# Cyan4973/FiniteStateEntropy

Hardware: AMD Instinct MI355X
Metric: MB/s encode+decode per GPU on 32KB probagen blocks; bit-exact vs CPU ref (higher is better)
Workload: dtype u8; 1 GPU; probagen Proba14, 100000 x 32KB blocks per GPU, FSE encode+decode (one-shot calls at the reference's default limits: tableLog 11, decode maxLog 12), bit-exact check; blocks_per_gpu=100000, block_bytes=32768, codec=fse, parity=fse: roundtrip-all-blocks

## Files before the change

finitestateentropy_amd/_lib.py:

```python
import ctypes
import os
import subprocess

_CSRC = os.path.join(os.path.dirname(os.path.abspath(__file__)), "csrc")


def library_path():
    if os.environ.get("FSEHIP_LIB"):
        return os.environ["FSEHIP_LIB"]
    return os.path.join(_CSRC, "libfsehip.so")


def build_library(force=False):
    if force:
        subprocess.check_call(["make", "-C", _CSRC, "clean"], stdout=subprocess.DEVNULL)
    subprocess.check_call(["make", "-C", _CSRC, "-j8", "all"], stdout=subprocess.DEVNULL)
    return library_path()


_LIB = None


def load():
    global _LIB
    if _LIB is None:
        path = library_path()
        if not os.path.exists(path):
            raise OSError("libfsehip.so is missing (%s): build it with finitestateentropy_amd.build_library(); "
                          "there is no CPU fallback" % path)
        _LIB = ctypes.CDLL(path)
    return _LIB
```

finitestateentropy_amd/csrc/capi.hip:

```cpp
#include "internal.h"
#include <string.h>
#include <stdlib.h>
#include <new>

extern "C" unsigned FSEHIP_isError(size_t code) { return code > FSEHIP_ERROR(maxCode); }

extern "C" const char* FSEHIP_getErrorName(size_t code)
{
    if (!FSEHIP_isError(code)) return "No error detected";
    switch ((int)(0 - code)) {
        case FSEHIP_error_GENERIC: return "Error (generic)";
        case FSEHIP_error_dstSize_tooSmall: return "Destination buffer is too small";
        case FSEHIP_error_srcSize_wrong: return "Src size is incorrect";
        case FSEHIP_error_corruption_detected: return "Corrupted block detected";
        case FSEHIP_error_tableLog_tooLarge: return "tableLog requires too much memory : unsupported";
        case FSEHIP_error_maxSymbolValue_tooLarge: return "Unsupported max Symbol Value : too large";
        case FSEHIP_error_maxSymbolValue_tooSmall: return "Specified maxSymbolValue is too small";
        case FSEHIP_error_workSpace_tooSmall: return "workspace buffer is too small";
        default: return "Unspecified error code";
    }
}

extern "C" const char* FSEHIP_versionString(void) { return "fsehip 0.3 (gfx950)"; }

extern "C" void FSEHIP_shardRange(size_t nBlocks, int rank, int world, size_t* first, size_t* count)
{
    if (world < 1) world = 1;
    if (rank < 0) rank = 0;
    const size_t base = nBlocks / (size_t)world, rem = nBlocks % (size_t)world, r = (size_t)rank;
    const size_t lo = r * base + (r < rem ? r : rem);
    if (first) *first = lo;
    if (count) *count = r < (size_t)world ? base + (r < rem ? 1 : 0) : 0;
}

#include <mutex>
#include <vector>
#include <utility>
namespace {
std::mutex g_devMutex;
const int MAX_DEVS = 64;
DevProps g_props[MAX_DEVS];
std::vector<std::pair<int, const void*>> g_ldsAttrDone;
}
const DevProps& dev_props()
{
    static const DevProps none = { 0, 0, false };
    int dev = 0;
    if (hipGetDevice(&dev) != hipSuccess || dev < 0 || dev >= MAX_DEVS) return none;
    std::lock_guard<std::mutex> lock(g_devMutex);
    DevProps& p = g_props[dev];
    if (!p.ok) {
        hipDeviceProp_t prop;
        if (hipGetDeviceProperties(&prop, dev) == hipSuccess) {
            p.cus = prop.multiProcessorCount;
            p.ldsPerCU = (int)prop.maxSharedMemoryPerMultiProcessor;
            p.ok = true;
        }
    }
    return p;
}
hipError_t ensure_dyn_lds(const void* kernel, int bytes)
{
    int dev = 0;
    hipError_t e = hipGetDevice(&dev);
    if (e != hipSuccess) return e;
    std::lock_guard<std::mutex> lock(g_devMutex);
    for (auto& d : g_ldsAttrDone) if (d.first == dev && d.second == kernel) return hipSuccess;
    e = hipFuncSetAttribute(kernel, hipFuncAttributeMaxDynamicSharedMemorySize, bytes);
    if (e == hipSuccess) g_ldsAttrDone.emplace_back(dev, kernel);
    return e;
}

extern "C" int FSEHIP_deviceInfo(FSEHIP_DeviceInfo* info)
{
    int dev = 0;
    hipDeviceProp_t prop;
    CK(hipGetDevice(&dev));
    CK(hipGetDeviceProperties(&prop, dev));
    info->deviceOrdinal = dev;
    info->computeUnits = prop.multiProcessorCount;
    info->ldsBytesPerCU = (int)prop.maxSharedMemoryPerMultiProcessor;
    info->wavefrontSize = prop.warpSize;
    strncpy(info->archName, prop.gcnArchName, sizeof(info->archName) - 1);
    info->archName[sizeof(info->archName) - 1] = 0;
    return 0;
}

namespace {
std::mutex g_probeMutex;
struct Probe {
    bool on = false;
    std::vector<hipEvent_t> pool;
    size_t used = 0;
    struct Rec { int id; hipEvent_t a, b; };
    std::vector<Rec> recs;
    hipEvent_t pending[PK_COUNT] = {};
    hipEvent_t get()
    {
        if (used == pool.size()) { hipEvent_t e; if (hipEventCreate(&e) != hipSuccess) return nullptr; pool.push_back(e); }
        return pool[used++];
    }
} g_probe;
}
void probe_before(int id, hipStream_t s)
{
    if (!g_probe.on) return;
    std::lock_guard<std::mutex> lock(g_probeMutex);
    hipEvent_t e = g_probe.get();
    g_probe.pending[id] = e;
    if (e) (void)hipEventRecord(e, s);
}
void probe_after(int id, hipStream_t s)
{
    if (!g_probe.on) return;
    std::lock_guard<std::mutex> lock(g_probeMutex);
    hipEvent_t e = g_probe.get();
    if (e && g_probe.pending[id]) { (void)hipEventRecord(e, s); g_probe.recs.push_back({ id, g_probe.pending[id], e }); }
}
extern "C" int FSEHIP_probe_begin(void)
{
    std::lock_guard<std::mutex> lock(g_probeMutex);
    g_probe.on = true; g_probe.used = 0; g_probe.recs.clear();
    return 0;
}
extern "C" int FSEHIP_probe_collect(double* totalMs, unsigned* launches)
{
    for (int i = 0; i < 16; ++i) { totalMs[i] = 0; launches[i] = 0; }
    std::lock_guard<std::mutex> lock(g_probeMutex);
    g_probe.on = false;
    for (auto& r : g_probe.recs) {
        CK(hipEventSynchronize(r.b));
        float ms = 0;
        CK(hipEventElapsedTime(&ms, r.a, r.b));
        totalMs[r.id] += ms; launches[r.id] += 1;
    }
    g_probe.recs.clear(); g_probe.used = 0;
    return 0;
}

extern "C" void FSEHIP_probagen_table(uint8_t table[4096], double p)
{
    int remaining = 4096;
    unsigned pos = 0, s = 0;
    if (p == 0.0) p = 0.005;
    while (remaining) {
        unsigned n = (unsigned)(remaining * p);
        if (!n) n = 1;
        memset(table + pos, (int)(uint8_t)s, n);
        pos += n; s++; remaining -= (int)n;
    }
}

extern "C" int FSEHIP_probagen_batch(void* d_dst, size_t dstStride, size_t blockSize, size_t nBlocks,
                                     const uint8_t h_table[4096], uint32_t firstSeed, void* stream)
{
    return FSEHIP_probagen_batch_ex(d_dst, dstStride, blockSize, nBlocks, h_table, firstSeed, 1, stream);
}
extern "C" int FSEHIP_probagen_batch_ex(void* d_dst, size_t dstStride, size_t blockSize, size_t nBlocks,
                                        const uint8_t h_table[4096], uint32_t firstSeed, uint32_t seedStep, void* stream)
{
    hipStream_t s = (hipStream_t)stream;
    enum { SLOTS = 16 };
    struct Ring { u8* dev = nullptr; u8* pin = nullptr; int device = -1; unsigned next = 0; hipEvent_t ev[SLOTS] = {}; bool used[SLOTS] = {}; int nEv = 0;
                  void drop() { for (int i = 0; i < nEv; ++i) (void)hipEventDestroy(ev[i]); nEv = 0;
                                if (pin) (void)hipHostFree(pin); if (dev) (void)hipFree(dev); pin = nullptr; dev = nullptr; device = -1; (void)hipGetLastError(); } };
    struct Rings { std::vector<Ring> v; ~Rings() { for (auto& r : v) r.drop(); } };
    static thread_local Rings rings;
    int dev = 0;
    CK(hipGetDevice(&dev));
    Ring* rp = nullptr;
    for (auto& r : rings.v) if (r.device == dev) rp = &r;
    if (!rp) {
        Ring r;
        hipError_t e = hipMalloc((void**)&r.dev, SLOTS * 4096);
        if (e == hipSuccess) e = hipHostMalloc((void**)&r.pin, SLOTS * 4096, hipHostMallocDefault);
        for (int i = 0; i < SLOTS && e == hipSuccess; ++i) { e = hipEventCreateWithFlags(&r.ev[i], hipEventDisableTiming); if (e == hipSuccess) r.nEv = i + 1; }
        if (e != hipSuccess) { r.drop(); return (int)e; }
        r.device = dev;
        rings.v.push_back(r);
        rp = &rings.v.back();
    }
    Ring& ring = *rp;
    const unsigned k = ring.next++ % SLOTS;
    if (ring.used[k]) CK(hipEventSynchronize(ring.ev[k]));
    memcpy(ring.pin + 4096u * k, h_table, 4096);
    u8* const d_table = ring.dev + 4096u * k;
    hipError_t e = hipMemcpyAsync(d_table, ring.pin + 4096u * k, 4096, hipMemcpyHostToDevice, s);
    if (e == hipSuccess) e = launch_probagen((u8*)d_dst, dstStride, blockSize, nBlocks, d_table, firstSeed, seedStep, s);
    if (e == hipSuccess) { e = hipEventRecord(ring.ev[k], s); ring.used[k] = e == hipSuccess; }
    return (int)e;
}

__global__ void k_batch_arg_error(size_t* results, const size_t* sizes, size_t uniform, size_t dstCapacity, size_t nBlocks, size_t code, int mode)
{
    const size_t b = (size_t)blockIdx.x * blockDim.x + threadIdx.x;
    if (b >= nBlocks) return;
    size_t r = code;
    if (mode == 1) {
        const size_t n = sizes ? sizes[b] : uniform;
        if (n == 0 || dstCapacity == 0) r = 0;
        else if (n > FSEHIP_HUF_BLOCKSIZE_MAX) r = FERR(srcSize_wrong);
    }
    if (mode == 2) { const size_t n = sizes ? sizes[b] : uniform; if (n <= 1) r = 0; }
    results[b] = r;
}
int batch_arg_error(size_t* d_results, const size_t* d_sizes, size_t uniform, size_t dstCapacity, size_t nBlocks, size_t code, int mode, hipStream_t s)
{
    hipLaunchKernelGGL(k_batch_arg_error, dim3((unsigned)((nBlocks + 255) / 256)), dim3(256), 0, s, d_results, d_sizes, uniform, dstCapacity, nBlocks, code, mode);
    return (int)hipGetLastError();
}

__global__ void k_hdr_results(const u8* meta, size_t metaStride, size_t* results, size_t nBlocks)
{
// ... 23 lines not shown
```

finitestateentropy_amd/csrc/capi_batch.hip:

```cpp
#include "internal.h"

extern "C" int FSEHIP_HIST_count_batch(unsigned* d_counts, unsigned* d_maxSymbolValues, size_t* d_results,
                                       const void* d_src, size_t srcStride, const size_t* d_sizes, size_t uniformSize,
                                       size_t nBlocks, void* stream)
{
    HistArgs a;
    a.counts = d_counts; a.maxSVs = d_maxSymbolValues; a.uniformMaxSV = 255; a.useUniformIn = 0;
    a.results = d_results; a.src = mkview(d_src, srcStride, d_sizes, uniformSize); a.nBlocks = nBlocks;
    return (int)launch_hist(a, (hipStream_t)stream);
}

extern "C" int FSEHIP_FSE_compress_usingCTable_batch(void* d_dst, size_t dstStride, size_t dstCapacity, size_t* d_results,
                                                     const void* d_src, size_t srcStride, const size_t* d_sizes, size_t uniformSize,
                                                     const FSEHIP_FSE_CTable* d_ctables, size_t ctableStrideU32, unsigned maxTableLog,
                                                     size_t nBlocks, void* stream)
{
    if (maxTableLog == 0 || maxTableLog > FSEHIP_FSE_MAX_TABLELOG) maxTableLog = FSEHIP_FSE_MAX_TABLELOG;
    FseEncArgs a;
    a.dst = (u8*)d_dst; a.dstStride = dstStride; a.dstCapacity = dstCapacity; a.results = d_results;
    a.src = mkview(d_src, srcStride, d_sizes, uniformSize);
    a.ctables = d_ctables; a.ctStrideU32 = ctableStrideU32; a.meta = nullptr;
    a.maxTableLog = maxTableLog; a.G = 0; a.slotU32 = 0; a.nBlocks = nBlocks; a.list = nullptr; a.count = nullptr;
    return (int)launch_fse_encode_auto(a, (hipStream_t)stream);
}

extern "C" int FSEHIP_FSE_decompress_usingDTable_batch(void* d_dst, size_t dstStride, size_t dstCapacity, size_t* d_results,
                                                       const void* d_cSrc, size_t cStride, const size_t* d_cSizes, size_t uniformCSize,
                                                       const FSEHIP_FSE_DTable* d_dtables, size_t dtableStrideU32, unsigned maxTableLog,
                                                       size_t nBlocks, void* stream)
{
    if (maxTableLog == 0 || maxTableLog > FSEHIP_FSE_MAX_TABLELOG) maxTableLog = FSEHIP_FSE_MAX_TABLELOG;
    FseDecArgs a;
    a.dst = (u8*)d_dst; a.dstStride = dstStride; a.dstCapacity = dstCapacity; a.results = d_results;
    a.csrc = mkview(d_cSrc, cStride, d_cSizes, uniformCSize);
    a.dtables = d_dtables; a.dtStrideU32 = dtableStrideU32; a.atab = nullptr; a.symtab = nullptr; a.meta = nullptr;
    a.maxTableLog = maxTableLog; a.G = 0; a.slotU32 = 0; a.nBlocks = nBlocks; a.tlMin = 0; a.declineNb0 = 0; a.onlyDeclined = 0;
    a.symScratch = nullptr; a.slotBitmap = nullptr; a.nSlots = 0; a.scratchSlotBytes = 0;
    return (int)launch_fse_decode(a, (hipStream_t)stream);
}

#define WS_SLACK 2048
#define WS_MAX_CHUNK 131072
static size_t ws_pass_blocks(size_t nBlocks) { const size_t c = nBlocks < WS_MAX_CHUNK ? nBlocks : WS_MAX_CHUNK; return c ? c : 1; }
static size_t ws_size(size_t nBlocks, size_t perBlock, size_t pad = 0) { return ws_pass_blocks(nBlocks) * perBlock + pad + WS_SLACK; }
static size_t round_chunk(size_t limit, size_t perRound)
{
    if (perRound == 0 || limit < perRound) return limit;
    return limit / perRound * perRound;
}
static size_t ws_chunk(size_t workspaceBytes, size_t nBlocks, size_t perBlock, size_t pad = 0, size_t perRound = 0)
{
    if (workspaceBytes < perBlock + pad + WS_SLACK) return 0;
    const size_t chunk = (workspaceBytes - WS_SLACK - pad) / perBlock;
    return chunk >= nBlocks ? nBlocks : round_chunk(chunk, perRound);
}
static inline size_t pass_blocks(size_t nBlocks, size_t b0, size_t chunk) { return nBlocks - b0 < chunk ? nBlocks - b0 : chunk; }

struct Carver {
    u8* const base; u8* p;
    explicit Carver(void* ws) : base((u8*)ws), p((u8*)ws) {}
    template <class T> T* take(size_t bytes) { T* const r = (T*)p; p += align_up(bytes, 256); return r; }
    template <class T> T* last(size_t bytes) { T* const r = (T*)p; p += bytes; return r; }
    size_t used() const { return (size_t)(p - base); }
};
template <class Meta> struct CounterWs {
    static constexpr size_t bytes_per_block = 1024 + 4 + 8 + sizeof(Meta);
    unsigned* counts; unsigned* maxSVs; size_t* hres; Meta* meta;
    CounterWs(Carver& c, size_t chunk)
        : counts(c.take<unsigned>(chunk * 1024)), maxSVs(c.take<unsigned>(chunk * 4)), hres(c.take<size_t>(chunk * 8)), meta(c.take<Meta>(chunk * sizeof(Meta))) {}
    HistArgs hist_args(unsigned msv, const BlockView& src, size_t nb) const
    {
        HistArgs h;
        h.counts = counts; h.maxSVs = maxSVs; h.uniformMaxSV = msv; h.useUniformIn = 1; h.results = hres; h.src = src; h.nBlocks = nb;
        return h;
    }
};
template <class Meta> struct BuildCTableWs {
    static constexpr size_t bytes_per_block = CounterWs<Meta>::bytes_per_block;
    Carver c; CounterWs<Meta> cb;
    BuildCTableWs(void* ws, size_t chunk) : c(ws), cb(c, chunk) {}
    size_t end() const { return c.used(); }
};

struct FseCWs { size_t perBlock; size_t ctU32; size_t ts; unsigned maxTl; };
static FseCWs fse_cws(unsigned tableLog)
{
    FseCWs w;
    unsigned tl = tableLog ? tableLog : FSEHIP_FSE_DEFAULT_TABLELOG;
    if (tl < 9) tl = 9;
    if (tl > FSEHIP_FSE_MAX_TABLELOG) tl = FSEHIP_FSE_MAX_TABLELOG;
    w.maxTl = tl;
    w.ctU32 = FSEHIP_FSE_CTABLE_SIZE_U32(tl, 255);
    w.ts = (size_t)1 << tl;
    w.perBlock = 1024 + 4 + 8 + sizeof(FseMeta) + 4 * w.ctU32 + FSE_EBINS * sizeof(u32);
    return w;
}
struct FseCompWs {
    Carver c; CounterWs<FseMeta> cb; u32* ctables; u32* encLists; u32* encCounts;
    FseCompWs(void* ws, size_t chunk, const FseCWs& w)
        : c(ws), cb(c, chunk), ctables(c.take<u32>(chunk * 4 * w.ctU32)), encLists(c.take<u32>(chunk * FSE_EBINS * sizeof(u32))),
          encCounts(c.last<u32>(FSE_EBINS * sizeof(u32))) {}
    size_t end() const { return c.used(); }
};

extern "C" size_t FSEHIP_FSE_compress_batch_workspaceSize(size_t nBlocks, unsigned tableLog) { return ws_size(nBlocks, fse_cws(tableLog).perBlock); }

extern "C" int FSEHIP_FSE_compress_batch(void* d_dst, size_t dstStride, size_t dstCapacity, size_t* d_results,
                                         const void* d_src, size_t srcStride, const size_t* d_sizes, size_t uniformSize,
                                         unsigned maxSymbolValue, unsigned tableLog, size_t nBlocks,
                                         void* d_workspace, size_t workspaceBytes, void* stream)
{
    hipStream_t s = (hipStream_t)stream;
    if ((uintptr_t)d_workspace & 255u) return (int)hipErrorInvalidValue;
    if (nBlocks == 0) return 0;
    if (tableLog > FSEHIP_FSE_MAX_TABLELOG)
        return batch_arg_error(d_results, nullptr, 0, dstCapacity, nBlocks, FSEHIP_ERROR(tableLog_tooLarge), 0, s);
    if (maxSymbolValue > 255 && tableLog != 0) {
        const size_t wksp = 4 * (size_t)FSEHIP_FSE_CTABLE_SIZE_U32(FSEHIP_FSE_MAX_TABLELOG, 255) + ((size_t)1 << FSEHIP_FSE_MAX_TABLELOG);
        const size_t ctBytes = 4 * (1 + ((size_t)1 << (tableLog - 1)) + 2 * ((size_t)maxSymbolValue + 1));
        if (ctBytes <= wksp && wksp - ctBytes < 4096)
            return batch_arg_error(d_results, d_sizes, uniformSize, dstCapacity, nBlocks, FSEHIP_ERROR(workSpace_tooSmall), 2, s);
    }
    return fse_compress_view(d_dst, dstStride, dstCapacity, d_results, mkview(d_src, srcStride, d_sizes, uniformSize), maxSymbolValue, tableLog, nBlocks,
                             d_workspace, workspaceBytes, s);
}
int fse_compress_view(void* d_dst, size_t dstStride, size_t dstCapacity, size_t* d_results, const BlockView& srcAll, unsigned maxSymbolValue, unsigned tableLog,
                      size_t nBlocks, void* d_workspace, size_t workspaceBytes, hipStream_t s)
{
    const FseCWs w = fse_cws(tableLog);
    const size_t chunk = ws_chunk(workspaceBytes, nBlocks, w.perBlock, 0, fse_encode_blocks_per_round(w.maxTl));
    if (chunk == 0) return (int)hipErrorInvalidValue;
    const FseCompWs ws(d_workspace, chunk, w);
    if (ws.end() > workspaceBytes) return (int)hipErrorInvalidValue;
    unsigned msv = maxSymbolValue ? maxSymbolValue : 255;
    if (msv > 255) msv = 255;
    for (size_t b0 = 0; b0 < nBlocks; b0 += chunk) {
        const size_t nb = pass_blocks(nBlocks, b0, chunk);
        const BlockView src = subview(srcAll, b0);
        CK(launch_hist(ws.cb.hist_args(msv, src, nb), s));
        FseCPrepArgs c;
        c.counts = ws.cb.counts; c.maxSVs = ws.cb.maxSVs; c.histResults = ws.cb.hres; c.src = src;
        c.dst = (u8*)d_dst + b0 * dstStride; c.dstStride = dstStride; c.dstCapacity = dstCapacity;
        c.maxSVReq = msv; c.tableLogReq = tableLog;
        c.ctables = ws.ctables; c.ctStrideU32 = w.ctU32; c.maxTl = w.maxTl;
        c.meta = ws.cb.meta; c.results = d_results + b0; c.nBlocks = nb;
        CK(launch_fse_cprep(c, s));
        FseEncArgs e;
        e.dst = (u8*)d_dst + b0 * dstStride; e.dstStride = dstStride; e.dstCapacity = dstCapacity; e.results = d_results + b0;
        e.src = src; e.ctables = ws.ctables; e.ctStrideU32 = w.ctU32; e.meta = ws.cb.meta;
        e.maxTableLog = w.maxTl; e.G = 0; e.slotU32 = 0; e.nBlocks = nb; e.list = ws.encLists; e.count = ws.encCounts;
        CK(launch_fse_encode_auto(e, s));
    }
    return 0;
}

struct FseDecWs {
    static size_t bytes_per_block(unsigned maxLog) { return sizeof(FseMeta) + 512 + 3 * ((size_t)1 << maxLog) + FSE_DCLS_COUNT * sizeof(u32); }
    Carver c; FseMeta* meta; s16* norms; u16* atab; u8* symtab; u32* lists; u32* counts;
    FseDecWs(void* ws, size_t chunk, unsigned maxLog)
        : c(ws), meta(c.take<FseMeta>(chunk * sizeof(FseMeta))), norms(c.take<s16>(chunk * 512)), atab(c.take<u16>((chunk * 2) << maxLog)),
          symtab(c.take<u8>(chunk << maxLog)), lists(c.take<u32>(chunk * FSE_DCLS_COUNT * sizeof(u32))), counts(c.last<u32>(FSE_DCLS_COUNT * sizeof(u32))) {}
    size_t end() const { return c.used(); }
    FseDPrepArgs dprep_args(const BlockView& cs, unsigned maxLog, size_t* results, size_t nb) const
    {
        FseDPrepArgs d;
        d.csrc = cs; d.maxLog = maxLog; d.atab = atab; d.symtab = symtab; d.norms = norms; d.meta = meta; d.lists = lists; d.counts = counts;
        d.results = results; d.nBlocks = nb; d.rawRle = 0; d.origSizes = nullptr; d.uniformOrig = 0;
        return d;
    }
};
static_assert(5 * 255 + FSE_DCLS_COUNT * sizeof(u32) <= WS_SLACK && 6 * 255 + FSE_EBINS * sizeof(u32) <= WS_SLACK, "WS_SLACK covers the padding of the FSE workspaces");
static unsigned clamp_maxlog(unsigned maxLog) { return (maxLog == 0 || maxLog > FSEHIP_FSE_MAX_TABLELOG) ? FSEHIP_FSE_MAX_TABLELOG : maxLog; }

extern "C" size_t FSEHIP_FSE_decompress_batch_workspaceSize(size_t nBlocks, unsigned maxLog) { return ws_size(nBlocks, FseDecWs::bytes_per_block(clamp_maxlog(maxLog))); }

static int fse_decompress_impl(void* d_dst, size_t dstStride, size_t dstCapacity, size_t* d_results, const BlockView& csAll, unsigned maxLog, size_t nBlocks,
                               void* d_workspace, size_t workspaceBytes, hipStream_t s, const size_t* d_origSizes, size_t uniformOrig, int rawRle,
                               const u64* d_dstOffsets = nullptr, const size_t* d_dstCaps = nullptr)
{
    if ((uintptr_t)d_workspace & 255u) return (int)hipErrorInvalidValue;
    if (nBlocks == 0) return 0;
    maxLog = clamp_maxlog(maxLog);
    const size_t chunk = ws_chunk(workspaceBytes, nBlocks, FseDecWs::bytes_per_block(maxLog), 0, fse_decode_blocks_per_round(maxLog));
    if (chunk == 0) return (int)hipErrorInvalidValue;
    const FseDecWs ws(d_workspace, chunk, maxLog);
    if (ws.end() > workspaceBytes) return (int)hipErrorInvalidValue;
    for (size_t b0 = 0; b0 < nBlocks; b0 += chunk) {
        const size_t nb = pass_blocks(nBlocks, b0, chunk);
        const BlockView cs = subview(csAll, b0);
        if (rawRle) CK(launch_rawrle_expand((u8*)d_dst + b0 * dstStride, dstStride, dstCapacity, d_results + b0, cs, d_origSizes ? d_origSizes + b0 : nullptr, uniformOrig, nb, s));
        FseDPrepArgs d = ws.dprep_args(cs, maxLog, d_results + b0, nb);
        d.rawRle = rawRle; d.origSizes = d_origSizes ? d_origSizes + b0 : nullptr; d.uniformOrig = uniformOrig;
        CK(launch_fse_dprep(d, s));
        FseDecArgs e;
        e.dst = (u8*)d_dst + b0 * dstStride; e.dstStride = dstStride; e.dstCapacity = dstCapacity; e.results = d_results + b0;
        e.csrc = cs; e.dtables = nullptr; e.dtStrideU32 = 0; e.atab = ws.atab; e.symtab = ws.symtab; e.meta = ws.meta;
        e.maxTableLog = maxLog; e.G = 0; e.slotU32 = 0; e.nBlocks = nb; e.tlMin = 0; e.declineNb0 = 0; e.onlyDeclined = 0;
        e.symScratch = nullptr; e.slotBitmap = nullptr; e.nSlots = 0; e.scratchSlotBytes = 0;
        if (d_dstOffsets) { e.dst = (u8*)d_dst; e.dstOffsets = d_dstOffsets + b0; e.dstCaps = d_dstCaps + b0; }
        CK(launch_fse_decode_classes(e, ws.lists, ws.counts, s));
    }
    return 0;
}
extern "C" int FSEHIP_FSE_decompress_batch(void* d_dst, size_t dstStride, size_t dstCapacity, size_t* d_results,
                                           const void* d_cSrc, size_t cStride, const size_t* d_cSizes, size_t uniformCSize,
                                           unsigned maxLog, size_t nBlocks,
                                           void* d_workspace, size_t workspaceBytes, void* stream)
{
    return fse_decompress_impl(d_dst, dstStride, dstCapacity, d_results, mkview(d_cSrc, cStride, d_cSizes, uniformCSize), maxLog, nBlocks,
                               d_workspace, workspaceBytes, (hipStream_t)stream, nullptr, 0, 0);
}
int fse_decompress_view(void* d_dst, const u64* d_dstOffsets, const size_t* d_dstCaps, size_t* d_results, const BlockView& csrc, unsigned maxLog, size_t nBlocks,
                        void* d_workspace, size_t workspaceBytes, hipStream_t s)
{
    return fse_decompress_impl(d_dst, 0, 0, d_results, csrc, maxLog, nBlocks, d_workspace, workspaceBytes, s, nullptr, 0, 0, d_dstOffsets, d_dstCaps);
}
extern "C" int FSEHIP_FSE_decompress_packed_batch(void* d_dst, size_t dstStride, size_t dstCapacity, size_t* d_results,
                                                  const void* d_packed, const uint64_t* d_offsets, const size_t* d_origSizes, size_t uniformOrigSize,
                                                  unsigned maxLog, size_t nBlocks, void* d_workspace, size_t workspaceBytes, void* stream)
{
    BlockView v = mkview(d_packed, 0, nullptr, 0);
    v.offsets = (const u64*)d_offsets;
    return fse_decompress_impl(d_dst, dstStride, dstCapacity, d_results, v, maxLog, nBlocks, d_workspace, workspaceBytes, (hipStream_t)stream,
                               d_origSizes, uniformOrigSize, 1);
}

extern "C" size_t FSEHIP_FSE_buildCTable_batch_workspaceSize(size_t nBlocks) { return ws_size(nBlocks, BuildCTableWs<FseMeta>::bytes_per_block); }
extern "C" int FSEHIP_FSE_buildCTable_batch(FSEHIP_FSE_CTable* d_ctables, size_t ctableStrideU32, void* d_headers, size_t headerStride, size_t headerCapacity,
                                            size_t* d_results, const void* d_src, size_t srcStride, const size_t* d_sizes, size_t uniformSize,
                                            unsigned maxSymbolValue, unsigned tableLog, size_t nBlocks, void* d_workspace, size_t workspaceBytes, void* stream)
{
    hipStream_t s = (hipStream_t)stream;
    if ((uintptr_t)d_workspace & 255u) return (int)hipErrorInvalidValue;
    if (nBlocks == 0) return 0;
    if (tableLog > FSEHIP_FSE_MAX_TABLELOG) return batch_arg_error(d_results, nullptr, 0, headerCapacity, nBlocks, FSEHIP_ERROR(tableLog_tooLarge), 0, s);
    const FseCWs w = fse_cws(tableLog);
    if (ctableStrideU32 < w.ctU32) return (int)hipErrorInvalidValue;
    const size_t chunk = ws_chunk(workspaceBytes, nBlocks, BuildCTableWs<FseMeta>::bytes_per_block);
    if (chunk == 0) return (int)hipErrorInvalidValue;
    const BuildCTableWs<FseMeta> ws(d_workspace, chunk);
    if (ws.end() > workspaceBytes) return (int)hipErrorInvalidValue;
    unsigned msv = maxSymbolValue ? maxSymbolValue : 255;
    if (msv > 255) msv = 255;
    for (size_t b0 = 0; b0 < nBlocks; b0 += chunk) {
        const size_t nb = pass_blocks(nBlocks, b0, chunk);
        const BlockView src = mkview((const u8*)d_src + b0 * srcStride, srcStride, d_sizes ? d_sizes + b0 : nullptr, uniformSize);
        CK(launch_hist(ws.cb.hist_args(msv, src, nb), s));
        FseCPrepArgs c;
        c.counts = ws.cb.counts; c.maxSVs = ws.cb.maxSVs; c.histResults = ws.cb.hres; c.src = src;
        c.dst = (u8*)d_headers + b0 * headerStride; c.dstStride = headerStride; c.dstCapacity = headerCapacity;
        c.maxSVReq = msv; c.tableLogReq = tableLog;
        c.ctables = d_ctables + b0 * ctableStrideU32; c.ctStrideU32 = ctableStrideU32; c.maxTl = w.maxTl;
        c.meta = ws.cb.meta; c.results = d_results + b0; c.nBlocks = nb;
        CK(launch_fse_cprep(c, s));
        CK(launch_hdr_results(ws.cb.meta, sizeof(FseMeta), d_results + b0, nb, s));
    }
    return 0;
}

extern "C" int FSEHIP_FSE_normalizeCount_batch(short* d_norms, size_t normStride, unsigned tableLog, const unsigned* d_counts, size_t countStride,
                                               const size_t* d_totals, const unsigned* d_maxSymbolValues, size_t nBlocks, size_t* d_results, void* stream)
{
    if (nBlocks == 0) return 0;
    if (!d_norms || !d_counts || !d_totals || !d_maxSymbolValues || !d_results || normStride < 256 || countStride < 256) return (int)hipErrorInvalidValue;
    return (int)launch_fse_glue_normalize((s16*)d_norms, normStride, tableLog, d_counts, countStride, d_totals, d_maxSymbolValues, d_results, nBlocks, (hipStream_t)stream);
}
extern "C" int FSEHIP_FSE_writeNCount_batch(void* d_headers, size_t headerStride, size_t headerCapacity, const short* d_norms, size_t normStride,
                                            const unsigned* d_maxSymbolValues, unsigned tableLog, size_t nBlocks, size_t* d_results, void* stream)
{
    if (nBlocks == 0) return 0;
    if (!d_headers || !d_norms || !d_maxSymbolValues || !d_results || normStride < 256 || headerCapacity > headerStride) return (int)hipErrorInvalidValue;
    return (int)launch_fse_glue_write_ncount((u8*)d_headers, headerStride, headerCapacity, (const s16*)d_norms, normStride, d_maxSymbolValues, tableLog, d_results, nBlocks,
                                             (hipStream_t)stream);
}
extern "C" int FSEHIP_FSE_readNCount_batch(short* d_norms, size_t normStride, unsigned* d_maxSymbolValues, unsigned* d_tableLogs,
                                           const void* d_headers, size_t headerStride, const size_t* d_headerSizes, size_t uniformHeaderSize,
                                           size_t nBlocks, size_t* d_results, void* stream)
{
    if (nBlocks == 0) return 0;
    if (!d_norms || !d_maxSymbolValues || !d_tableLogs || !d_headers || !d_results) return (int)hipErrorInvalidValue;
    return (int)launch_fse_glue_read_ncount((s16*)d_norms, normStride, d_maxSymbolValues, d_tableLogs, mkview(d_headers, headerStride, d_headerSizes, uniformHeaderSize),
                                            d_results, nBlocks, (hipStream_t)stream);
}

extern "C" size_t FSEHIP_FSE_buildDTable_batch_workspaceSize(size_t nBlocks, unsigned maxLog) { return FSEHIP_FSE_decompress_batch_workspaceSize(nBlocks, maxLog); }
extern "C" int FSEHIP_FSE_buildDTable_batch(FSEHIP_FSE_DTable* d_dtables, size_t dtableStrideU32, size_t* d_results,
                                            const void* d_headers, size_t headerStride, const size_t* d_headerSizes, size_t uniformHeaderSize,
                                            unsigned maxLog, size_t nBlocks, void* d_workspace, size_t workspaceBytes, void* stream)
{
    hipStream_t s = (hipStream_t)stream;
    if ((uintptr_t)d_workspace & 255u) return (int)hipErrorInvalidValue;
    if (nBlocks == 0) return 0;
    maxLog = clamp_maxlog(maxLog);
    if (dtableStrideU32 < FSEHIP_FSE_DTABLE_SIZE_U32(maxLog)) return (int)hipErrorInvalidValue;
    const size_t chunk = ws_chunk(workspaceBytes, nBlocks, FseDecWs::bytes_per_block(maxLog));
    if (chunk == 0) return (int)hipErrorInvalidValue;
    const FseDecWs ws(d_workspace, chunk, maxLog);
    if (ws.end() > workspaceBytes) return (int)hipErrorInvalidValue;
    for (size_t b0 = 0; b0 < nBlocks; b0 += chunk) {
        const size_t nb = pass_blocks(nBlocks, b0, chunk);
        const FseDPrepArgs d = ws.dprep_args(mkview((const u8*)d_headers + b0 * headerStride, headerStride, d_headerSizes ? d_headerSizes + b0 : nullptr, uniformHeaderSize),
                                             maxLog, d_results + b0, nb);
        CK(launch_fse_dprep(d, s));
// ... 433 lines not shown
```

finitestateentropy_amd/csrc/fse_decode.hip:

```cpp
#include "internal.h"
#include <atomic>

#include "bitreader.h"

#ifndef FSE_SYM_L1
#define FSE_SYM_L1 1
#endif
#ifndef FSE_DEC_RING
#define FSE_DEC_RING 64
#endif
#define FSE_IN_RING 256
#define FSE_IN_RING_LOG 8
#define FSE_IN_CHUNK 64
#define FSE_IN_LANES (FSE_IN_CHUNK / 4)
#define FSE_IN_MIRROR 16
#ifndef FSE_CHECK_EVERY
#define FSE_CHECK_EVERY 16
#endif
#ifndef FSE_PHASE_UNROLL
#define FSE_PHASE_UNROLL 16
#endif
#define FSE_FINISH_EVERY 2
#ifndef FSE_DEC_LDS_KB
#define FSE_DEC_LDS_KB 160
// ... 170 lines not shown
    if (lane == 0 && atomicAdd(&flagsSh[7], 1u) == FSE_SRV_WAVES + FSE_DEC_WAVES - 1) {
        const u32 slot = flagsSh[6];
        __hip_atomic_fetch_and(a.slotBitmap + (slot >> 5), ~(1u << (slot & 31u)), __ATOMIC_RELEASE, __HIP_MEMORY_SCOPE_AGENT);
    }
}
DEV u32 srv_rl(u32 v, int l) { return (u32)__builtin_amdgcn_readlane((int)v, l); }
DEV unsigned long long srv_rl64(unsigned long long v, int l) { return (unsigned long long)srv_rl((u32)v, l) | ((unsigned long long)srv_rl((u32)(v >> 32), l) << 32); }
template <bool TIMED, bool CALLER>
DEV void fse_decode_service(const FseDecArgs& a, u8* ldsb, DecCtl* ctlAll, u32 slotBytes, u32 ringOff, u32 inOff, int lane, int g0, bool rev, u32* flagsSh)
{
    const int myG = g0 + (lane < FSE_SRV_G ? lane : 0);
    DecCtl* const ctl = ctlAll + (myG < a.G ? myG : 0);
    const unsigned long long inBits = ((unsigned long long)ctl->inHi << 32) | ctl->inLo;
    const unsigned long long outBits = ((unsigned long long)ctl->outHi << 32) | ctl->outLo;
    const unsigned long long tabBits = ((unsigned long long)ctl->symHi << 32) | ctl->symLo;
    const int S32 = ctl->S32;
    int validLo = ctl->initValidLo;
    u32 flushed = 0, fpos = 0;
    bool live = lane < FSE_SRV_G && myG < a.G && !(ctl->pubPofs >> 31);

    static_assert(64 / FSE_IN_LANES == FSE_SRV_G, "one 16-lane group per block of a service wave");
    const int grp = lane / FSE_IN_LANES, sub = lane % FSE_IN_LANES;
    const int SgK = __shfl(S32, grp, WAVE);
    const gbl_u8_ptr igK = (gbl_u8_ptr)(uintptr_t)__shfl(inBits, grp, WAVE);
    u32* const rgK = (u32*)(ldsb + (size_t)(g0 + grp) * slotBytes + inOff);
    {   const bool liveK = (__ballot(live) >> grp) & 1ull;
        const int vlo = __shfl(validLo, grp, WAVE);
#pragma unroll
        for (int c = 0; c < FSE_IN_RING / FSE_IN_CHUNK; ++c) {
            const int off = liveK ? vlo + FSE_IN_CHUNK * c + 4 * sub : -1;
            if (off >= 0 && off + 4 <= SgK) { const u32 w = gbl_load_u32(igK + off); if (rev) fse_ring_put_rev(rgK, SgK, off, w); else fse_ring_put(rgK, off, w); }
            else if (off >= 0 && off < SgK) {
                u32 w = 0;
                for (int i = 0; i < 3; ++i) if (off + i < SgK) w |= (u32)igK[off + i] << (8 * i);
                if (rev) fse_ring_put_rev(rgK, SgK, off, w); else fse_ring_put(rgK, off, w);
            }
        }
        if (live) ctl_store(&ctl->srvValidLo, validLo);
    }

    int nextOff = __shfl(validLo, grp, WAVE) - FSE_IN_CHUNK + 4 * sub;
    u32 pend = 0;
    if (((__ballot(live) >> grp) & 1ull) && nextOff >= 0 && nextOff + 4 <= SgK) pend = gbl_load_u32(igK + nextOff);
    u32 yq[FSE_SRV_G][4];
#pragma unroll
    for (int l = 0; l < FSE_SRV_G; ++l) { yq[l][0] = yq[l][1] = yq[l][2] = yq[l][3] = 0; }
    unsigned long long sBusy = 0, sIdle = 0, nBusy = 0, sA = 0;
    (void)sBusy; (void)sIdle; (void)nBusy; (void)sA;
    TIMING(sA = __builtin_readcyclecounter(););
    for (;;) {
        u32 pp = 0x80000000u, it = flushed;
        if (live) { const u64 pub = ctl_load2(&ctl->pubIters); it = (u32)pub; pp = (u32)(pub >> 32); }
        const bool fin = (pp >> 31) != 0;
        const int P = (int)(pp & 0x7FFFFFFFu);
        const u32 avail = it - flushed;
        const bool wantFlush = live && (avail >= FSE_FLUSH_MIN || (fin && avail > 0));
        const bool wantFill = live && !fin && validLo > 0 && P + 4 <= validLo + (FSE_IN_RING - FSE_IN_CHUNK);
        const unsigned long long fm = __ballot(wantFlush), rm = __ballot(wantFill);
        if (live && fin && avail == 0) live = false;
        if (!(fm | rm)) {
            if (!__any(live)) break;
            __builtin_amdgcn_s_sleep(4);
            TIMING(const unsigned long long sB = __builtin_readcyclecounter(); sIdle += sB - sA; sA = sB;);
            continue;
        }
        const bool fillK = (rm >> grp) & 1ull;
        if (rm) {
            if (fillK) { if (rev) fse_ring_put_rev(rgK, SgK, nextOff, pend); else fse_ring_put(rgK, nextOff, pend); }
            if (wantFill) { validLo -= FSE_IN_CHUNK; ctl_store(&ctl->srvValidLo, validLo); }
            if (fillK) {
                nextOff -= FSE_IN_CHUNK;
                pend = 0;
                if (nextOff >= 0 && nextOff + 4 <= SgK) pend = gbl_load_u32(igK + nextOff);
            }
        }
#pragma unroll
        for (int l = 0; l < FSE_SRV_G; ++l) {
            if (!((fm >> l) & 1ull)) continue;
            const u32 cnt = srv_rl(avail, l), fp_g = srv_rl(fpos, l);
            const gbl_u8_ptr tg = (gbl_u8_ptr)(uintptr_t)srv_rl64(tabBits, l);
            if ((u32)lane < cnt) {
                u32 ri = fp_g + (u32)lane;
                ri = ri >= FSE_DEC_RING ? ri - FSE_DEC_RING : ri;
                const u32* const rw = (const u32*)(ldsb + (size_t)(g0 + l) * slotBytes + ringOff) + 4u * (ri >> 1) + (ri & 1u);
                uint2 rec; rec.x = rw[0]; rec.y = rw[2];
                const u32 x0 = __builtin_amdgcn_ubfe(rec.x, 1u, a.ldsLog), x1 = __builtin_amdgcn_ubfe(rec.x, 17u, a.ldsLog);
                const u32 x2 = __builtin_amdgcn_ubfe(rec.y, 1u, a.ldsLog), x3 = __builtin_amdgcn_ubfe(rec.y, 17u, a.ldsLog);
#if FSE_SYM_L1
                yq[l][0] = tg[x0]; yq[l][2] = tg[x1]; yq[l][1] = tg[x2]; yq[l][3] = tg[x3];
#else
                if (CALLER) {
                    yq[l][0] = __hip_atomic_load(tg + x0, __ATOMIC_RELAXED, __HIP_MEMORY_SCOPE_AGENT); yq[l][2] = __hip_atomic_load(tg + x1, __ATOMIC_RELAXED, __HIP_MEMORY_SCOPE_AGENT);
                    yq[l][1] = __hip_atomic_load(tg + x2, __ATOMIC_RELAXED, __HIP_MEMORY_SCOPE_AGENT); yq[l][3] = __hip_atomic_load(tg + x3, __ATOMIC_RELAXED, __HIP_MEMORY_SCOPE_AGENT);
                } else { yq[l][0] = tg[x0]; yq[l][2] = tg[x1]; yq[l][1] = tg[x2]; yq[l][3] = tg[x3]; }
#endif
            }
        }
        if (wantFlush) { ctl_store(&ctl->srvFlushed, it); }
#pragma unroll
        for (int l = 0; l < FSE_SRV_G; ++l) {
            if (!((fm >> l) & 1ull)) continue;
            const u32 cnt = srv_rl(avail, l), fl_g = srv_rl(flushed, l);
            gbl_u8_w_ptr const og = (gbl_u8_w_ptr)(uintptr_t)(srv_rl64(outBits, l) + 4ull * fl_g);
            if ((u32)lane < cnt) {
                const u32 w = yq[l][0] | (yq[l][1] << 8) | (yq[l][2] << 16) | (yq[l][3] << 24);
                gbl_store_u32(og + 4u * lane, w);
            }
        }
        if (wantFlush) { fpos += it - flushed; fpos = fpos >= FSE_DEC_RING ? fpos - FSE_DEC_RING : fpos; flushed = it; }
        TIMING(const unsigned long long sB = __builtin_readcyclecounter(); sBusy += sB - sA; sA = sB; ++nBusy;);
    }
    TIMING(if (lane == 0 && g0 == 0) { atomicAdd(&g_decTiming[5], sBusy); atomicAdd(&g_decTiming[6], sIdle); });
    if (CALLER) fse_scratch_slot_done(a, flagsSh, lane);
}

struct FseCellsRef { const u32* cells;
    DEV void get(u32 st, u32& ns, u32& nb, u32& sym) const { const u32 c = cells[st]; ns = c & 0xFFFFu; sym = (c >> 16) & 0xFFu; nb = c >> 24; } };
struct FseCellsCompact { const u16* A; const u8* syms;
    DEV void get(u32 st, u32& ns, u32& nb, u32& sym) const { const u32 c = A[st]; ns = c & 0xFFFu; nb = c >> 12; sym = syms[st]; } };
struct FseCellsRev { const u16* A; const u8* syms; u32 tl, cellShift;
    DEV void get(u32 st, u32& ns, u32& nb, u32& sym) const { const u32 i = __brev(st) >> (32u - tl); const u32 c = A[i]; nb = c & 31u; ns = __brev(c >> cellShift) >> (32u - tl); sym = syms[i]; } };
template <class Cells>
DEV u32 fse_tail_step(const Cells& t, u32& state, BitReader& r, bool fast)
{
    u32 ns, nb, sym;
    t.get(state, ns, nb, sym);
    const u32 low = fast ? r.read_fast(nb) : r.read(nb);
    state = ns + low;
    return sym;
}
template <class Cells>
DEV size_t fse_tail(const Cells& t, u32 s1, u32 s2, BitReader& r, u8* out, long op, long omax, bool fast)
{
    for (;;) {
        const int st = r.reload();
        if (!((st == BR_UNFINISHED) & (op < omax - 3))) break;
        u32 w = fse_tail_step(t, s1, r, fast);
        w |= fse_tail_step(t, s2, r, fast) << 8;
        w |= fse_tail_step(t, s1, r, fast) << 16;
        w |= fse_tail_step(t, s2, r, fast) << 24;
        __builtin_memcpy(out + op, &w, 4);
        op += 4;
    }
    for (;;) {
        if (op > omax - 2) return FERR(dstSize_tooSmall);
        out[op++] = (u8)fse_tail_step(t, s1, r, fast);
        if (r.reload() == BR_OVERFLOW) { out[op++] = (u8)fse_tail_step(t, s2, r, fast); return (size_t)op; }
        if (op > omax - 2) return FERR(dstSize_tooSmall);
        out[op++] = (u8)fse_tail_step(t, s2, r, fast);
        if (r.reload() == BR_OVERFLOW) { out[op++] = (u8)fse_tail_step(t, s1, r, fast); return (size_t)op; }
    }
}

template <bool FAST, bool TIMED, bool CALLER, bool VIEW = false>
__global__ __launch_bounds__(FSE_DEC_THREADS) void k_fse_decode(FseDecArgs a)
{
    extern __shared__ __attribute__((aligned(16))) u32 lds[];
    const int tid = threadIdx.x, lane = tid & 63, wave = tid >> 6;
    unsigned long long tBorn = 0, wBorn = 0;
    (void)tBorn; (void)wBorn;
    TIMING(tBorn = __builtin_readcyclecounter(); wBorn = wall_clock64(););
    const size_t first = (size_t)blockIdx.x * a.G;
    static_assert(FSE_DBINS % 4 == 0, "the bin lengths are read as 16-byte vectors");
    size_t nTot = a.nBlocks, q0 = first;
    u32 bin0 = 0, cnt0 = 0xFFFFFFFFu;
    if (a.count) {
        uint4 cv[FSE_DBINS / 4];
#pragma unroll
        for (u32 i = 0; i < FSE_DBINS / 4; ++i) cv[i] = ((const uint4*)a.count)[i];
        u64 before = 0;
        bool found = false;
#pragma unroll
        for (u32 i = 0; i < FSE_DBINS; ++i) {
            const uint4 v = cv[i >> 2];
            const u32 c = (i & 3u) == 0 ? v.x : (i & 3u) == 1 ? v.y : (i & 3u) == 2 ? v.z : v.w;
            const bool here = !found & (((u64)first < before + c) | (i == FSE_DBINS - 1));
            bin0 = here ? i : bin0; q0 = here ? (size_t)((u64)first - before) : q0; cnt0 = here ? c : cnt0;
            found |= here;
            before += c;
        }
        nTot = (size_t)before;
    }
    if (first >= nTot) return;
    auto slotBlock = [&](size_t g) -> size_t {
        if (!a.list) return first + g;
        size_t q = q0 + g; u32 i = bin0;
        if (q >= cnt0) {
            while (i < FSE_DBINS - 1) { const u32 c = a.count[i]; if (q < c) break; q -= c; ++i; }
        }
        return a.list[(size_t)i * a.nBlocks + q];
    };
    u8* const lds8 = (u8*)lds;
    const u32 tabStride = 2u << a.ldsLog;
    DecCtl* const ctlAll = (DecCtl*)(lds8 + (size_t)a.G * tabStride);
    u8* const ldsb = (u8*)ctlAll + (size_t)a.G * sizeof(DecCtl);
    const u32 slotBytes = a.slotU32 * 4u;
    const u32 ringOff = 0;
    const u32 inOff = FSE_DEC_RING * 8;

    u32* const flagsSh = (u32*)(ldsb + (size_t)a.G * slotBytes);
    if (tid < 6 || tid == 7) flagsSh[tid] = 0;
    const bool decWave = wave < FSE_DEC_WAVES;
    u8* const tlSh = (u8*)(flagsSh + 8);
    if (CALLER) {
        __syncthreads();
        bool mine = false;
        if (tid >= 64 && tid < 64 + a.G) {
            const size_t g = (size_t)tid - 64;
            u32 tl = 0xFFu;
            if (first + g < nTot) {
                const size_t bi = slotBlock(g);
                if (!(a.onlyDeclined && a.results[bi] != FSE_DECLINED)) {
                    const u32 t0 = a.dtables[bi * a.dtStrideU32] & 0xFFFFu;
                    if (t0 <= a.ldsLog && t0 >= a.tlMin) tl = t0;
                    else if (t0 > a.maxTableLog && a.tlMin == 0 && !a.onlyDeclined) a.results[bi] = FERR(tableLog_tooLarge);
                }
            }
            tlSh[g] = (u8)tl;
            mine = tl != 0xFFu;
        }
        if (mine) flagsSh[1] = 1u;
        u32 slot = 0;
        if (tid == 0) slot = fse_scratch_slot_claim(a, flagsSh);
        __syncthreads();
        if (!flagsSh[1]) {
            if (tid == 0) __hip_atomic_fetch_and(a.slotBitmap + (slot >> 5), ~(1u << (slot & 31u)), __ATOMIC_RELEASE, __HIP_MEMORY_SCOPE_AGENT);
            return;
        }
    }
    else __syncthreads();
    u8* const symSlot = CALLER ? a.symScratch + (size_t)flagsSh[6] * a.scratchSlotBytes : nullptr;
    {   u64 badBits = 0, declBits = 0; bool anyNb0 = false;
        if (!CALLER) {
            const size_t nTab = nTot - first < (size_t)a.G ? nTot - first : (size_t)a.G;
            if (tabStride >= 1024u) {
                const u32 ppt = tabStride >> 10;
                const u32 nPieces = (u32)nTab * ppt;
                for (u32 p = (u32)wave; p < nPieces; p += FSE_DEC_THREADS / 64) {
                    const u32 g = p / ppt, k = p - g * ppt;
                    const size_t bi = slotBlock(g);
                    const u8* const src = (const u8*)(a.atab + (bi << a.maxTableLog)) + 1024u * k + 16u * (u32)lane;
                    __builtin_amdgcn_global_load_lds((const __attribute__((address_space(1))) void*)src,
                                                     (__attribute__((address_space(3))) void*)(lds8 + 1024u * p), 16, 0, 0);
                }
            }
            else {
            uint4* const dstv = (uint4*)lds8;
            const u32 vptLog = a.ldsLog - 3u;
            const u32 nvec = (u32)nTab << vptLog;
            constexpr u32 MAXV = (FSE_MAXG * 512u / 16u + FSE_DEC_THREADS - 1) / FSE_DEC_THREADS;
            uint4 buf[MAXV];
#pragma unroll
            for (u32 k = 0; k < MAXV; ++k) {
                const u32 idx = tid + k * FSE_DEC_THREADS;
                if (idx < nvec) {
                    const size_t sl = first + (idx >> vptLog);
                    const size_t bi = slotBlock(sl - first);
                    buf[k] = ((const uint4*)(a.atab + (bi << a.maxTableLog)))[idx & ((1u << vptLog) - 1u)];
                }
            }
#pragma unroll
            for (u32 k = 0; k < MAXV; ++k) { const u32 idx = tid + k * FSE_DEC_THREADS; if (idx < nvec) dstv[idx] = buf[k]; }
            }
            if (!FAST) for (size_t g = 0; g < nTab; ++g) {
                const u32 st = a.meta[slotBlock(g)].state; anyNb0 |= st != 0 && !(st & 2u); }
        }
        else {
            const size_t nTab = nTot - first < (size_t)a.G ? nTot - first : (size_t)a.G;
            constexpr u32 QL = 2048u / 4u / 64u;
            if (!decWave) for (u32 g = (u32)wave - FSE_DEC_WAVES; g < (u32)nTab; g += FSE_SRV_WAVES) {
                const u32 tl = tlSh[g];
                if (tl == 0xFFu) continue;
                const u32 ts = 1u << tl;
                const u32* const t = a.dtables + slotBlock(g) * a.dtStrideU32;
                u8* const slotB = lds8 + (size_t)g * tabStride;
                u16* const A = (u16*)slotB;
                u8* const symOut = symSlot + ((size_t)g << a.ldsLog);
                bool bad = false, nbz = false;
                if (FAST && tl >= 4u) {
                    const u32 sR = 32u - tl;
                    const u32 qo[4] = { 0u, 1u << (tl - 1u), 1u << (tl - 2u), 3u << (tl - 2u) };
                    const u32 passes = ts > 2048u ? ts / 2048u : 1u;
                    u32 acc = 0, minNb = 15u;
                    uint4 cv[QL];
                    for (u32 h = 0; h < passes; ++h) {
#pragma unroll
                        for (u32 j = 0; j < QL; ++j) {
                            const u32 i0 = 2048u * h + 4u * ((u32)lane + 64u * j);
                            cv[j] = make_uint4(0, 0, 0, 0);
                            if (i0 < ts) __builtin_memcpy(&cv[j], t + 1 + i0, 16);
                        }
#pragma unroll
                        for (u32 j = 0; j < QL; ++j) {
                            const u32 i0 = 2048u * h + 4u * ((u32)lane + 64u * j);
                            if (i0 >= ts) continue;
                            const u32 r0 = __brev(i0) >> sR;
                            const u32 cw[4] = { cv[j].x, cv[j].y, cv[j].z, cv[j].w };
#pragma unroll
                            for (u32 q = 0; q < 4; ++q) {
                                const u32 c = cw[q], ns = c & 0xFFFFu, nb = c >> 24;
                                acc |= (ns >> tl) | ((tl - nb) >> 5) | (ns & ((1u << (nb & 31u)) - 1u));
                                minNb = nb < minNb ? nb : minNb;
                                slotB[r0 | qo[q]] = (u8)(c >> 16);
                            }
                        }
                    }
                    { for (u32 off = 16u * (u32)lane; off < ts; off += 1024u) { const uint4 v = *(const uint4*)(slotB + off); *(uint4*)(symOut + off) = v; } }
                    for (u32 h = 0; h < passes; ++h) {
                        if (passes > 1u) {
#pragma unroll
                            for (u32 j = 0; j < QL; ++j) { const u32 i0 = 2048u * h + 4u * ((u32)lane + 64u * j); __builtin_memcpy(&cv[j], t + 1 + i0, 16); }
                        }
#pragma unroll
                        for (u32 j = 0; j < QL; ++j) {
                            const u32 i0 = 2048u * h + 4u * ((u32)lane + 64u * j);
                            if (i0 >= ts) continue;
                            const u32 r0 = __brev(i0) >> sR;
                            const u32 cw[4] = { cv[j].x, cv[j].y, cv[j].z, cv[j].w };
#pragma unroll
                            for (u32 q = 0; q < 4; ++q) {
                                const u32 c = cw[q];
                                A[r0 | qo[q]] = (u16)(((__brev(c << 16) >> (16u - tl)) << 5) | ((c >> 24) & 31u));
                            }
                        }
                    }
                    bad = acc != 0; nbz = minNb == 0;
                } else {
#pragma unroll 2
                    for (u32 i = (u32)lane; i < ts; i += 64u) {
                        const u32 c = t[1 + i];
                        const u32 ns = c & 0xFFFFu, nb = c >> 24;
                        bad |= (ns >> tl) != 0 || nb > tl || nb > 15u || (ns & ((1u << (nb & 15u)) - 1u)) != 0;
                        nbz |= nb == 0;
                        const u32 pos = FAST ? __brev(i) >> (32u - tl) : i;
                        symOut[pos] = (u8)(c >> 16);
                        if (FAST) A[pos] = (u16)((nb & 31u) | ((__brev(ns & ((1u << tl) - 1u)) >> (32u - tl)) << 5));
                        else A[pos] = (u16)((ns & 0xFFFu) | (nb << 12));
                    }
                }
                if (__any(bad)) badBits |= 1ull << g;
                if (FAST && tl == 12u && __any(nbz)) declBits |= 1ull << g;
                anyNb0 |= __any(nbz) != 0;
            }
        }
        if (badBits) { atomicOr(&flagsSh[2], (u32)badBits); atomicOr(&flagsSh[3], (u32)(badBits >> 32)); }
        if (declBits) { atomicOr(&flagsSh[4], (u32)declBits); atomicOr(&flagsSh[5], (u32)(declBits >> 32)); }
        if (anyNb0) atomicOr(&flagsSh[0], 1u);
    }
    const int ppw = (a.G + FSE_DEC_WAVES - 1) / FSE_DEC_WAVES;
    const int gsl = (decWave ? wave * ppw : 0) + (lane >> 1);
    const u32 half = (u32)lane & 1u, maskB = half ? ~0u : 0u;
    const bool inRange = (lane >> 1) < ppw && gsl < a.G && first + (size_t)gsl < nTot;
    const size_t b = inRange ? slotBlock((size_t)gsl) : 0;
    bool owner = decWave && inRange;
    u32 hdr = 0;
    if (owner && a.meta) { if (a.meta[b].state == 0) owner = false; else hdr = a.meta[b].hdrSize; }
    u32 tl = 0; bool fast = false;
    constexpr bool compact = !CALLER;
    const u32* const gtab = compact ? nullptr : a.dtables + (owner ? b : 0) * a.dtStrideU32;
    if (owner) {
        if (compact) { tl = a.meta[b].tableLog; fast = (a.meta[b].state & 2u) != 0; if (tl > a.ldsLog) { a.results[b] = FERR(tableLog_tooLarge); owner = false; } }
        else {
            const u32 h0 = gtab[0]; tl = h0 & 0xFFFFu; fast = (h0 >> 16) != 0;
            if (tlSh[gsl] == 0xFFu) owner = false;
        }
    }
    const u32* const cells = compact ? nullptr : gtab + 1;
    const u8* const syms = compact ? a.symtab + ((owner ? b : 0) << a.maxTableLog) : symSlot + ((size_t)(gsl < a.G ? gsl : 0) << a.ldsLog);
    const u32 ldsBase = (u32)(uintptr_t)(__attribute__((address_space(3))) u8*)lds8;
    if (ldsBase & (tabStride - 1)) __builtin_trap();
    const u32 tabOff = ldsBase + (u32)(gsl < a.G ? gsl : 0) * tabStride;
    const u16* const A = (const u16*)(lds8 + (tabOff - ldsBase));
    const u8* in = nullptr; size_t S = 0; u8* out = nullptr;
    const long omax = VIEW ? (long)a.dstCaps[owner ? b : 0] : (long)a.dstCapacity;
    long op = 0;
    BitReader r; r.base = nullptr; r.size = 0; r.at = 0; r.win = 0; r.used = 0;
    u32 s1 = 0, s2 = 0;
    if (owner) {
        in = view_ptr(a.csrc, b) + hdr;
        S = view_size(a.csrc, b) - hdr;
        out = VIEW ? a.dst + a.dstOffsets[b] : a.dst + b * a.dstStride;
        const size_t e = r.init(in, S);
        if (is_err(e)) { a.results[b] = e; owner = false; }
        else {
            s1 = r.read(tl); r.reload();
            s2 = r.read(tl); r.reload();
        }
    }

    __builtin_amdgcn_s_waitcnt(0x0f70);
    __syncthreads();
    const u64 badMask = (u64)flagsSh[2] | ((u64)flagsSh[3] << 32);
    const u64 declMask = (u64)flagsSh[4] | ((u64)flagsSh[5] << 32);
    const bool nb0 = flagsSh[0] != 0;
    if (CALLER && owner && a.declineNb0 && ((declMask >> gsl) & 1ull)) { if (half == 0) a.results[b] = FSE_DECLINED; owner = false; }

    const bool bulkOk = owner && S < (1ull << 28) && !((badMask >> gsl) & 1ull) && !(FAST && !compact && ((declMask >> gsl) & 1ull));
    const int Bstart = bulkOk ? (int)(8u * ((u32)r.at + 8u)) - (int)r.used : 0;
    const long groups0 = (omax - 3 - op + 3) / 4;
    bool can = bulkOk && (FAST ? Bstart >= 65 + 48 * (FSE_CHECK_EVERY - 1) : r.at >= 24 + 6 * FSE_CHECK_EVERY + 8) && groups0 >= FSE_CHECK_EVERY;
    bool can2 = FAST && bulkOk && Bstart >= 65 + 48 * (FSE_FINISH_EVERY - 1) && groups0 >= FSE_FINISH_EVERY;
    const bool everBulk = can || can2;
    BulkState bs; bs.q = 0; bs.bq = 0;
    {   const u32 st = half ? s2 : s1;
        bs.s = tabOff + 2u * (FAST ? __brev(st) >> (32u - (tl ? tl : 1u)) : st); }
    const u32 inA = (u32)((uintptr_t)in & 3u);
    const u32 R8 = 8u * (((u32)S + inA + 3u) & ~3u);
    u32 P = 0;
    long groups = 0;
    u32 iters = 0;
    int validLo = 0;
    if (everBulk) {
        const u32 B = 8u * ((u32)r.at + 8u + inA) - r.used;
        bs.q = 4u * (B >> 5) - 8u; bs.bq = B & 31u; P = R8 - B;
        groups = (omax - 3 - op + 3) >> 2;
        const int c0 = (int)((0 - ((uintptr_t)in - inA)) & (FSE_IN_CHUNK - 1));
        validLo = (((int)bs.q + 8 - 112 - c0) & ~(FSE_IN_CHUNK - 1)) + c0;
    }
    DecCtl* const ctl = ctlAll + (gsl < a.G ? gsl : 0);
    if (decWave && (lane >> 1) < ppw && gsl < a.G && half == 0) {
        ctl->pubIters = 0; ctl->pubPofs = everBulk ? bs.q + 8u : 0x80000000u;
        ctl->srvFlushed = 0; ctl->srvValidLo = 0x7FFFFFFF;
        ctl->initValidLo = validLo; ctl->S32 = (int)(S < (1ull << 31) ? S + inA : 0);
        const unsigned long long ib = (unsigned long long)(uintptr_t)(in - inA), ob = (unsigned long long)(uintptr_t)out, tb = (unsigned long long)(uintptr_t)syms;
        ctl->inLo = (u32)ib; ctl->inHi = (u32)(ib >> 32); ctl->outLo = (u32)ob; ctl->outHi = (u32)(ob >> 32); ctl->symLo = (u32)tb; ctl->symHi = (u32)(tb >> 32);
    }
    __syncthreads();
    if (!decWave) { fse_decode_service<TIMED, CALLER>(a, ldsb, ctlAll, slotBytes, ringOff, inOff, lane, (wave - FSE_DEC_WAVES) * FSE_SRV_G, FAST, flagsSh); return; }

    __builtin_amdgcn_s_setprio(3);
    uint2* const myRing = (uint2*)(ldsb + (size_t)(gsl < a.G ? gsl : 0) * slotBytes + ringOff) + half;
    const u32 myIn = (u32)(uintptr_t)(__attribute__((address_space(3))) u8*)(ldsb + (size_t)(gsl < a.G ? gsl : 0) * slotBytes + inOff);
    unsigned long long tRun = 0, tWait = 0, nRun = 0, nWait = 0, tA = 0, tFin = 0, nFin = 0, tInner = 0;
    (void)tRun; (void)tWait; (void)nRun; (void)nWait; (void)tA; (void)tFin; (void)nFin; (void)tInner;
    TIMING(tA = __builtin_readcyclecounter(););
    const unsigned long long tBulk0 = tA;
    (void)tBulk0;
    u32 rpos = 0;
    u64 srvNext = ctl_peek2(&ctl->srvFlushed);
    const u32 inA8 = 8u * inA;
    u32 Phead = P;
    int grp = groups > (1 << 30) ? (1 << 30) : (int)groups;
    if constexpr (FAST) {
        uint2* const dummyRing = (uint2*)(flagsSh + 32) + half;
        if ((lane >> 1) < ppw && everBulk) {
        for (;;) {
            const int lowest = (int)bs.q - 4 * ((48 * (FSE_CHECK_EVERY - 1) + 31) / 32);
            const int need = lowest > 0 ? lowest : 0;
            bool rdy;
            do {
                const u32 fl = (u32)srvNext;
                const int vlo = (int)(u32)(srvNext >> 32);
                srvNext = ctl_peek2(&ctl->srvFlushed);
                rdy = !can | ((iters + FSE_CHECK_EVERY - fl <= FSE_DEC_RING) & (need >= vlo));
                TIMING(if (!__all(rdy)) { const unsigned long long tB = __builtin_readcyclecounter(); tWait += tB - tA; ++nWait; tA = tB; });
            } while (!__all(rdy));
            if (!__any(can)) break;
            uint2* const ring = can ? myRing + rpos : dummyRing;
            u32 sN = bs.s, Pn = P, PhN = Phead;
            unsigned long long tI = 0; (void)tI;
            TIMING(tI = __builtin_readcyclecounter(););
            fse_bulk_phase_rev<FSE_CHECK_EVERY>(sN, Pn, PhN, tl + 1u, 4u, tabOff, myIn, maskB & 31u, ring);
            TIMING(tInner += __builtin_readcyclecounter() - tI;);
            bs.s = can ? sN : bs.s; P = can ? Pn : P; Phead = can ? PhN : Phead;
            const u32 adv = can ? (u32)FSE_CHECK_EVERY : 0u;
            rpos = (rpos + adv) & (FSE_DEC_RING - 1);
            iters += adv; grp -= (int)adv;
            const u32 B = R8 - P;
            bs.q = 4u * (B >> 5) - 8u;
            const u32 Bp = B - inA8;
            const bool canN = can & (Bp >= 65u + 48u * (FSE_CHECK_EVERY - 1)) & (grp >= FSE_CHECK_EVERY);
            const bool more = canN | ((Bp >= 65u + 48u * (FSE_FINISH_EVERY - 1)) & (grp >= FSE_FINISH_EVERY));
            if (can & (half == 0)) ctl_store2(&ctl->pubIters, iters, more ? bs.q + 8u : ((bs.q + 8u) | 0x80000000u));
            can = canN;
            TIMING(const unsigned long long tB = __builtin_readcyclecounter(); tRun += tB - tA; ++nRun; tA = tB;);
        }
        {   const u32 B = R8 - P; bs.bq = B & 31u;
            can2 = bulkOk & (B - inA8 >= 65u + 48u * (FSE_FINISH_EVERY - 1)) & (grp >= FSE_FINISH_EVERY); }
        can2 = can2 & bulkOk;
        for (;;) {
            const u32 fl = (u32)srvNext;
            const int vlo = (int)(u32)(srvNext >> 32);
            srvNext = ctl_peek2(&ctl->srvFlushed);
            const int lowest = (int)bs.q - 8;
            const bool rdy = !can2 | ((iters + FSE_FINISH_EVERY - fl <= FSE_DEC_RING) & ((lowest > 0 ? lowest : 0) >= vlo));
            if (!__all(rdy)) {
                TIMING(const unsigned long long tB = __builtin_readcyclecounter(); tWait += tB - tA; ++nWait; tA = tB;);
                continue;
            }
            if (!__any(can2)) break;
            uint2* const ring = can2 ? myRing + rpos : dummyRing;
            u32 sN = bs.s, Pn = P, PhN = Phead;
            fse_bulk_phase_rev<FSE_FINISH_EVERY>(sN, Pn, PhN, tl + 1u, 4u, tabOff, myIn, maskB & 31u, ring);
            bs.s = can2 ? sN : bs.s; P = can2 ? Pn : P; Phead = can2 ? PhN : Phead;
            rpos = can2 ? (rpos + FSE_FINISH_EVERY) & (FSE_DEC_RING - 1) : rpos;
            iters += can2 ? FSE_FINISH_EVERY : 0u; grp -= can2 ? FSE_FINISH_EVERY : 0;
            const u32 B = R8 - P;
            bs.q = 4u * (B >> 5) - 8u; bs.bq = B & 31u;
            const bool can2N = can2 & (B - inA8 >= 65u + 48u * (FSE_FINISH_EVERY - 1)) & (grp >= FSE_FINISH_EVERY);
            if (can2 & (half == 0)) ctl_store2(&ctl->pubIters, iters, can2N ? bs.q + 8u : ((bs.q + 8u) | 0x80000000u));
            can2 = can2N;
            TIMING(const unsigned long long tB = __builtin_readcyclecounter(); tFin += tB - tA; ++nFin; tA = tB;);
        }
        }
    } else {
    while (__any(can)) {
        const u32 fl = (u32)srvNext;
        const int vlo = (int)(u32)(srvNext >> 32);
        srvNext = ctl_peek2(&ctl->srvFlushed);
        const int lowest = (int)bs.q - (6 * FSE_CHECK_EVERY + 8);
        const bool ready = can & (iters + FSE_CHECK_EVERY - fl <= FSE_DEC_RING) & ((lowest > 0 ? lowest : 0) >= vlo);
        if (ready) {
            uint2* const ring = myRing + rpos;
            rpos = (rpos + FSE_CHECK_EVERY) & (FSE_DEC_RING - 1);
            if (nb0) fse_bulk_phase<true>(bs.s, bs.q, bs.bq, tabOff, myIn, half, maskB, ring);
            else     fse_bulk_phase<false>(bs.s, bs.q, bs.bq, tabOff, myIn, half, maskB, ring);
            iters += FSE_CHECK_EVERY; grp -= FSE_CHECK_EVERY;
            can = (bs.q >= 24u + 6u * FSE_CHECK_EVERY + 4u) & (grp >= FSE_CHECK_EVERY);
            if (half == 0) ctl_store2(&ctl->pubIters, iters, can ? bs.q + 8u : ((bs.q + 8u) | 0x80000000u));
        }
        TIMING(const unsigned long long tB = __builtin_readcyclecounter(); if (__any(ready)) { tRun += tB - tA; ++nRun; } else { tWait += tB - tA; ++nWait; } tA = tB;);
    }
    }
    TIMING(if (lane == 0) { atomicAdd(&g_decTiming[0], tRun); atomicAdd(&g_decTiming[1], tWait); atomicAdd(&g_decTiming[2], nRun); atomicAdd(&g_decTiming[3], nWait); atomicAdd(&g_decTiming[4], 1ull);
                            atomicAdd(&g_decTiming[13], tBulk0 - tBorn); atomicAdd(&g_decTiming[15], tFin); atomicAdd(&g_decTiming[10], nFin); atomicAdd(&g_decTiming[7], tInner); });
    const u32 sOther = dpp_swap(bs.s);
    const unsigned long long tBulk1 = tA;
    (void)tBulk1;
    if (owner && !half) {
    op = 4 * (long)iters;
    if (iters) {
        const u32 B = 8u * (bs.q + 8u) + bs.bq - 8u * inA;
        const u32 Bh = FAST ? R8 - Phead - 8u * inA : B;
        r.at = (size_t)((Bh + 7u) >> 3) - 8; r.used = 8u * ((u32)r.at + 8u) - B; r.win = ldg64u(in + r.at); s1 = (bs.s - tabOff) >> 1; s2 = (sOther - tabOff) >> 1;
        if (FAST) { s1 = __brev(s1) >> (32u - tl); s2 = __brev(s2) >> (32u - tl); }
    }

    size_t result;
    if (!compact) {
        if ((badMask >> gsl) & 1ull) result = fse_tail(FseCellsRef{cells}, s1, s2, r, out, op, omax, fast);
        else if (FAST)               result = fse_tail(FseCellsRev{A, syms, tl, 5u}, s1, s2, r, out, op, omax, fast);
        else                         result = fse_tail(FseCellsCompact{A, syms}, s1, s2, r, out, op, omax, fast);
    }
    else if (FAST)    result = fse_tail(FseCellsRev{A, syms, tl, 5u}, s1, s2, r, out, op, omax, fast);
    else              result = fse_tail(FseCellsCompact{A, syms}, s1, s2, r, out, op, omax, fast);
    a.results[b] = result;
    TIMING(if (lane == 0) { const unsigned long long tE = __builtin_readcyclecounter(); atomicAdd(&g_decTiming[11], tE - tBorn); atomicAdd(&g_decTiming[12], wall_clock64() - wBorn);
                            atomicAdd(&g_decTiming[14], tE - tBulk1); });
    }
    if (CALLER) fse_scratch_slot_done(a, flagsSh, lane);
}

static void fse_decode_geometry(unsigned ldsLog, size_t ldsBytes, unsigned* slotU32, int* G)
{
    *slotU32 = (FSE_DEC_RING * 8 + FSE_IN_RING + FSE_IN_MIRROR + 16) / 4;
    int g = (int)((ldsBytes - 256) / ((2u << ldsLog) + *slotU32 * 4 + sizeof(DecCtl)));
    if (g > FSE_MAXG) g = FSE_MAXG;
    *G = g;
}
#define FSE_DEC_LDS (FSE_DEC_LDS_KB * 1024)
size_t fse_decode_blocks_per_round(unsigned maxTableLog)
{
    unsigned slot; int G;
    fse_decode_geometry(maxTableLog < FSE_DEC_FAST_MAXLOG ? maxTableLog : FSE_DEC_FAST_MAXLOG, FSE_DEC_LDS, &slot, &G);
    const int cus = dev_props().ok ? dev_props().cus : 256;
    return (size_t)G * FSE_WGS_PER_CU * cus;
}

#define FSE_SYM_SLOT_BYTES (FSE_MAXG * 2048u)
#include <mutex>
namespace {
std::mutex g_symMutex;
struct SymScratch { u8* base = nullptr; u32* bitmap = nullptr; u32 nSlots = 0; };
SymScratch g_symScratch[64];
}
static hipError_t fse_sym_scratch(FseDecArgs& a, hipStream_t s)
{
    int dev = 0;
    hipError_t e = hipGetDevice(&dev);
    if (e != hipSuccess) return e;
    if (dev < 0 || dev >= 64) return hipErrorInvalidDevice;
    std::lock_guard<std::mutex> lock(g_symMutex);
    SymScratch& sc = g_symScratch[dev];
    if (!sc.base && s) {
        hipStreamCaptureStatus st = hipStreamCaptureStatusNone;
        if (hipStreamIsCapturing(s, &st) == hipSuccess && st != hipStreamCaptureStatusNone) return hipErrorStreamCaptureUnsupported;
        (void)hipGetLastError();
    }
    if (!sc.base) {
        const u32 nSlots = 2u * (u32)(dev_props().ok ? dev_props().cus : 256);
        const size_t bitmapBytes = ((nSlots + 31u) / 32u * 4u + 255u) & ~(size_t)255;
        u8* p = nullptr;
        e = hipMalloc((void**)&p, bitmapBytes + (size_t)nSlots * FSE_SYM_SLOT_BYTES);
        if (e != hipSuccess) return e;
        e = hipMemset(p, 0, bitmapBytes);
        if (e != hipSuccess) { (void)hipFree(p); return e; }
        sc.bitmap = (u32*)p; sc.base = p + bitmapBytes; sc.nSlots = nSlots;
    }
    a.symScratch = sc.base; a.slotBitmap = sc.bitmap; a.nSlots = sc.nSlots; a.scratchSlotBytes = FSE_SYM_SLOT_BYTES;
    return hipSuccess;
}

static hipError_t fse_decode_launch(FseDecArgs a, bool rev, hipStream_t s)
{
    const size_t ldsBytes = FSE_DEC_LDS;
    const bool caller = a.atab == nullptr;
    {   hipError_t e = ensure_dyn_lds((const void*)k_fse_decode<true, false, false>, FSE_DEC_LDS);
        if (e == hipSuccess) e = ensure_dyn_lds((const void*)k_fse_decode<false, false, false>, FSE_DEC_LDS);
        if (e == hipSuccess) e = ensure_dyn_lds((const void*)k_fse_decode<true, true, false>, FSE_DEC_LDS);
        if (e == hipSuccess && caller) e = ensure_dyn_lds((const void*)k_fse_decode<true, false, true>, FSE_DEC_LDS);
        if (e == hipSuccess && caller) e = ensure_dyn_lds((const void*)k_fse_decode<false, false, true>, FSE_DEC_LDS);
        if (e == hipSuccess && caller) e = fse_sym_scratch(a, s);
        if (e != hipSuccess) return e;
    }
    fse_decode_geometry(a.ldsLog, ldsBytes, &a.slotU32, &a.G);
    if (a.G < 1) return hipErrorInvalidValue;
    if (caller && ((size_t)a.G << a.ldsLog) > FSE_SYM_SLOT_BYTES) return hipErrorInvalidValue;
    const size_t groups = (a.nBlocks + a.G - 1) / a.G;
    if (a.dstOffsets) {
        if (caller || !a.dstCaps) return hipErrorInvalidValue;
        hipError_t e = ensure_dyn_lds((const void*)k_fse_decode<true, false, false, true>, FSE_DEC_LDS);
        if (e == hipSuccess) e = ensure_dyn_lds((const void*)k_fse_decode<false, false, false, true>, FSE_DEC_LDS);
        if (e != hipSuccess) return e;
        if (rev) hipLaunchKernelGGL((k_fse_decode<true, false, false, true>), dim3((unsigned)groups), dim3(FSE_DEC_THREADS), ldsBytes, s, a);
        else     hipLaunchKernelGGL((k_fse_decode<false, false, false, true>), dim3((unsigned)groups), dim3(FSE_DEC_THREADS), ldsBytes, s, a);
        return hipGetLastError();
    }
    if (caller) {
        if (rev && g_decTimingOn.load(std::memory_order_relaxed)) {
            hipError_t e = ensure_dyn_lds((const void*)k_fse_decode<true, true, true>, FSE_DEC_LDS);
            if (e != hipSuccess) return e;
            hipLaunchKernelGGL((k_fse_decode<true, true, true>), dim3((unsigned)groups), dim3(FSE_DEC_THREADS), ldsBytes, s, a);
        }
        else if (rev) hipLaunchKernelGGL((k_fse_decode<true, false, true>), dim3((unsigned)groups), dim3(FSE_DEC_THREADS), ldsBytes, s, a);
        else     hipLaunchKernelGGL((k_fse_decode<false, false, true>), dim3((unsigned)groups), dim3(FSE_DEC_THREADS), ldsBytes, s, a);
    }
    else if (rev && g_decTimingOn.load(std::memory_order_relaxed)) hipLaunchKernelGGL((k_fse_decode<true, true, false>), dim3((unsigned)groups), dim3(FSE_DEC_THREADS), ldsBytes, s, a);
    else if (rev) hipLaunchKernelGGL((k_fse_decode<true, false, false>), dim3((unsigned)groups), dim3(FSE_DEC_THREADS), ldsBytes, s, a);
    else          hipLaunchKernelGGL((k_fse_decode<false, false, false>), dim3((unsigned)groups), dim3(FSE_DEC_THREADS), ldsBytes, s, a);
    return hipGetLastError();
}

extern "C" __attribute__((visibility("default"))) int FSEHIP_prepareDevice(void)
{
    FseDecArgs a = FseDecArgs();
    return (int)fse_sym_scratch(a, nullptr);
}

extern "C" __attribute__((visibility("default"))) int FSEHIP_debug_decodeTiming(int enable, unsigned long long* out16)
{
    hipError_t e = hipDeviceSynchronize();
    if (e != hipSuccess) return (int)e;
    if (enable) {
        unsigned long long zero[16] = { 0 };
        e = hipMemcpyToSymbol(HIP_SYMBOL(g_decTiming), zero, sizeof(zero));
        g_decTimingOn.store(e == hipSuccess);
        return (int)e;
    }
    g_decTimingOn.store(false);
    if (!out16) return 0;
    e = hipMemcpyFromSymbol(out16, HIP_SYMBOL(g_decTiming), sizeof(g_decTiming));
    if (e != hipSuccess) return (int)e;
    int dev = 0, khz = 0;
    (void)hipGetDevice(&dev);
    (void)hipDeviceGetAttribute(&khz, hipDeviceAttributeClockRate, dev);
    unsigned slot; int G;
    fse_decode_geometry(FSE_DEC_FAST_MAXLOG, FSE_DEC_LDS, &slot, &G);
    out16[8] = (unsigned long long)khz; out16[9] = (unsigned long long)G | ((unsigned long long)FSE_WGS_PER_CU << 32) | ((unsigned long long)FSE_DEC_WAVES << 40) | ((unsigned long long)FSE_CHECK_EVERY << 48);
    return 0;
}

hipError_t launch_fse_decode(FseDecArgs a, hipStream_t s)
{
    if (a.nBlocks == 0) return hipSuccess;
    a.list = nullptr; a.count = nullptr;
    probe_before(PK_FSE_DECODE, s);
    a.ldsLog = a.maxTableLog < FSE_DEC_FAST_MAXLOG ? a.maxTableLog : FSE_DEC_FAST_MAXLOG;
    a.tlMin = 0; a.declineNb0 = 0; a.onlyDeclined = 0;
    hipError_t e = fse_decode_launch(a, true, s);
    if (e == hipSuccess && a.maxTableLog > FSE_DEC_FAST_MAXLOG) {
        a.ldsLog = a.maxTableLog; a.tlMin = FSE_DEC_FAST_MAXLOG + 1; a.declineNb0 = 1;
        e = fse_decode_launch(a, true, s);
        if (e == hipSuccess) { a.tlMin = 0; a.declineNb0 = 0; a.onlyDeclined = 1; e = fse_decode_launch(a, false, s); }
    }
    probe_after(PK_FSE_DECODE, s);
    return e;
}

hipError_t launch_fse_decode_classes(FseDecArgs a, const u32* lists, const u32* counts, hipStream_t s)
{
    if (a.nBlocks == 0) return hipSuccess;
    probe_before(PK_FSE_DECODE, s);
    hipError_t e = hipSuccess;
    for (int c = 0; c < FSE_DCLS_KINDS && e == hipSuccess; ++c) {
        if (c != FSE_DCLS_REV11 && a.maxTableLog <= FSE_DEC_FAST_MAXLOG) break;
        a.list = lists + (size_t)c * FSE_DBINS * a.nBlocks; a.count = counts + c * FSE_DBINS;
        a.ldsLog = c == FSE_DCLS_REV11 ? (a.maxTableLog < FSE_DEC_FAST_MAXLOG ? a.maxTableLog : FSE_DEC_FAST_MAXLOG) : a.maxTableLog;
        e = fse_decode_launch(a, c != FSE_DCLS_PLAIN, s);
    }
    probe_after(PK_FSE_DECODE, s);
    return e;
}
```

finitestateentropy_amd/csrc/fse_encode.hip:

```cpp
#include "internal.h"

#define FSE_ENC_STEP(x, sym, bits, nb)                                                              \
    {   const u32 f2 = tt[2 * (sym)], dn = tt[2 * (sym) + 1];                                        \
        nb = ((x) + dn) >> 16;                                                                       \
        bits = __builtin_amdgcn_ubfe((x), 0u, nb);                                                   \
        (x) = *(const u16*)(ldsb + ((((x) >> nb) << 1) + f2));                                       \
    }

__global__ __launch_bounds__(64) void k_fse_encode(FseEncArgs a)
{
    extern __shared__ __attribute__((aligned(16))) u32 lds[];
    const u8* const ldsb = (const u8*)lds;
    const u32 lane = threadIdx.x;
    const size_t first = (size_t)blockIdx.x * a.G;

    if (a.meta) {
        const size_t bb = first + lane;
        const bool mine = lane < (u32)a.G && bb < a.nBlocks && !fse_enc_skip(a.meta[bb].state, a.onlyState);
        if (!__any(mine)) return;
    }

    for (int g = 0; g < a.G; ++g) {
        const size_t b = first + g;
        if (b >= a.nBlocks) break;
        if (a.meta && fse_enc_skip(a.meta[b].state, a.onlyState)) continue;
        if (a.sizeSplit && view_size(a.src, b) >= FSE_ENC_WAVE_MIN) continue;
        const u32* t = a.ctables + b * a.ctStrideU32;
        const u32 h = t[0];
        const u32 tl = h & 0xFFFFu, msv = (h >> 16) > 255u ? 255u : (h >> 16);
        if (tl > a.maxTableLog) continue;
        const u32 ttStart = 1 + (tl ? (1u << (tl - 1)) : 1u);
        const u32 words = ttStart + 2 * (msv + 1);
        u32* s = lds + (size_t)g * a.slotU32;
        const u32 stOff = (u32)(g * a.slotU32 + 1) * 4u;
        for (u32 i = lane; i < words; i += 64) {
            u32 v = t[i];
            if (i >= ttStart && (((i - ttStart) & 1u) == 0)) v = 2u * v + stOff;
            s[i] = v;
        }
    }
    __syncthreads();
    if (lane >= (u32)a.G) return;
    const size_t b = first + lane;
    if (b >= a.nBlocks) return;
    u32 hdr = 0;
    if (a.meta) { if (fse_enc_skip(a.meta[b].state, a.onlyState)) return; hdr = a.meta[b].hdrSize; }
    if (a.sizeSplit && view_size(a.src, b) >= FSE_ENC_WAVE_MIN) return;

    const u32 h0 = a.ctables[b * a.ctStrideU32];
    const u32 tl = h0 & 0xFFFFu;
    if (tl > a.maxTableLog) {
        a.results[b] = FERR(tableLog_tooLarge);
        return;
    }
    const u32* const tt = lds + (size_t)lane * a.slotU32 + 1 + (tl ? (1u << (tl - 1)) : 1u);

    const u8* const sbase = a.src.offsets ? a.src.base + a.src.offsets[b] : a.src.base + first * a.src.stride;
    const u32 soff = a.src.offsets ? 0u : lane * (u32)a.src.stride;
    u8* const dbase = a.dst + first * a.dstStride;
    const u32 doff = lane * (u32)a.dstStride + hdr;
    const size_t n64 = view_size(a.src, b);
    const size_t cap64 = a.dstCapacity - hdr;

    size_t csize = 0;
    if (n64 >= ((size_t)1 << 31)) { a.results[b] = FERR(srcSize_wrong); return; }
    const u32 n = (u32)n64;
    if (n > 2 && cap64 > 8) {
        const u32 lim = (u32)(cap64 - 8);
        u64 acc = 0; u32 nacc = 0, pos = 0;
#define FSE_FLUSH()                                                                                  \
        {   __builtin_memcpy(dbase + (doff + pos), &acc, 8);                                          \
            const u32 nby = nacc >> 3;                                                                \
            pos += nby; pos = pos > lim ? lim : pos;                                                  \
            acc >>= (nby << 3); nacc &= 7u; }
        u32 xa, xb;
        {   const u32 s0 = sbase[soff + n - 1], s1 = sbase[soff + n - 2];
            const u32 f0 = tt[2 * s0], d0 = tt[2 * s0 + 1], f1 = tt[2 * s1], d1 = tt[2 * s1 + 1];
            const u32 n0 = (d0 + (1u << 15)) >> 16, n1 = (d1 + (1u << 15)) >> 16;
            xa = *(const u16*)(ldsb + (((((n0 << 16) - d0) >> n0) << 1) + f0));
            xb = *(const u16*)(ldsb + (((((n1 << 16) - d1) >> n1) << 1) + f1));
        }
        u32 idx = n - 2;
        bool swapped = false;
        while (idx > 0 && (((uintptr_t)(sbase + soff) + idx) & 15u)) {
            const u32 sym = sbase[soff + idx - 1];
            u32 bits, nb;
            FSE_ENC_STEP(xa, sym, bits, nb)
            acc |= (u64)bits << nacc; nacc += nb;
            FSE_FLUSH()
            const u32 tsw = xa; xa = xb; xb = tsw; swapped = !swapped;
            --idx;
        }
        if (idx >= 16) {
            uint4 cur = *(const uint4*)(sbase + (soff + idx - 16));
            while (idx >= 16) {
                const u32 nidx = idx - 16;
                const uint4 nxt = *(const uint4*)(sbase + (soff + (nidx >= 16 ? nidx - 16 : nidx)));
                u32 ba, na, bb, nbb;
#define FSE_PAIR(w, hiA, hiB)                                                                        \
                {   const u32 sa = __builtin_amdgcn_ubfe(w, hiA, 8u), sb = __builtin_amdgcn_ubfe(w, hiB, 8u); \
                    FSE_ENC_STEP(xa, sa, ba, na)                                                      \
                    FSE_ENC_STEP(xb, sb, bb, nbb)                                                     \
                    acc |= (u64)(ba | (bb << na)) << nacc; nacc += na + nbb; }
                FSE_PAIR(cur.w, 24u, 16u) FSE_PAIR(cur.w, 8u, 0u) FSE_FLUSH()
                FSE_PAIR(cur.z, 24u, 16u) FSE_PAIR(cur.z, 8u, 0u) FSE_FLUSH()
                FSE_PAIR(cur.y, 24u, 16u) FSE_PAIR(cur.y, 8u, 0u) FSE_FLUSH()
                FSE_PAIR(cur.x, 24u, 16u) FSE_PAIR(cur.x, 8u, 0u) FSE_FLUSH()
                cur = nxt;
                idx = nidx;
            }
        }
        while (idx > 0) {
            const u32 sym = sbase[soff + idx - 1];
            u32 bits, nb;
            FSE_ENC_STEP(xa, sym, bits, nb)
            acc |= (u64)bits << nacc; nacc += nb;
            FSE_FLUSH()
            const u32 tsw = xa; xa = xb; xb = tsw; swapped = !swapped;
            --idx;
        }
        if (swapped) { const u32 tsw = xa; xa = xb; xb = tsw; }
        const u32 c2 = (n & 1) ? xb : xa, c1 = (n & 1) ? xa : xb;
        acc |= (u64)(c2 & ((1u << tl) - 1u)) << nacc; nacc += tl; FSE_FLUSH()
        acc |= (u64)(c1 & ((1u << tl) - 1u)) << nacc; nacc += tl; FSE_FLUSH()
        acc |= (u64)1 << nacc; nacc += 1; FSE_FLUSH()
        csize = (pos >= lim) ? 0 : (size_t)pos + (nacc > 0);
#undef FSE_FLUSH
#undef FSE_PAIR
    }
    if (a.meta) {
        size_t r = 0;
        if (csize != 0 && (size_t)hdr + csize < n64 - 1) r = (size_t)hdr + csize;
        a.results[b] = r;
    } else a.results[b] = csize;
}

#define FSE_ENC_LDS (80 * 1024)
static void fse_encode_geometry(unsigned maxTableLog, unsigned* slotU32, int* G)
{
    *slotU32 = (1 + (1u << (maxTableLog - 1)) + 512) | 1u;
    int g = (int)(FSE_ENC_LDS / (*slotU32 * 4));
    if (g > 64) g = 64;
    *G = g;
}
size_t fse_encode_blocks_per_round(unsigned maxTableLog)
{
    unsigned slot; int G;
    fse_encode_geometry(maxTableLog, &slot, &G);
    const int cus = dev_props().ok ? dev_props().cus : 256;
    return (size_t)G * 2 * cus;
}

hipError_t launch_fse_encode(FseEncArgs a, hipStream_t s)
{
    if (a.nBlocks == 0) return hipSuccess;
    const size_t ldsBytes = FSE_ENC_LDS;
    {   const hipError_t e = ensure_dyn_lds((const void*)k_fse_encode, (int)ldsBytes); if (e != hipSuccess) return e; }
    fse_encode_geometry(a.maxTableLog, &a.slotU32, &a.G);
    if (a.nBlocks > 1 && ((a.src.stride > 0x3FFFFFFu) || (a.dstStride > 0x3FFFFFFu))) a.G = 1;
    if (a.dstCapacity > 0x7FFFFFF0u) a.dstCapacity = 0x7FFFFFF0u;
    const size_t groups = (a.nBlocks + a.G - 1) / a.G;
    probe_before(PK_FSE_ENCODE, s);
    hipLaunchKernelGGL(k_fse_encode, dim3((unsigned)groups), dim3(64), ldsBytes, s, a);
    probe_after(PK_FSE_ENCODE, s);
    return hipGetLastError();
}
```

finitestateentropy_amd/csrc/fse_encode_wave.hip:

```cpp
#include "internal.h"

#ifndef FSE_WV_WARM_FACTOR
#define FSE_WV_WARM_FACTOR 2u
#endif
#define FSE_WV_WARM_MIN 64u
#define FSE_WV_WARM_MAX 4096u

typedef const __attribute__((address_space(3))) u16* wv_lds_u16;
typedef const __attribute__((address_space(3))) u32* wv_lds_u32;
typedef u32 wv_u32x2 __attribute__((ext_vector_type(2)));
typedef const __attribute__((address_space(3))) wv_u32x2* wv_lds_u64;
DEV u32 wv_lds_addr(const void* p) { return (u32)(uintptr_t)(const __attribute__((address_space(3))) u8*)p; }
template <bool TT4>
DEV void wv_step(u32& st, u32 ttb, u32 sym, u32& nb)
{
    if (TT4) {
        const u32 e = *(wv_lds_u32)(uintptr_t)(ttb + 4u * sym);
        nb = (st + (e & 0xFFFFu)) >> 12;
        st = *(wv_lds_u16)(uintptr_t)(((st >> nb) + (u32)((int)e >> 16)) << 1);
    } else {
        const wv_u32x2 e = *(wv_lds_u64)(uintptr_t)(ttb + 8u * sym);
        nb = (st + e.y) >> 16;
        st = *(wv_lds_u16)(uintptr_t)(((st >> nb) << 1) + e.x);
    }
// ... 284 lines not shown
    WvCk ck; ck.slot = (uint2*)(ringBase + hl * (WV_RING / 4)); ck.merged = false; ck.d = 0; ck.idx = 0;
    ck.every = (2u * C / 64u + WV_CK_MAX - 1u) / WV_CK_MAX; ck.every = ck.every ? ck.every : 1u;
    if (C & 63u) ck.every = 0x7FFFFFFFu;
    ck.left = ck.every; ck.total = (2u * C / 64u) / ck.every;
    u32 cstart = 0, cmid = 0, cend = 0, bitsLo = 0, bitsTot = 0;
    if (mineC) {
        u32 x, scratch = 0;
        if (sLo <= 2 + warm) {
            x = wv_init_state<TT4>(ttb, src[n - 1 - cc]);
            wv_chain<TT4, WV_CK_NONE>(ttb, src, n, 2, sLo, cc, x, scratch);
        } else {
            x = 1u << tl;
            wv_chain<TT4, WV_CK_NONE>(ttb, src, n, sLo - warm, sLo, cc, x, scratch);
        }
        cstart = x;
        u32 lo = sLo, hi = sMid, nbits = 0;
#pragma nounroll
        for (int piece = 0; piece < 2; ++piece) {
            wv_chain<TT4, WV_CK_RECORD>(ttb, src, n, lo, hi, cc, x, nbits, &ck);
            if (piece == 0) { cmid = x; bitsLo = nbits; }
            lo = sMid; hi = sHi;
        }
        cend = x; bitsTot = nbits;
    }
    ETIMING(T2 = __builtin_readcyclecounter();)
#ifndef WV_SAMPLE_CACHE
#define WV_SAMPLE_CACHE 1
#endif
    u32 oStart = 0xFFFFFFFFu, oEnd = 0, oMid = 0, oLo = 0, oTot = 0;
    u32 rEnd = cend, rMid = cmid, rLo = bitsLo, rTot = bitsTot;
    for (;;) {
        u32 prevEnd; bool bad;
        for (;;) {
            prevEnd = (u32)__shfl_up((int)cend, 2, WAVE);
            bad = mineC && kk > 0 && cstart != prevEnd;
            const bool hit = WV_SAMPLE_CACHE && bad && oStart == prevEnd;
            if (!__any(hit)) break;
            if (hit) {
                u32 t;
                t = cstart; cstart = oStart; oStart = t;  t = cend; cend = oEnd; oEnd = t;  t = cmid; cmid = oMid; oMid = t;
                t = bitsLo; bitsLo = oLo; oLo = t;  t = bitsTot; bitsTot = oTot; oTot = t;
            }
        }
        if (!__any(bad)) break;
        ETIMING(if (rounds == 0) { const unsigned long long bm = __ballot(bad); nBad0 = (u32)__builtin_popcountll(bm); firstBad = (u32)__builtin_ctzll(bm); })
        if (bad) {
            oStart = cstart; oEnd = cend; oMid = cmid; oLo = bitsLo; oTot = bitsTot;
            cstart = prevEnd; cend = rEnd; cmid = rMid; bitsLo = rLo; bitsTot = rTot;
            u32 x = cstart, lo = sLo, hi = sMid, nbits = 0;
            ck.merged = false; ck.idx = 0; ck.left = ck.every;
            bool midDone = false;
#pragma nounroll
            for (int piece = 0; piece < 2 && !ck.merged; ++piece) {
                wv_chain<TT4, WV_CK_MERGE>(ttb, src, n, lo, hi, cc, x, nbits, &ck);
                if (piece == 0 && !ck.merged) { cmid = x; bitsLo = nbits; midDone = true; }
                lo = sMid; hi = sHi;
            }
            if (ck.merged) {
                if (!midDone) bitsLo += ck.d;
                bitsTot += ck.d;
            } else { cend = x; bitsTot = nbits; }
            rEnd = cend; rMid = cmid; rLo = bitsLo; rTot = bitsTot;
        }
        ETIMING(++rounds;)
    }
    ETIMING(T3 = __builtin_readcyclecounter();)
    u32 start, bits;
    {   const int la = (int)(partBase + (hl & ~1u)), lb = la + 1;
        const u32 sA = (u32)__shfl((int)cstart, la, WAVE), sB = (u32)__shfl((int)cstart, lb, WAVE);
        const u32 mA = (u32)__shfl((int)cmid, la, WAVE), mB = (u32)__shfl((int)cmid, lb, WAVE);
        const u32 lA = (u32)__shfl((int)bitsLo, la, WAVE), lB = (u32)__shfl((int)bitsLo, lb, WAVE);
        const u32 tA = (u32)__shfl((int)bitsTot, la, WAVE), tB = (u32)__shfl((int)bitsTot, lb, WAVE);
        start = cc ? (mA | (mB << 16)) : (sA | (sB << 16));
        bits = cc ? (tA - lA) + (tB - lB) : lA + lB;
    }
    u32 xa = 0, xb = 0;

    u32 incl = bits;
#pragma unroll
    for (int off = 1; off < (int)WV_LANES; off <<= 1) { const u32 o = (u32)__shfl_up((int)incl, off, WAVE); if ((int)hl >= off) incl += o; }
    const u32 excl = incl - bits;
    const u64 bodyBits = (u32)__shfl((int)incl, (int)(partBase + WV_LANES - 1u), WAVE);

    const u64 totalBits = bodyBits + 2u * tl + 1u;
    const size_t whole = (size_t)(totalBits >> 3);
    size_t csize = (whole >= cap - 8) ? 0 : (size_t)((totalBits + 7) >> 3);
    size_t result = csize;
    if (a.meta) result = (csize != 0 && (size_t)hdr + csize < n64 - 1) ? (size_t)hdr + csize : 0;
    if (on && result == 0) { if (hl == 0) a.results[b] = 0; on = false; }

    {   const unsigned long long thin = __ballot(on && mine && hl < lastLane && bits < 8u);
        const unsigned long long partMask = (WV_LANES == 64u ? ~0ull : ((1ull << (WV_LANES & 63u)) - 1ull)) << partBase;
        if (on && (thin & partMask)) {
            if (a.meta && a.onlyState == FSE_ENC_PAR) {
                if (hl == 0) const_cast<FseMeta*>(a.meta)[b].state = FSE_ENC_LANE;
            } else if (hl == 0) {
                const size_t cs = wv_serial<TT4>(ttb, src, n, dst, cap, tl);
                a.results[b] = a.meta ? ((cs != 0 && (size_t)hdr + cs < n64 - 1) ? (size_t)hdr + cs : 0) : cs;
            }
            on = false;
        }
    }
    u32 tail = 0;
    if (on && mine) {
        WvSink k;
        const u32 lead = (u32)((uintptr_t)dst & (WV_RING - 1));
        const u32 off0 = lead + (excl >> 3);
        k.dstAl = dst - lead; k.ring = ringBase + hl * (WV_RING / 4); k.ringA = wv_lds_addr(k.ring);
        k.woff = off0 & ~3u; k.done = off0; k.acc = 0; k.nacc = 8u * (off0 & 3u) + (excl & 7u);
        xa = start & 0xFFFFu; xb = start >> 16;
        wv_emit<TT4>(ttb, src, n, j0, j1, xa, xb, k);
        if (hl == lastLane) {
            const u32 c2 = (n & 1u) ? xb : xa, c1 = (n & 1u) ? xa : xb;
            const u32 mask = (1u << tl) - 1u;
            k.push(c2 & mask, tl);
            k.push(c1 & mask, tl);
            k.push(1u, 1u);
            k.nacc = (k.nacc + 7u) & ~7u;
        }
        k.ring[(k.woff & (WV_RING - 1)) >> 2] = k.acc;
        k.copy_out(k.woff + (k.nacc >> 3));
        tail = k.acc >> (k.nacc & ~7u);
    }
    const u32 prevTail = (u32)__shfl_up((int)tail, 1, WAVE);
    if (on && mine && hl > 0 && (excl & 7u)) {
        u8* const p = dst + (excl >> 3);
        const uintptr_t ad = (uintptr_t)p;
        atomicOr((u32*)(ad & ~(uintptr_t)3), prevTail << (8u * (u32)(ad & 3u)));
    }
    ETIMING(T4 = __builtin_readcyclecounter(); if (hl == 0 && b < 4096) { unsigned long long* t = g_encTiming + 8 * b; t[0] = T1 - T0; t[1] = T2 - T1; t[2] = T3 - T2; t[3] = T4 - T3; t[4] = rounds; t[5] = nBad0; t[6] = firstBad; })
    if (on && hl == 0) a.results[b] = result;
}

__global__ __launch_bounds__(64) void k_fse_enc_lists(FseEncArgs a)
{
    const size_t b = (size_t)blockIdx.x * 64 + threadIdx.x;
    const u32 lane = threadIdx.x;
    int bin = -1;
    if (b < a.nBlocks && a.meta[b].state == FSE_ENC_PAR) { const u32 p = a.meta[b].pace; bin = (int)(p < FSE_EBINS ? p : FSE_EBINS - 1); }
    const unsigned long long below = (1ull << lane) - 1ull;
    for (int c = 0; c < FSE_EBINS; ++c) {
        const unsigned long long mask = __ballot(bin == c);
        if (!mask) continue;
        const int leader = __builtin_ctzll(mask);
        u32 base = 0;
        if ((int)lane == leader) base = atomicAdd(&a.count[c], (u32)__builtin_popcountll(mask));
        base = (u32)__shfl((int)base, leader, WAVE);
        if (bin == c) a.list[(size_t)c * a.nBlocks + base + (u32)__builtin_popcountll(mask & below)] = (u32)b;
    }
}
hipError_t launch_fse_enc_lists(const FseEncArgs& a, hipStream_t s)
{
    if (a.nBlocks == 0) return hipSuccess;
    const hipError_t e = launch_zero_u32(a.count, FSE_EBINS, s);
    if (e != hipSuccess) return e;
    hipLaunchKernelGGL(k_fse_enc_lists, dim3((unsigned)((a.nBlocks + 63) / 64)), dim3(64), 0, s, a);
    return hipGetLastError();
}

hipError_t launch_fse_encode_wave(FseEncArgs a, hipStream_t s)
{
    if (a.nBlocks == 0) return hipSuccess;
    const bool tt4 = a.maxTableLog <= 11;
    const u32 tableWords = (2 + (1u << (a.maxTableLog - 1)) + (tt4 ? 256 : 512) + 2 + 31) & ~31u;
#ifndef WV_EXTRA_LDS_WORDS
#define WV_EXTRA_LDS_WORDS 0u
#endif
    const u32 slotWords = tableWords + WV_LANES * (WV_RING / 4) + WV_EXTRA_LDS_WORDS;
    const size_t ldsBytes = 4 * (size_t)slotWords * WV_BPW * FSE_WV_WAVES;
    const size_t perGroup = (size_t)WV_BPW * FSE_WV_WAVES;
    probe_before(PK_FSE_ENCODE_WAVE, s);
    const dim3 grid((unsigned)((a.nBlocks + perGroup - 1) / perGroup));
    if (tt4) hipLaunchKernelGGL(k_fse_encode_wave<true>, grid, dim3(64 * FSE_WV_WAVES), ldsBytes, s, a, slotWords, tableWords);
    else     hipLaunchKernelGGL(k_fse_encode_wave<false>, grid, dim3(64 * FSE_WV_WAVES), ldsBytes, s, a, slotWords, tableWords);
    probe_after(PK_FSE_ENCODE_WAVE, s);
    return hipGetLastError();
}
```

finitestateentropy_amd/csrc/fse_tables.hip:

```cpp
#include "internal.h"

#include "wave_glue.h"
#include "ncount_reader.h"
#include "fse_wave_build.h"

template <u32 MAXC>
DEV void fse_wave_build_ctable(const WaveBuildLds& w, const int nn[4], u32 maxSV, u32 tl, u32* img, u32 lane)
{
    u16* const cumAll = w.cumP;
    *(uint2*)(w.nrm + 4 * lane) = make_uint2(((u32)nn[0] & 0xFFFFu) | ((u32)nn[1] << 16), ((u32)nn[2] & 0xFFFFu) | ((u32)nn[3] << 16));
    __syncthreads();
    const u32 ts = 1u << tl;
    u16* const stateTable = (u16*)(img + 1);
    u32* const tt = img + 1 + (ts >> 1);
    {
        u32 eff[4], laneSum = 0;
#pragma unroll
        for (int i = 0; i < 4; ++i) { eff[i] = nn[i] == -1 ? 1u : (u32)nn[i]; laneSum += eff[i]; }
        u32 total;
        u32 run = wb_scan_excl(laneSum, lane, &total);
#pragma unroll
        for (int i = 0; i < 4; ++i) {
            const u32 s = 4 * lane + i;
            cumAll[s] = (u16)run;
            if (s <= maxSV) {
                if (nn[i] == 0) { tt[2 * s] = 0; tt[2 * s + 1] = ((tl + 1) << 16) - ts; }
                else if (nn[i] == -1 || nn[i] == 1) { tt[2 * s] = run - 1u; tt[2 * s + 1] = (tl << 16) - ts; }
                else {
                    const u32 maxBitsOut = tl - hibit32((u32)nn[i] - 1);
                    tt[2 * s] = run - (u32)nn[i];
                    tt[2 * s + 1] = (maxBitsOut << 16) - ((u32)nn[i] << maxBitsOut);
                }
            }
            run += eff[i];
        }
        if (lane == 0) img[0] = tl | (maxSV << 16);
    }
    __syncthreads();
    wave_spread_rank<MAXC>(w, maxSV, tl, lane, [&](u32 s) { return (u32)cumAll[s]; },
                     [&](u32 u, u32 s, u32 r, u32 first) { (void)s; stateTable[first + r] = (u16)(ts + u); });
}

template <u32 MAXC>
__global__ __launch_bounds__(64) void k_fse_cprep(FseCPrepArgs a, u32 capTs)
{
    extern __shared__ __attribute__((aligned(16))) u8 wbLds[];
    const size_t b = blockIdx.x;
    const u32 lane = threadIdx.x;
    const size_t n = view_size(a.src, b);
    FseMeta m; m.state = 0; m.hdrSize = 0; m.tableLog = 0; m.maxSV = 0; m.pace = 0;
    const size_t top = a.histResults[b];
    size_t result = 0; bool go = false;
    if (n <= 1) result = 0;
    else if (is_err(top)) result = top;
    else if (top == n) result = 1;
    else if (top == 1 || top < (n >> 7)) result = 0;
    else go = true;
    const WaveBuildLds w = wave_build_carve(wbLds, capTs, true);
    u32* const hdrImg = w.cnt;
    u32 maxSV = 0, tl = 0;
    int nn[4] = { 0, 0, 0, 0 };
    if (go) {
        maxSV = a.maxSVs[b];
        tl = wg_optimal_tablelog(a.tableLogReq, n, maxSV, 2);
        if ((1u << tl) > 64u * MAXC || (1u << tl) > capTs) { result = FERR(tableLog_tooLarge); go = false; }
    }
    if (go) {
        const uint4 cv = ((const uint4*)(a.counts + b * 256))[lane];
        const u32 c[4] = { cv.x, cv.y, cv.z, cv.w };
        for (u32 i = lane; i < 136; i += 64) hdrImg[i] = 0;
        const size_t e = wg_normalize<64>(nn, c, (u64)n, maxSV, tl, lane);
        if (is_err(e)) { result = e; go = false; }
    }
    __syncthreads();
    if (go) {
        const size_t h = wg_write_ncount<64>(hdrImg, a.dstCapacity, nn, maxSV, tl, lane);
        if (is_err(h)) { result = h; go = false; }
        else m.hdrSize = (u32)h;
    }
    __syncthreads();
    if (!go) { if (lane == 0) { a.meta[b] = m; a.results[b] = result; } return; }
    {   u8* const dst = a.dst + b * a.dstStride;
        const u8* const hb = (const u8*)hdrImg;
        for (u32 i = lane; i < m.hdrSize; i += 64) dst[i] = hb[i];
    }
    int top1 = nn[0] > nn[1] ? nn[0] : nn[1]; top1 = nn[2] > top1 ? nn[2] : top1; top1 = nn[3] > top1 ? nn[3] : top1;
    top1 = wave_max_i32(top1);
    m.state = ((u32)top1 * 64u > (63u << tl) || n < FSE_ENC_WAVE_MIN) ? FSE_ENC_LANE : FSE_ENC_PAR;
    {
        u32 present = (nn[0] != 0) + (nn[1] != 0) + (nn[2] != 0) + (nn[3] != 0);
        present = wg_sum<64>(present);
        const u32 mix = (1u << tl) / (present ? present : 1u);
        m.pace = mix < 64u ? 0u : mix < 128u ? 1u : mix < 256u ? 2u : 3u;
    }
    m.tableLog = tl; m.maxSV = maxSV;
    if (lane == 0) a.meta[b] = m;
    fse_wave_build_ctable<MAXC>(w, nn, maxSV, tl, a.ctables + b * a.ctStrideU32, lane);
}

__global__ __launch_bounds__(64) void k_fse_dparse(FseDPrepArgs a)
{
    __shared__ __attribute__((aligned(16))) u32 stage[NCS_WORDS];
    const size_t b0 = (size_t)blockIdx.x * 64, b = b0 + threadIdx.x;
    const u32 lane = threadIdx.x;
    const bool have = b < a.nBlocks;
    const u8* const in = have ? view_ptr(a.csrc, b) : nullptr;
    const size_t cSize = have ? view_size(a.csrc, b) : 0;
    bool done = false;
    if (have && a.rawRle) { const size_t orig = a.origSizes ? a.origSizes[b] : a.uniformOrig; done = cSize == orig || cSize == 1; }
    const u32 staged = ncount_stage(stage, in, cSize, lane, have && !done);
    {   uint4* const rows = (uint4*)(a.norms + b0 * 256);
        const u32 nRows = a.nBlocks - b0 < 64 ? (u32)(a.nBlocks - b0) : 64u;
        for (u32 i = lane; i < nRows * 32u; i += 64) rows[i] = make_uint4(0, 0, 0, 0);
    }
    __syncthreads();
    int cls = -1;
    if (have) {
        FseMeta m; m.state = 0; m.hdrSize = 0; m.tableLog = 0; m.maxSV = 0; m.pace = 0; m.pace = 0;
        size_t result = 0;
        if (!done) do {
            u32 tl = 0, maxSV = 255;
            s16* const norm = a.norms + b * 256;
            const size_t h = ncount_read_staged(norm, &maxSV, &tl, stage + lane, staged, in, cSize);
            if (is_err(h)) { result = h; break; }
            if (tl > a.maxLog) { result = FERR(tableLog_tooLarge); break; }
            cls = FSE_DCLS_REV11;
            if (tl > FSE_DEC_FAST_MAXLOG) {
                int top = 0;
                for (u32 i = 0; i <= maxSV >> 3; ++i) {
                    const uint4 v = ((const uint4*)norm)[i];
                    const u32 q[4] = { v.x, v.y, v.z, v.w };
#pragma unroll
                    for (int k = 0; k < 4; ++k) { const int lo = (s16)(q[k] & 0xFFFFu), hi = (s16)(q[k] >> 16); top = lo > top ? lo : top; top = hi > top ? hi : top; }
                }
                cls = 2 * top > (1 << tl) ? FSE_DCLS_PLAIN : FSE_DCLS_REV12;
            }
            m.state = 1u | ((u32)cls << 2); m.hdrSize = (u32)h; m.tableLog = tl; m.maxSV = maxSV;
        } while (0);
        a.meta[b] = m;
        if (m.state == 0 && !done) a.results[b] = result;
    }
    if (cls >= 0) { const size_t bin = view_size(a.csrc, b) >> FSE_DBIN_LOG; cls = cls * FSE_DBINS + (int)(bin < FSE_DBINS - 1 ? bin : FSE_DBINS - 1); }
    const unsigned long long below = (1ull << lane) - 1ull;
    unsigned long long todo = __ballot(cls >= 0);
    while (todo) {
        const int leader = __builtin_ctzll(todo);
        const int c = __shfl(cls, leader, WAVE);
        const unsigned long long mask = __ballot(cls == c);
        u32 base = 0;
        if ((int)lane == leader) {
            base = atomicAdd(&a.counts[c], (u32)__builtin_popcountll(mask));
            atomicAdd(&a.counts[FSE_DCLS_COUNT + c / FSE_DBINS], (u32)__builtin_popcountll(mask));
        }
        base = (u32)__shfl((int)base, leader, WAVE);
        if (cls == c) a.lists[(size_t)c * a.nBlocks + base + (u32)__builtin_popcountll(mask & below)] = (u32)b;
        todo &= ~mask;
    }
}

template <u32 MAXC>
__global__ __launch_bounds__(64) void k_fse_dbuild(FseDPrepArgs a, u32 capTs, int firstList, int nLists, u32 ldsCapTs)
{
    extern __shared__ __attribute__((aligned(16))) u8 wbLds[];
    {   u32 total = 0;
        for (int k = firstList / (int)FSE_DBINS; k < (firstList + nLists) / (int)FSE_DBINS; ++k) total += a.counts[FSE_DCLS_COUNT + k];
        if (blockIdx.x >= total) return;
    }
    constexpr int MAXL = 2 * FSE_DBINS;
    static_assert(FSE_DBINS % 4 == 0, "the list lengths are read as 16-byte vectors");
    uint4 cv[MAXL / 4];
#pragma unroll
    for (int i = 0; i < MAXL / 4; ++i) cv[i] = 4 * i < nLists ? ((const uint4*)(a.counts + firstList))[i] : make_uint4(0, 0, 0, 0);
    u32 idx = blockIdx.x;
    int c = firstList + nLists;
    {   u32 before = 0; bool found = false;
#pragma unroll
        for (int i = 0; i < MAXL; ++i) {
            const uint4 v = cv[i >> 2];
            const u32 n = (i & 3) == 0 ? v.x : (i & 3) == 1 ? v.y : (i & 3) == 2 ? v.z : v.w;
            const bool here = !found & (i < nLists) & (idx < before + n);
            c = here ? firstList + i : c; idx = here ? idx - before : idx;
            found |= here;
            before += n;
        }
    }
    if (c == firstList + nLists) return;
    const size_t b = a.lists[(size_t)c * a.nBlocks + idx];
    const u32 lane = threadIdx.x;
    const FseMeta m = a.meta[b];
    if (m.state == 0) return;
    const u32 tl = m.tableLog, ts = 1u << tl;
    if (ts > ldsCapTs || ts > 64u * MAXC) {
        if (lane == 0) { a.meta[b].state = 0; a.results[b] = FERR(tableLog_tooLarge); }
        return;
    }
    const WaveBuildLds w = wave_build_carve(wbLds, ldsCapTs, false);
    *(uint2*)(w.nrm + 4 * lane) = *(const uint2*)(a.norms + b * 256 + 4 * lane);
    __syncthreads();
    const bool rev = ((m.state >> 2) & 3u) != FSE_DCLS_PLAIN;
    u16* const A = a.atab + b * capTs;
    u8* const S = a.symtab + b * capTs;
    const bool fast = wave_spread_rank<MAXC>(w, m.maxSV, tl, lane, [&](u32 s) { return (u32)(int)w.nrm[s]; }, [&](u32 u, u32 s, u32 r, u32 nrm) {
        const int n = (int)nrm;
        const u32 next = (n > 0 ? (u32)n : 1u) + r;
        const u32 nb = tl - hibit32(next);
        const u32 ns = (next << nb) - ts;
        const u32 x = rev ? __brev(u) >> (32u - tl) : u;
        A[x] = rev ? (u16)(nb | ((__brev(ns) >> (32u - tl)) << 5)) : (u16)((ns & 0xFFFu) | (nb << 12));
        S[x] = (u8)s;
    });
    if (lane == 0) a.meta[b].state = m.state | (fast ? 2u : 0u);
}

__global__ __launch_bounds__(256) void k_fse_export_dtable(FseDPrepArgs a, u32 capTs, u32* dtables, size_t dtStrideU32)
{
    const size_t b = blockIdx.x;
    const FseMeta m = a.meta[b];
    if (m.state == 0) return;
    const u32 tl = m.tableLog, ts = 1u << tl;
    const bool rev = ((m.state >> 2) & 3u) != FSE_DCLS_PLAIN;
    const u16* const A = a.atab + b * capTs;
    const u8* const S = a.symtab + b * capTs;
    u32* const dt = dtables + b * dtStrideU32;
    if (threadIdx.x == 0) dt[0] = tl | ((m.state & 2u) ? 1u << 16 : 0u);
    for (u32 x = threadIdx.x; x < ts; x += blockDim.x) {
        const u32 i = rev ? __brev(x) >> (32u - tl) : x;
        const u32 c = A[i];
        const u32 nb = rev ? (c & 31u) : (c >> 12);
        const u32 ns = rev ? __brev(c >> 5) >> (32u - tl) : (c & 0xFFFu);
        dt[1 + x] = ns | ((u32)S[i] << 16) | (nb << 24);
    }
}
hipError_t launch_fse_export_dtables(const FseDPrepArgs& a, u32* dtables, size_t dtStrideU32, hipStream_t s)
{
    if (a.nBlocks == 0) return hipSuccess;
    hipLaunchKernelGGL(k_fse_export_dtable, dim3((unsigned)a.nBlocks), dim3(256), 0, s, a, 1u << a.maxLog, dtables, dtStrideU32);
    return hipGetLastError();
}

DEV size_t fse_norm_load_checked(int nn[4], const s16* nb, u32 maxSV, u32 tl, u32 maxTl, u32 lane)
{
    if (maxSV > 255u) return FERR(maxSymbolValue_tooLarge);
    if (tl > maxTl) return FERR(tableLog_tooLarge);
    if (tl == 0 || tl == 1 || tl == 3) return FERR(GENERIC);
    u32 cells = 0; bool bad = false;
#pragma unroll
    for (int i = 0; i < 4; ++i) {
        nn[i] = 4 * lane + i <= maxSV ? (int)nb[4 * lane + i] : 0;
        bad |= nn[i] < -1;
        cells += nn[i] == -1 ? 1u : nn[i] > 0 ? (u32)nn[i] : 0u;
    }
    cells = wg_sum<64>(cells);
    return (wg_any<64>(bad, lane) || cells != (1u << tl)) ? FERR(GENERIC) : 0;
}
template <u32 MAXC>
__global__ __launch_bounds__(64) void k_fse_ctable_from_norm(const s16* norms, size_t normStride, const u32* maxSVs, u32 tl, u32* ctables, size_t ctStrideU32,
                                                            size_t* results, u32 capTs)
{
    extern __shared__ __attribute__((aligned(16))) u8 wbLds[];
    const size_t b = blockIdx.x;
    const u32 lane = threadIdx.x;
    const u32 maxSV = maxSVs[b];
    int nn[4] = { 0, 0, 0, 0 };
    static_assert(MAXC == 32 || MAXC == 64, "64 * MAXC cells = a table of tableLog 11 or 12");
    const size_t r = fse_norm_load_checked(nn, norms + b * normStride, maxSV, tl, MAXC == 32 ? 11u : FSE_MAX_TL, lane);
    if (lane == 0) results[b] = r;
    if (is_err(r)) return;
    fse_wave_build_ctable<MAXC>(wave_build_carve(wbLds, capTs, true), nn, maxSV, tl, ctables + b * ctStrideU32, lane);
}
hipError_t launch_fse_ctable_from_norm(const s16* norms, size_t normStride, const u32* maxSVs, u32 tl, u32* ctables, size_t ctStrideU32, size_t* results,
                                       size_t nBlocks, hipStream_t s)
{
    if (nBlocks == 0) return hipSuccess;
    const u32 capTs = 1u << (tl >= 1 && tl <= FSE_MAX_TL ? tl : FSE_MAX_TL);
    if (wb_small(capTs))
        hipLaunchKernelGGL(k_fse_ctable_from_norm<32>, dim3((unsigned)nBlocks), dim3(64), wave_build_lds_bytes(capTs, true), s, norms, normStride, maxSVs, tl, ctables,
                           ctStrideU32, results, capTs);
    else
        hipLaunchKernelGGL(k_fse_ctable_from_norm<64>, dim3((unsigned)nBlocks), dim3(64), wave_build_lds_bytes(capTs, true), s, norms, normStride, maxSVs, tl, ctables,
                           ctStrideU32, results, capTs);
    return hipGetLastError();
}

static void launch_fse_dbuild_lists(const FseDPrepArgs& a, u32 capTs, int firstList, int nLists, u32 ldsCapTs, hipStream_t s)
{
    if (wb_small(ldsCapTs))
        hipLaunchKernelGGL(k_fse_dbuild<32>, dim3((unsigned)a.nBlocks), dim3(64), wave_build_lds_bytes(ldsCapTs, false), s, a, capTs, firstList, nLists, ldsCapTs);
    else
        hipLaunchKernelGGL(k_fse_dbuild<64>, dim3((unsigned)a.nBlocks), dim3(64), wave_build_lds_bytes(ldsCapTs, false), s, a, capTs, firstList, nLists, ldsCapTs);
}
static void launch_fse_dbuilds(const FseDPrepArgs& a, hipStream_t s)
{
    const u32 capTs = 1u << a.maxLog;
    const u32 capA = a.maxLog < FSE_DEC_FAST_MAXLOG ? capTs : (1u << FSE_DEC_FAST_MAXLOG);
    launch_fse_dbuild_lists(a, capTs, (int)FSE_DCLS_REV11 * FSE_DBINS, (int)FSE_DBINS, capA, s);
    if (a.maxLog > FSE_DEC_FAST_MAXLOG) launch_fse_dbuild_lists(a, capTs, (int)FSE_DCLS_REV12 * FSE_DBINS, 2 * (int)FSE_DBINS, capTs, s);
}

__global__ __launch_bounds__(64) void k_fse_dmeta_from_norm(FseDPrepArgs a, const s16* norms, size_t normStride, const u32* maxSVs, u32 tl)
{
    const size_t b = blockIdx.x;
    const u32 lane = threadIdx.x;
    const u32 maxSV = maxSVs[b];
    int nn[4] = { 0, 0, 0, 0 };
    const size_t r = fse_norm_load_checked(nn, norms + b * normStride, maxSV, tl, a.maxLog, lane);
    FseMeta m; m.state = 0; m.hdrSize = 0; m.tableLog = tl; m.maxSV = maxSV; m.pace = 0;
    if (!is_err(r)) {
        *(uint2*)(a.norms + b * 256 + 4 * lane) = make_uint2(((u32)nn[0] & 0xFFFFu) | ((u32)nn[1] << 16), ((u32)nn[2] & 0xFFFFu) | ((u32)nn[3] << 16));
        int top = nn[0] > nn[1] ? nn[0] : nn[1]; top = nn[2] > top ? nn[2] : top; top = nn[3] > top ? nn[3] : top;
        top = wave_max_i32(top);
        const u32 cls = tl <= FSE_DEC_FAST_MAXLOG ? (u32)FSE_DCLS_REV11 : 2 * top > (1 << tl) ? (u32)FSE_DCLS_PLAIN : (u32)FSE_DCLS_REV12;
        m.state = 1u | (cls << 2);
        if (lane == 0) {
            const u32 at = atomicAdd(&a.counts[cls * FSE_DBINS], 1u);
            atomicAdd(&a.counts[FSE_DCLS_COUNT + cls], 1u);
            a.lists[(size_t)cls * FSE_DBINS * a.nBlocks + at] = (u32)b;
        }
    }
    if (lane == 0) { a.meta[b] = m; if (is_err(r)) a.results[b] = r; }
}
hipError_t launch_fse_dprep_from_norm(const FseDPrepArgs& a, const s16* norms, size_t normStride, const u32* maxSVs, u32 tl, hipStream_t s)
{
    if (a.nBlocks == 0) return hipSuccess;
    hipError_t e = launch_zero_u32(a.counts, FSE_DCLS_COUNT + FSE_DCLS_KINDS, s);
    if (e != hipSuccess) return e;
    hipLaunchKernelGGL(k_fse_dmeta_from_norm, dim3((unsigned)a.nBlocks), dim3(64), 0, s, a, norms, normStride, maxSVs, tl);
    launch_fse_dbuilds(a, s);
    return hipGetLastError();
}

#ifdef FSE_WB_TIMING
extern "C" __attribute__((visibility("default"))) int FSEHIP_debug_wbTiming(unsigned long long* host) { return (int)hipMemcpyFromSymbol(host, HIP_SYMBOL(g_wbTiming), sizeof(g_wbTiming)); }
#endif
__global__ __launch_bounds__(64) void k_fse_glue_normalize(s16* norms, size_t normStride, u32 tlReq, const u32* counts, size_t countStride,
                                                          const size_t* totals, const u32* maxSVs, size_t* results)
{
    const size_t b = blockIdx.x;
    const u32 lane = threadIdx.x;
    const u32 maxSV = maxSVs[b] > 255u ? 255u : maxSVs[b];
    const u32* const cb = counts + b * countStride;
    u32 c[4];
#pragma unroll
    for (int i = 0; i < 4; ++i) c[i] = 4 * lane + i <= maxSV ? cb[4 * lane + i] : 0u;
    int nn[4] = { 0, 0, 0, 0 };
    const u32 tl = tlReq ? tlReq : FSE_DEF_TL;
    const u64 total = (u64)totals[b];
    size_t r = total ? wg_normalize<64>(nn, c, total, maxSV, tl, lane) : FERR(GENERIC);
    if (!is_err(r)) r = tl;
    s16* const nb = norms + b * normStride;
#pragma unroll
    for (int i = 0; i < 4; ++i) if (4 * lane + i <= maxSV && !is_err(r)) nb[4 * lane + i] = (s16)nn[i];
    if (lane == 0) results[b] = r;
}

__global__ __launch_bounds__(64) void k_fse_glue_write_ncount(u8* headers, size_t headerStride, size_t headerCapacity, const s16* norms, size_t normStride,
                                                             const u32* maxSVs, u32 tl, size_t* results)
{
    __shared__ u32 img[136];
    const size_t b = blockIdx.x;
    const u32 lane = threadIdx.x;
    const u32 maxSV = maxSVs[b];
    size_t r;
    if (tl > FSE_MAX_TL) r = FERR(tableLog_tooLarge);
    else if (tl < FSE_MIN_TL || maxSV > 255u) r = FERR(GENERIC);
    else {
        const s16* const nb = norms + b * normStride;
        int nn[4];
#pragma unroll
        for (int i = 0; i < 4; ++i) nn[i] = 4 * lane + i <= maxSV ? (int)nb[4 * lane + i] : 0;
        for (u32 i = lane; i < 136; i += 64) img[i] = 0;
        __syncthreads();
        r = wg_write_ncount<64>(img, headerCapacity, nn, maxSV, tl, lane);
        __syncthreads();
        if (!is_err(r)) {
            u8* const dst = headers + b * headerStride;
            const u8* const hb = (const u8*)img;
            for (u32 i = lane; i < (u32)r; i += 64) dst[i] = hb[i];
        }
    }
    if (lane == 0) results[b] = r;
}

__global__ __launch_bounds__(64) void k_fse_glue_read_ncount(s16* norms, size_t normStride, u32* maxSVs, u32* tableLogs, BlockView headers, size_t nBlocks, size_t* results)
{
    const size_t b = (size_t)blockIdx.x * 64 + threadIdx.x;
    if (b >= nBlocks) return;
    u32 maxSV = maxSVs[b], tl = 0;
    size_t r;
    if ((size_t)maxSV >= normStride) r = FERR(maxSymbolValue_tooLarge);
    else r = ncount_read<1>(norms + b * normStride, &maxSV, &tl, view_ptr(headers, b), view_size(headers, b));
    if (!is_err(r)) { maxSVs[b] = maxSV; tableLogs[b] = tl; }
    results[b] = r;
}

hipError_t launch_fse_glue_normalize(s16* norms, size_t normStride, u32 tl, const u32* counts, size_t countStride, const size_t* totals, const u32* maxSVs,
                                     size_t* results, size_t nBlocks, hipStream_t s)
{
    if (nBlocks == 0) return hipSuccess;
    hipLaunchKernelGGL(k_fse_glue_normalize, dim3((unsigned)nBlocks), dim3(64), 0, s, norms, normStride, tl, counts, countStride, totals, maxSVs, results);
    return hipGetLastError();
}
hipError_t launch_fse_glue_write_ncount(u8* headers, size_t headerStride, size_t headerCapacity, const s16* norms, size_t normStride, const u32* maxSVs, u32 tl,
                                        size_t* results, size_t nBlocks, hipStream_t s)
{
    if (nBlocks == 0) return hipSuccess;
    hipLaunchKernelGGL(k_fse_glue_write_ncount, dim3((unsigned)nBlocks), dim3(64), 0, s, headers, headerStride, headerCapacity, norms, normStride, maxSVs, tl, results);
    return hipGetLastError();
}
hipError_t launch_fse_glue_read_ncount(s16* norms, size_t normStride, u32* maxSVs, u32* tableLogs, const BlockView& headers, size_t* results, size_t nBlocks, hipStream_t s)
{
    if (nBlocks == 0) return hipSuccess;
    hipLaunchKernelGGL(k_fse_glue_read_ncount, dim3((unsigned)((nBlocks + 63) / 64)), dim3(64), 0, s, norms, normStride, maxSVs, tableLogs, headers, nBlocks, results);
    return hipGetLastError();
}

hipError_t launch_fse_cprep(const FseCPrepArgs& a, hipStream_t s)
{
    if (a.nBlocks == 0) return hipSuccess;
    const u32 capTs = 1u << a.maxTl;
    const size_t ldsBytes = wave_build_lds_bytes(capTs, true);
    probe_before(PK_FSE_CPREP, s);
    if (wb_small(capTs)) hipLaunchKernelGGL(k_fse_cprep<32>, dim3((unsigned)a.nBlocks), dim3(64), ldsBytes, s, a, capTs);
    else hipLaunchKernelGGL(k_fse_cprep<64>, dim3((unsigned)a.nBlocks), dim3(64), ldsBytes, s, a, capTs);
    probe_after(PK_FSE_CPREP, s);
    return hipGetLastError();
}
hipError_t launch_fse_dprep(const FseDPrepArgs& a, hipStream_t s)
{
    if (a.nBlocks == 0) return hipSuccess;
    hipError_t e = launch_zero_u32(a.counts, FSE_DCLS_COUNT + FSE_DCLS_KINDS, s);
    if (e != hipSuccess) return e;
    probe_before(PK_FSE_DPREP, s);
    hipLaunchKernelGGL(k_fse_dparse, dim3((unsigned)((a.nBlocks + 63) / 64)), dim3(64), 0, s, a);
    launch_fse_dbuilds(a, s);
    probe_after(PK_FSE_DPREP, s);
    return hipGetLastError();
}
```

finitestateentropy_amd/csrc/hist.hip:

```cpp
#include "internal.h"

#define HIST_SEG (1u << 28)

#ifndef HIST_COLS_LOG
#define HIST_COLS_LOG 4
#endif
#define HIST_COLS (1u << HIST_COLS_LOG)
#ifndef HIST_GROUP
#define HIST_GROUP 4
#endif
DEV void hist_add(u32* cnt, u32 col, u32 byte)
{
    atomicAdd(&cnt[(byte << HIST_COLS_LOG) | col], 1u);
}
DEV void hist_add4(u32* cnt, u32 col, u32 w)
{
    hist_add(cnt, col, w & 0xFFu);
    hist_add(cnt, col, (w >> 8) & 0xFFu);
    hist_add(cnt, col, (w >> 16) & 0xFFu);
    hist_add(cnt, col, w >> 24);
}
DEV void hist_add16(u32* cnt, u32 col, const uint4& v)
{
    hist_add4(cnt, col, v.x); hist_add4(cnt, col, v.y); hist_add4(cnt, col, v.z); hist_add4(cnt, col, v.w);
}

__global__ __launch_bounds__(64) void k_hist(HistArgs a)
{
    __shared__ __attribute__((aligned(16))) u32 cnt[256 * HIST_COLS];
    const u32 lane = threadIdx.x;
    const u32 col = lane & (HIST_COLS - 1u);
    const size_t b = blockIdx.x;
    const u8* const p = view_ptr(a.src, b);
    const size_t n = view_size(a.src, b);
    const unsigned limitIn = (a.maxSVs && !a.useUniformIn) ? a.maxSVs[b] : a.uniformMaxSV;
    const bool checked = limitIn < 255u && !a.trustInput;
    const unsigned nOut = limitIn < 255u ? limitIn + 1u : 256u;

    u32 t0 = 0, t1 = 0, t2 = 0, t3 = 0;

    for (size_t seg = 0; seg < n; seg += HIST_SEG) {
        for (u32 i = lane; i < sizeof(cnt) / 16u; i += 64u) ((uint4*)cnt)[i] = make_uint4(0, 0, 0, 0);
        __syncthreads();
        const u8* q = p + seg;
        const size_t len = (n - seg) < (size_t)HIST_SEG ? (n - seg) : (size_t)HIST_SEG;
        size_t head = (size_t)((0 - (uintptr_t)q) & 15u);
        if (head > len) head = len;
        if (lane < head) hist_add(cnt, col, q[lane]);
        const uint4* v = (const uint4*)(q + head);
        const size_t nvec = (len - head) >> 4;
        size_t i = lane;
        constexpr size_t HG = HIST_GROUP;
        if (i + 64 * (HG - 1) < nvec) {
            uint4 x[HG];
#pragma unroll
            for (size_t g = 0; g < HG; ++g) x[g] = v[i + 64 * g];
            for (;;) {
                const size_t j = i + 64 * HG;
                const bool more = j + 64 * (HG - 1) < nvec;
                uint4 y[HG];
#pragma unroll
                for (size_t g = 0; g < HG; ++g) y[g] = x[g];
                if (more) {
#pragma unroll
                    for (size_t g = 0; g < HG; ++g) y[g] = v[j + 64 * g];
                }
                __asm__ volatile("" ::: "memory");
#pragma unroll
                for (size_t g = 0; g < HG; ++g) hist_add16(cnt, col, x[g]);
                i = j;
                if (!more) break;
#pragma unroll
                for (size_t g = 0; g < HG; ++g) x[g] = y[g];
            }
        }
        for (; i < nvec; i += 64) { const uint4 x = v[i]; hist_add16(cnt, col, x); }
        const size_t done = head + (nvec << 4);
        if (lane < len - done) hist_add(cnt, col, q[done + lane]);
        __syncthreads();
        u32 s0 = 0, s1 = 0, s2 = 0, s3 = 0;
#pragma unroll 8
        for (u32 c = 0; c < HIST_COLS; ++c) {
            const u32 cc = (c + lane) & (HIST_COLS - 1u);
            s0 += cnt[(lane << HIST_COLS_LOG) | cc]; s1 += cnt[((lane + 64u) << HIST_COLS_LOG) | cc];
            s2 += cnt[((lane + 128u) << HIST_COLS_LOG) | cc]; s3 += cnt[((lane + 192u) << HIST_COLS_LOG) | cc];
        }
        t0 += s0; t1 += s1; t2 += s2; t3 += s3;
        __syncthreads();
    }

    u32 best = t0 > t1 ? t0 : t1; best = t2 > best ? t2 : best; best = t3 > best ? t3 : best;
    int top = -1;
    if (t0) top = (int)lane;
    if (t1) top = (int)lane + 64;
    if (t2) top = (int)lane + 128;
    if (t3) top = (int)lane + 192;
    best = wave_max_u32(best);
    top = wave_max_i32(top);

    if (n == 0) {
        for (u32 s = lane; s < nOut; s += 64) a.counts[b * 256 + s] = 0;
        if (lane == 0) { if (a.maxSVs) a.maxSVs[b] = 0; a.results[b] = 0; }
        return;
    }
    if (checked && (unsigned)top > limitIn) {
        if (lane == 0) a.results[b] = FERR(maxSymbolValue_tooSmall);
        return;
    }
    unsigned* out = a.counts + b * 256;
    if (lane < nOut) out[lane] = t0;
    if (lane + 64 < nOut) out[lane + 64] = t1;
    if (lane + 128 < nOut) out[lane + 128] = t2;
    if (lane + 192 < nOut) out[lane + 192] = t3;
    if (lane == 0) { if (a.maxSVs) a.maxSVs[b] = (unsigned)top; a.results[b] = (size_t)best; }
}

__global__ __launch_bounds__(1024) void k_hist_fold(const unsigned* __restrict__ part, size_t nPart, unsigned limitIn, int checked, size_t n,
                                                   unsigned* count, unsigned* maxSV, size_t* result)
{
    __shared__ u32 sums[4][256];
    __shared__ u32 wbest[4];
    __shared__ int wtop[4];
    const u32 t = threadIdx.x, sym = t & 255u, q = t >> 8;
    u32 acc = 0;
    for (size_t p = q; p < nPart; p += 4) acc += part[p * 256 + sym];
    sums[q][sym] = acc;
    __syncthreads();
    if (t >= 256) return;
    const u32 c = sums[0][t] + sums[1][t] + sums[2][t] + sums[3][t];
    const u32 best = wave_max_u32(c);
    const int top = wave_max_i32(c ? (int)t : -1);
    if ((t & 63u) == 0) { wbest[t >> 6] = best; wtop[t >> 6] = top; }
    __syncthreads();
    u32 b = wbest[0]; int tp = wtop[0];
    for (int w = 1; w < 4; ++w) { b = wbest[w] > b ? wbest[w] : b; tp = wtop[w] > tp ? wtop[w] : tp; }
    const unsigned nOut = limitIn < 255u ? limitIn + 1u : 256u;
    if (checked && (unsigned)tp > limitIn) { if (t == 0) *result = FERR(maxSymbolValue_tooSmall); return; }
    (void)n;
    if (t < nOut) count[t] = c;
    if (t == 0) { *maxSV = (unsigned)tp; *result = (size_t)b; }
}

hipError_t launch_hist_large(const u8* d_src, size_t n, unsigned limitIn, int trustInput, unsigned* d_part, unsigned* d_count, unsigned* d_maxSV,
                             size_t* d_result, size_t* d_scratchResults, hipStream_t s)
{
    const size_t nFull = n / HIST_PIECE, tail = n % HIST_PIECE, nPart = nFull + (tail ? 1 : 0);
    HistArgs a;
    a.counts = d_part; a.maxSVs = nullptr; a.uniformMaxSV = 255; a.useUniformIn = 1; a.trustInput = 1; a.results = d_scratchResults;
    a.src = BlockView{d_src, HIST_PIECE, nullptr, HIST_PIECE, nullptr}; a.nBlocks = nFull;
    hipError_t e = launch_hist(a, s);
    if (e != hipSuccess) return e;
    if (tail) {
        a.counts = d_part + nFull * 256; a.results = d_scratchResults + nFull;
        a.src = BlockView{d_src + nFull * HIST_PIECE, tail, nullptr, tail, nullptr}; a.nBlocks = 1;
        e = launch_hist(a, s);
        if (e != hipSuccess) return e;
    }
    hipLaunchKernelGGL(k_hist_fold, dim3(1), dim3(1024), 0, s, (const unsigned*)d_part, nPart, limitIn, (int)(limitIn < 255u && !trustInput), n,
                       d_count, d_maxSV, d_result);
    return hipGetLastError();
}

__global__ __launch_bounds__(64) void k_zero_u32(u32* p, u32 n)
{
    for (u32 i = blockIdx.x * 64u + threadIdx.x; i < n; i += gridDim.x * 64u) p[i] = 0;
}
hipError_t launch_zero_u32(u32* p, u32 n, hipStream_t s)
{
    if (n == 0) return hipSuccess;
    const u32 groups = (n + 63u) / 64u;
    hipLaunchKernelGGL(k_zero_u32, dim3(groups < 1024u ? groups : 1024u), dim3(64), 0, s, p, n);
    return hipGetLastError();
}

hipError_t launch_hist(const HistArgs& a, hipStream_t s)
{
    if (a.nBlocks == 0) return hipSuccess;
    probe_before(PK_HIST, s);
    hipLaunchKernelGGL(k_hist, dim3((unsigned)a.nBlocks), dim3(64), 0, s, a);
    probe_after(PK_HIST, s);
    return hipGetLastError();
}
```

finitestateentropy_amd/csrc/internal.h:

```cpp
#pragma once
#include "dev_common.h"

#define CK(x) do { hipError_t e__ = (x); if (e__ != hipSuccess) return (int)e__; } while (0)
static inline size_t align_up(size_t v, size_t a) { return (v + a - 1) / a * a; }

static inline BlockView mkview(const void* base, size_t stride, const size_t* sizes, size_t uniform)
{
    BlockView v; v.base = (const u8*)base; v.stride = stride; v.sizes = sizes; v.uniform = uniform; v.offsets = nullptr; return v;
}
static inline BlockView subview(const BlockView& v, size_t b0)
{
    BlockView r = v;
    if (v.offsets) r.offsets = v.offsets + b0; else r.base = v.base + b0 * v.stride;
    r.sizes = v.sizes ? v.sizes + b0 : nullptr;
    return r;
}

struct HistArgs {
    unsigned* counts;
    unsigned* maxSVs;
    unsigned uniformMaxSV;
    int useUniformIn;
    int trustInput = 0;
    size_t* results;
    BlockView src;
    size_t nBlocks;
};
hipError_t launch_hist(const HistArgs& a, hipStream_t s);
#define HIST_PIECE ((size_t)65536)
#define HIST_LARGE_MIN ((size_t)262144)
hipError_t launch_hist_large(const u8* d_src, size_t n, unsigned limitIn, int trustInput, unsigned* d_part, unsigned* d_count, unsigned* d_maxSV,
                             size_t* d_result, size_t* d_scratchResults, hipStream_t s);
hipError_t launch_zero_u32(u32* p, u32 n, hipStream_t s);

struct FseMeta {
    u32 state;
    u32 hdrSize;
    u32 tableLog;
    u32 maxSV;
    u32 pace;
};

struct FseCPrepArgs {
    const unsigned* counts;
    const unsigned* maxSVs;
    const size_t* histResults;
    BlockView src;
    u8* dst; size_t dstStride; size_t dstCapacity;
    unsigned maxSVReq, tableLogReq;
    u32* ctables; size_t ctStrideU32;
    unsigned maxTl;
    FseMeta* meta;
    size_t* results;
    size_t nBlocks;
};
hipError_t launch_fse_cprep(const FseCPrepArgs& a, hipStream_t s);
hipError_t launch_fse_glue_normalize(s16* norms, size_t normStride, u32 tl, const u32* counts, size_t countStride, const size_t* totals, const u32* maxSVs,
                                     size_t* results, size_t nBlocks, hipStream_t s);
hipError_t launch_fse_glue_write_ncount(u8* headers, size_t headerStride, size_t headerCapacity, const s16* norms, size_t normStride, const u32* maxSVs, u32 tl,
                                        size_t* results, size_t nBlocks, hipStream_t s);
hipError_t launch_fse_glue_read_ncount(s16* norms, size_t normStride, u32* maxSVs, u32* tableLogs, const BlockView& headers, size_t* results, size_t nBlocks, hipStream_t s);
hipError_t launch_fse_ctable_from_norm(const s16* norms, size_t normStride, const u32* maxSVs, u32 tl, u32* ctables, size_t ctStrideU32, size_t* results,
                                       size_t nBlocks, hipStream_t s);

struct FseEncArgs {
    u8* dst; size_t dstStride; size_t dstCapacity;
    size_t* results;
    BlockView src;
    const u32* ctables; size_t ctStrideU32;
    const FseMeta* meta;
    unsigned maxTableLog;
    int G;
    unsigned slotU32;
    size_t nBlocks;
    unsigned onlyState;
    unsigned sizeSplit;
    u32* list; u32* count;
};
enum { FSE_EBINS = 4 };
enum { FSE_ENC_PAR = 1, FSE_ENC_LANE = 2 };
#define FSE_ENC_WAVE_MIN 2048u
__host__ __device__ inline bool fse_enc_skip(unsigned state, unsigned onlyState) { return state == 0 || (onlyState != 0 && state != onlyState); }
hipError_t launch_fse_encode(FseEncArgs a, hipStream_t s);
size_t fse_encode_blocks_per_round(unsigned maxTableLog);
hipError_t launch_fse_encode_wave(FseEncArgs a, hipStream_t s);
hipError_t launch_fse_enc_lists(const FseEncArgs& a, hipStream_t s);
inline hipError_t launch_fse_encode_auto(FseEncArgs a, hipStream_t s)
{
    a.onlyState = 0; a.sizeSplit = 0;
    const bool ragged = a.src.sizes || a.src.offsets;
    if (a.dstCapacity > 0x7FFFFFF0u || (!ragged && a.src.uniform < FSE_ENC_WAVE_MIN)) return launch_fse_encode(a, s);
    if (!a.meta) {
        a.list = nullptr; a.count = nullptr;
        if (!ragged) return launch_fse_encode_wave(a, s);
        a.sizeSplit = 1;
        const hipError_t e = launch_fse_encode_wave(a, s);
        return e != hipSuccess ? e : launch_fse_encode(a, s);
    }
    a.onlyState = FSE_ENC_PAR;
    hipError_t e = a.list ? launch_fse_enc_lists(a, s) : hipSuccess;
    if (e == hipSuccess) e = launch_fse_encode_wave(a, s);
    if (e != hipSuccess) return e;
    a.onlyState = FSE_ENC_LANE;
    return launch_fse_encode(a, s);
}

#ifndef FSE_DBINS_N
#define FSE_DBINS_N 16
#define FSE_DBIN_LOG 11
#endif
enum { FSE_DCLS_REV11 = 0, FSE_DCLS_REV12 = 1, FSE_DCLS_PLAIN = 2, FSE_DCLS_KINDS = 3, FSE_DBINS = FSE_DBINS_N, FSE_DCLS_COUNT = FSE_DCLS_KINDS * FSE_DBINS };
struct FseDPrepArgs {
    BlockView csrc;
    unsigned maxLog;
    u16* atab;
    u8* symtab;
    s16* norms;
    FseMeta* meta;
    u32* lists;
    u32* counts;
    size_t* results;
    size_t nBlocks;
    int rawRle; const size_t* origSizes; size_t uniformOrig;
};
hipError_t launch_fse_dprep(const FseDPrepArgs& a, hipStream_t s);
hipError_t launch_fse_dprep_from_norm(const FseDPrepArgs& a, const s16* norms, size_t normStride, const u32* maxSVs, u32 tl, hipStream_t s);

struct FseDecArgs {
    u8* dst; size_t dstStride; size_t dstCapacity;
    size_t* results;
    BlockView csrc;
    const u32* dtables; size_t dtStrideU32;
    const u16* atab; const u8* symtab;
    const FseMeta* meta;
    unsigned maxTableLog;
    unsigned ldsLog;
    const u32* list;
    const u32* count;
    int G;
    unsigned slotU32;
    size_t nBlocks;
    unsigned tlMin; int declineNb0; int onlyDeclined;
    u8* symScratch; u32* slotBitmap; u32 nSlots; u32 scratchSlotBytes;
    const u64* dstOffsets = nullptr; const size_t* dstCaps = nullptr;
};
#define FSE_DECLINED ((size_t)0 - (size_t)0x7001)
#define FSE_DEC_FAST_MAXLOG 11u
hipError_t launch_fse_decode(FseDecArgs a, hipStream_t s);
hipError_t launch_fse_decode_classes(FseDecArgs a, const u32* lists, const u32* counts, hipStream_t s);
size_t fse_decode_blocks_per_round(unsigned maxTableLog);

struct HufMeta {
    u32 state;
    u32 hdrSize;
    u32 tableLog;
    u32 maxSV;
};

struct HufCPrepArgs {
    const unsigned* counts; const unsigned* maxSVs; const size_t* histResults;
    BlockView src;
    u8* dst; size_t dstStride; size_t dstCapacity;
    unsigned maxSVReq, huffLogReq;
    u32* ctables; size_t ctStrideU32;
    HufMeta* meta;
    size_t* results;
    size_t nBlocks;
};
hipError_t launch_huf_cprep(const HufCPrepArgs& a, hipStream_t s, void* nodeScratch );
hipError_t launch_huf_cprep_glue(const HufCPrepArgs& a, int mode , hipStream_t s);

struct HufEncArgs {
    u8* dst; size_t dstStride; size_t dstCapacity;
    size_t* results;
    BlockView src;
    const u32* ctables; size_t ctStrideU32;
    const HufMeta* meta;
    int streams;
    int split1X;
    size_t nBlocks;
};
hipError_t launch_huf_encode(const HufEncArgs& a, hipStream_t s);

enum { HUF_DKIND_PAR_TINY = 0, HUF_DKIND_PAR_SMALL = 1, HUF_DKIND_PAR_LARGE = 2, HUF_DKIND_SERIAL = 3, HUF_DCLS_COUNT = 8 };
#ifndef HPAR_ALL_SMALL
#define HPAR_ALL_SMALL 1
#endif
#ifndef HPAR_USE_TINY
#define HPAR_USE_TINY 0
#endif
#define HPAR_DATA_TINY  2304u
#ifndef HPAR_DATA_SMALL
#define HPAR_DATA_SMALL 4608u
#endif
#define HPAR_DATA_LARGE (8192u + 384u)
#define HPAR_MIN_BITS 4096u
struct HufDPrepArgs {
    BlockView csrc;
    BlockView dstSizes;
    u8* dst; size_t dstStride;
    u32* dtables; size_t dtStrideU32;
    HufMeta* meta;
    u32* lists;
    u32* counts;
    size_t* results;
    size_t nBlocks;
    const u64* dstOffsets = nullptr;
    int tableOnly;
    unsigned dtMaxLog;
};
hipError_t launch_huf_dprep(const HufDPrepArgs& a, hipStream_t s);
hipError_t launch_huf_dprep_x2(const HufDPrepArgs& a, hipStream_t s);
hipError_t launch_hdr_results(const void* meta, size_t metaStride, size_t* results, size_t nBlocks, hipStream_t s);
hipError_t launch_fse_export_dtables(const FseDPrepArgs& a, u32* dtables, size_t dtStrideU32, hipStream_t s);

struct HufDecArgs {
    u8* dst; size_t dstStride;
    BlockView dstSizes;
    size_t* results;
    BlockView csrc;
    const u32* dtables; size_t dtStrideU32;
    const HufMeta* meta;
    unsigned maxTableLog;
    unsigned ldsLog;
    const u32* list;
    const u32* count;
    int G; unsigned slotU32;
    int streams;
    int acceptX2;
    int onlyDeclined;
    unsigned classLo;
    size_t nBlocks;
    const u64* dstOffsets = nullptr;
};
#define HUF_DECLINED ((size_t)0 - (size_t)0x7000)
hipError_t launch_huf_decode(HufDecArgs a, hipStream_t s);
hipError_t launch_huf_decode_classes(HufDecArgs a, u32* lists, u32* counts, hipStream_t s);
hipError_t launch_huf_decode_par(HufDecArgs a, unsigned dataBytes, u32* serialList, u32* serialCount, hipStream_t s);
hipError_t launch_huf_decode_par_x2(HufDecArgs a, hipStream_t s);

struct U16Meta { u32 state, hdrSize, tableLog, maxSV; };
struct U16CArgs {
    const u16* src; size_t srcStrideBytes; const size_t* srcSizes; size_t uniformSrcSize;
    u8* dst; size_t dstStride; size_t dstCapacity;
    u32 maxSVReq, tableLogReq;
    u16* stateTables; u32* symTT; U16Meta* meta;
    unsigned* countsOut; unsigned* maxSVOut;
    size_t* results; size_t nBlocks;
};
struct U16DArgs {
    u16* dst; size_t dstStrideBytes; size_t dstCapacity;
    const u8* csrc; size_t cStride; const size_t* cSizes; size_t uniformCSize;
    u32* cells; U16Meta* meta;
    size_t* results; size_t nBlocks;
};
hipError_t launch_u16_compress(const U16CArgs& a, hipStream_t s);
hipError_t launch_u16_decompress(const U16DArgs& a, hipStream_t s);
hipError_t launch_u16_decode_lds(const U16DArgs& a, hipStream_t s);

hipError_t launch_probagen(u8* dst, size_t dstStride, size_t blockSize, size_t nBlocks, const u8* d_table, u32 firstSeed, u32 seedStep, hipStream_t s);

hipError_t launch_compact(u8* packed, size_t packedCapacity, u64* offsets, const u8* slots, size_t slotStride, const size_t* results, const BlockView& src,
                          size_t nBlocks, u64* partials, hipStream_t s);
hipError_t launch_rawrle_expand(u8* dst, size_t dstStride, size_t dstCapacity, size_t* results, const BlockView& csrc, const size_t* origSizes, size_t uniformOrig,
                                size_t nBlocks, hipStream_t s);

#define PLANES_TILE ((u64)32768)
void launch_planes_offsets(u64* planeOff, size_t* tensorRes, const u64* srcOff, size_t nTensors, unsigned E, u64 capacity, hipStream_t s);
void launch_planes_verdicts(size_t* results, const u64* dstOff, const size_t* planeSizes, size_t nTensors, unsigned E, u64 dstCapacity, hipStream_t s);
hipError_t launch_planes_split(u8* planes, u64* planeOff, size_t* tensorRes, const u8* src, const u64* srcOff, size_t nTensors, unsigned E, u64 capacity, hipStream_t s);
hipError_t launch_planes_merge(u8* dst, const u64* dstOff, size_t* results, const u8* planes, const u64* planeOff, const size_t* planeSizes, size_t nTensors, unsigned E,
                               u64 dstCapacity, hipStream_t s);

enum { PK_HIST = 0, PK_FSE_CPREP, PK_FSE_ENCODE, PK_FSE_DPREP, PK_FSE_DECODE, PK_HUF_CPREP, PK_HUF_ENCODE, PK_HUF_DPREP, PK_HUF_DECODE, PK_FSE_ENCODE_WAVE, PK_COUNT };
void probe_before(int kernelId, hipStream_t s);
void probe_after(int kernelId, hipStream_t s);

struct HostCallBuf {
    void* p = nullptr;
    hipError_t alloc(size_t n);
    ~HostCallBuf();
    HostCallBuf() = default;
    HostCallBuf(const HostCallBuf&) = delete; HostCallBuf& operator=(const HostCallBuf&) = delete;
private:
    size_t carved = 0; bool owned = false;
};
#define FSEHIP_SCRATCH_MAX ((size_t)1 << 30)

struct DevProps { int cus; int ldsPerCU; bool ok; };
const DevProps& dev_props();
hipError_t ensure_dyn_lds(const void* kernel, int bytes);
int fse_compress_view(void* d_dst, size_t dstStride, size_t dstCapacity, size_t* d_results, const BlockView& src, unsigned maxSymbolValue, unsigned tableLog,
                      size_t nBlocks, void* d_workspace, size_t workspaceBytes, hipStream_t s);
int huf_compress_view(int streams, void* d_dst, size_t dstStride, size_t dstCapacity, size_t* d_results, const BlockView& src, unsigned maxSymbolValue,
                      unsigned tableLog, size_t nBlocks, void* d_workspace, size_t workspaceBytes, hipStream_t s);
int fse_decompress_view(void* d_dst, const u64* d_dstOffsets, const size_t* d_dstCaps, size_t* d_results, const BlockView& csrc, unsigned maxLog, size_t nBlocks,
                        void* d_workspace, size_t workspaceBytes, hipStream_t s);
int huf_decompress_view(void* d_dst, const u64* d_dstOffsets, const size_t* d_dstSizes, size_t* d_results, const BlockView& csrc, size_t nBlocks,
                        void* d_workspace, size_t workspaceBytes, hipStream_t s);
int huf_compress_batch_impl(int streams, void* d_dst, size_t dstStride, size_t dstCapacity, size_t* d_results,
                            const void* d_src, size_t srcStride, const size_t* d_sizes, size_t uniformSize,
                            unsigned maxSymbolValue, unsigned tableLog, size_t nBlocks, void* d_workspace, size_t workspaceBytes, void* stream);
int batch_arg_error(size_t* d_results, const size_t* d_sizes, size_t uniform, size_t dstCapacity, size_t nBlocks, size_t code, int mode, hipStream_t s);
hipError_t launch_xxh32(u32* hashes, const u8* data, const u64* starts, const u64* lens, size_t nItems, u32 seed, hipStream_t s);
int release_thread_scratch(void);
int frame_pool_release_scratch(void);
int frame_pool_shutdown(void);
```

include/fsehip.h:

```cpp
#ifndef FSEHIP_H
#define FSEHIP_H

#include <stddef.h>
#include <stdint.h>

#ifdef __cplusplus
extern "C" {
#endif

#define FSEHIP_API __attribute__((visibility("default")))

typedef enum {
    FSEHIP_error_no_error = 0,
    FSEHIP_error_GENERIC = 1,
    FSEHIP_error_dstSize_tooSmall = 2,
    FSEHIP_error_srcSize_wrong = 3,
    FSEHIP_error_corruption_detected = 4,
    FSEHIP_error_tableLog_tooLarge = 5,
    FSEHIP_error_maxSymbolValue_tooLarge = 6,
    FSEHIP_error_maxSymbolValue_tooSmall = 7,
    FSEHIP_error_workSpace_tooSmall = 8,
    FSEHIP_error_maxCode = 9
} FSEHIP_ErrorCode;
#define FSEHIP_ERROR(name) ((size_t)0 - (size_t)FSEHIP_error_##name)
// ... 155 lines not shown
                                            unsigned maxSymbolValue, unsigned tableLog, size_t nBlocks, void* d_workspace, size_t workspaceBytes, void* stream);
FSEHIP_API size_t FSEHIP_FSE_buildDTable_batch_workspaceSize(size_t nBlocks, unsigned maxLog);
FSEHIP_API int FSEHIP_FSE_buildDTable_batch(FSEHIP_FSE_DTable* d_dtables, size_t dtableStrideU32, size_t* d_results,
                                            const void* d_headers, size_t headerStride, const size_t* d_headerSizes, size_t uniformHeaderSize,
                                            unsigned maxLog, size_t nBlocks, void* d_workspace, size_t workspaceBytes, void* stream);
FSEHIP_API size_t FSEHIP_HUF_buildCTable_batch_workspaceSize(size_t nBlocks);
FSEHIP_API int FSEHIP_HUF_buildCTable_batch(FSEHIP_HUF_CElt* d_ctables, size_t ctableStrideU32, void* d_headers, size_t headerStride, size_t headerCapacity,
                                            size_t* d_results, const void* d_src, size_t srcStride, const size_t* d_sizes, size_t uniformSize,
                                            unsigned maxSymbolValue, unsigned tableLog, size_t nBlocks, void* d_workspace, size_t workspaceBytes, void* stream);
FSEHIP_API int FSEHIP_HUF_buildCTable_fromCount_batch(FSEHIP_HUF_CElt* d_ctables, size_t ctableStrideU32, const unsigned* d_counts, size_t countStride,
                                                      const unsigned* d_maxSymbolValues, unsigned maxNbBits, size_t nBlocks, size_t* d_results, void* stream);
FSEHIP_API int FSEHIP_HUF_writeCTable_batch(void* d_headers, size_t headerStride, size_t headerCapacity, const FSEHIP_HUF_CElt* d_ctables, size_t ctableStrideU32,
                                            const unsigned* d_maxSymbolValues, unsigned huffLog, size_t nBlocks, size_t* d_results, void* stream);
FSEHIP_API size_t FSEHIP_HUF_readDTableX1_batch_workspaceSize(size_t nBlocks);
FSEHIP_API int FSEHIP_HUF_readDTableX1_batch(FSEHIP_HUF_DTable* d_dtables, size_t dtableStrideU32, unsigned maxTableLog, size_t* d_results,
                                             const void* d_src, size_t srcStride, const size_t* d_srcSizes, size_t uniformSrcSize,
                                             size_t nBlocks, void* d_workspace, size_t workspaceBytes, void* stream);
FSEHIP_API size_t FSEHIP_HUF_readDTableX2_batch_workspaceSize(size_t nBlocks);
FSEHIP_API int FSEHIP_HUF_readDTableX2_batch(FSEHIP_HUF_DTable* d_dtables, size_t dtableStrideU32, unsigned maxTableLog, size_t* d_results,
                                             const void* d_src, size_t srcStride, const size_t* d_srcSizes, size_t uniformSrcSize,
                                             size_t nBlocks, void* d_workspace, size_t workspaceBytes, void* stream);

FSEHIP_API int FSEHIP_FSE_normalizeCount_batch(short* d_norms, size_t normStride, unsigned tableLog, const unsigned* d_counts, size_t countStride,
                                               const size_t* d_totals, const unsigned* d_maxSymbolValues, size_t nBlocks, size_t* d_results, void* stream);
FSEHIP_API int FSEHIP_FSE_writeNCount_batch(void* d_headers, size_t headerStride, size_t headerCapacity, const short* d_norms, size_t normStride,
                                            const unsigned* d_maxSymbolValues, unsigned tableLog, size_t nBlocks, size_t* d_results, void* stream);
FSEHIP_API int FSEHIP_FSE_readNCount_batch(short* d_norms, size_t normStride, unsigned* d_maxSymbolValues, unsigned* d_tableLogs,
                                           const void* d_headers, size_t headerStride, const size_t* d_headerSizes, size_t uniformHeaderSize,
                                           size_t nBlocks, size_t* d_results, void* stream);
FSEHIP_API int FSEHIP_FSE_buildCTable_fromNorm_batch(FSEHIP_FSE_CTable* d_ctables, size_t ctableStrideU32, const short* d_norms, size_t normStride,
                                                     const unsigned* d_maxSymbolValues, unsigned tableLog, size_t nBlocks, size_t* d_results, void* stream);
FSEHIP_API size_t FSEHIP_FSE_buildDTable_fromNorm_batch_workspaceSize(size_t nBlocks, unsigned tableLog);
FSEHIP_API int FSEHIP_FSE_buildDTable_fromNorm_batch(FSEHIP_FSE_DTable* d_dtables, size_t dtableStrideU32, const short* d_norms, size_t normStride,
                                                     const unsigned* d_maxSymbolValues, unsigned tableLog, size_t nBlocks, size_t* d_results,
                                                     void* d_workspace, size_t workspaceBytes, void* stream);

FSEHIP_API size_t FSEHIP_compact_batch_workspaceSize(size_t nBlocks);
FSEHIP_API size_t FSEHIP_compact_batch_bound(size_t nBlocks, size_t blockSize);
FSEHIP_API int FSEHIP_compact_batch(void* d_packed, size_t packedCapacity, uint64_t* d_offsets, const void* d_slots, size_t slotStride, const size_t* d_results,
                                    const void* d_src, size_t srcStride, const size_t* d_srcSizes, size_t uniformSrcSize, size_t nBlocks,
                                    void* d_workspace, size_t workspaceBytes, void* stream);
FSEHIP_API int FSEHIP_FSE_decompress_packed_batch(void* d_dst, size_t dstStride, size_t dstCapacity, size_t* d_results,
                                                  const void* d_packed, const uint64_t* d_offsets, const size_t* d_origSizes, size_t uniformOrigSize,
                                                  unsigned maxLog, size_t nBlocks, void* d_workspace, size_t workspaceBytes, void* stream);
FSEHIP_API int FSEHIP_HUF_decompress_packed_batch(void* d_dst, size_t dstStride, const size_t* d_dstSizes, size_t uniformDstSize, size_t* d_results,
                                                  const void* d_packed, const uint64_t* d_offsets, size_t nBlocks, void* d_workspace, size_t workspaceBytes, void* stream);

FSEHIP_API void FSEHIP_probagen_table(uint8_t table4096[4096], double p);
FSEHIP_API int FSEHIP_probagen_batch(void* d_dst, size_t dstStride, size_t blockSize, size_t nBlocks,
                                     const uint8_t h_table4096[4096], uint32_t firstSeed, void* stream);
FSEHIP_API int FSEHIP_probagen_batch_ex(void* d_dst, size_t dstStride, size_t blockSize, size_t nBlocks,
                                        const uint8_t h_table4096[4096], uint32_t firstSeed, uint32_t seedStep, void* stream);

FSEHIP_API size_t FSEHIP_frame_compressBound(size_t srcSize, unsigned blockSizeId);
FSEHIP_API size_t FSEHIP_frame_compress(void* dst, size_t dstCapacity, const void* src, size_t srcSize, unsigned blockSizeId, int codec);
FSEHIP_API size_t FSEHIP_frame_decompress(void* dst, size_t dstCapacity, const void* src, size_t srcSize);
FSEHIP_API size_t FSEHIP_frame_compress_batch(void* const* dsts, const size_t* dstCapacities, const void* const* srcs, const size_t* srcSizes,
                                              size_t* results, size_t nFrames, unsigned blockSizeId, int codec, unsigned nThreads);
FSEHIP_API size_t FSEHIP_frame_decompress_batch(void* const* dsts, const size_t* dstCapacities, const void* const* srcs, const size_t* srcSizes,
                                                size_t* results, size_t nFrames, unsigned nThreads);

typedef struct {
    uint64_t contentBound;
    uint64_t nBlocks;
    uint32_t status;
    uint32_t checksum22;
    uint8_t  codec;
    uint8_t  blockSizeId;
    uint8_t  reserved[6];
} FSEHIP_FrameInfo;
FSEHIP_API int FSEHIP_XXH32_batch(uint32_t* d_hashes, const void* d_data, const uint64_t* d_offsets, size_t nItems, uint32_t seed, void* stream);
FSEHIP_API size_t FSEHIP_frame_blockCount(size_t srcSize, unsigned blockSizeId);
FSEHIP_API size_t FSEHIP_frame_compress_dbatch_workspaceSize(size_t nFrames, size_t maxTotalBlocks, unsigned blockSizeId, int codec);
FSEHIP_API int FSEHIP_frame_compress_dbatch(void* d_dst, const uint64_t* d_dstOffsets, size_t* d_results, const void* d_src, const uint64_t* d_srcOffsets,
                                            size_t nFrames, size_t maxTotalBlocks, unsigned blockSizeId, int codec,
                                            void* d_workspace, size_t workspaceBytes, void* stream);
FSEHIP_API size_t FSEHIP_frame_packedBound(size_t totalSrcBytes, size_t nFrames, size_t totalBlocks, unsigned slotAlignLog);
FSEHIP_API size_t FSEHIP_frame_compress_packed_dbatch_workspaceSize(size_t nFrames, size_t maxTotalBlocks, unsigned blockSizeId, int codec);
FSEHIP_API int FSEHIP_frame_compress_packed_dbatch(void* d_dst, uint64_t dstCapacity, uint64_t* d_dstOffsets, size_t* d_results,
                                                   const void* d_src, const uint64_t* d_srcOffsets, size_t nFrames, size_t maxTotalBlocks,
                                                   unsigned blockSizeId, int codec, unsigned slotAlignLog,
                                                   void* d_workspace, size_t workspaceBytes, void* stream);
#define FSEHIP_CODECS_GIVEN  0
#define FSEHIP_CODECS_CHOOSE 1
FSEHIP_API size_t FSEHIP_frame_mixedWorkspaceBound(size_t nFrames, size_t maxTotalBlocks, unsigned blockSizeId, int policy);
FSEHIP_API int FSEHIP_frame_compress_packed_mixed_dbatch(void* d_dst, uint64_t dstCapacity, uint64_t* d_dstOffsets, size_t* d_results,
                                                         const void* d_src, const uint64_t* d_srcOffsets, size_t nFrames, size_t maxTotalBlocks,
                                                         unsigned blockSizeId, uint8_t* d_codecs, int policy, unsigned tolerancePermille,
                                                         unsigned slotAlignLog, void* d_workspace, size_t workspaceBytes, void* stream);
FSEHIP_API size_t FSEHIP_frame_decompress_dbatch_workspaceSize(size_t nFrames, size_t maxTotalBlocks);
FSEHIP_API int FSEHIP_frame_decompress_dbatch(void* d_dst, const uint64_t* d_dstOffsets, size_t* d_results, const void* d_frames, const uint64_t* d_frameOffsets,
                                              size_t nFrames, size_t maxTotalBlocks, void* d_workspace, size_t workspaceBytes, void* stream);
FSEHIP_API size_t FSEHIP_frame_inspect(FSEHIP_FrameInfo* info, const void* src, size_t srcSize);
FSEHIP_API size_t FSEHIP_frame_plan_dbatch_workspaceSize(size_t nFrames);
FSEHIP_API int FSEHIP_frame_plan_dbatch(uint64_t* d_dstOffsets, uint64_t* d_blockFirst, FSEHIP_FrameInfo* d_infos, const void* d_frames, const uint64_t* d_frameOffsets,
                                        size_t nFrames, uint64_t dstCapacity, unsigned slotAlignLog, void* d_workspace, size_t workspaceBytes, void* stream);
FSEHIP_API size_t FSEHIP_frame_decompress_packed_dbatch_workspaceSize(size_t nFrames, size_t maxTotalBlocks);
FSEHIP_API int FSEHIP_frame_decompress_packed_dbatch(void* d_dst, size_t dstCapacity, uint64_t* d_dstOffsets, size_t* d_results, const void* d_frames,
                                                     const uint64_t* d_frameOffsets, size_t nFrames, size_t maxTotalBlocks, unsigned slotAlignLog,
                                                     void* d_workspace, size_t workspaceBytes, void* stream);

FSEHIP_API size_t FSEHIP_planes_blockBound(size_t totalBytes, size_t nTensors, unsigned elemBytes, unsigned blockSizeId);
FSEHIP_API int FSEHIP_planes_split_dbatch(void* d_planes, uint64_t* d_planeOffsets, size_t* d_tensorResults, const void* d_src, const uint64_t* d_srcOffsets,
                                          size_t nTensors, unsigned elemBytes, uint64_t capacity, void* stream);
FSEHIP_API int FSEHIP_planes_merge_dbatch(void* d_dst, const uint64_t* d_dstOffsets, size_t* d_results, const void* d_planes, const uint64_t* d_planeOffsets,
                                          const size_t* d_planeSizes, size_t nTensors, unsigned elemBytes, uint64_t dstCapacity, void* stream);
FSEHIP_API int FSEHIP_tensor_compress_dbatch(void* d_dst, uint64_t dstCapacity, uint64_t* d_frameOffsets, size_t* d_frameResults, size_t* d_tensorResults,
                                             const void* d_src, const uint64_t* d_srcOffsets, size_t nTensors, unsigned elemBytes, uint64_t capacity,
                                             size_t maxTotalBlocks, unsigned blockSizeId, int codec, unsigned slotAlignLog,
                                             void* d_planes, uint64_t* d_planeOffsets, void* d_workspace, size_t workspaceBytes, void* stream);
FSEHIP_API int FSEHIP_tensor_decompress_dbatch(void* d_dst, const uint64_t* d_dstOffsets, uint64_t dstCapacity, size_t* d_results,
                                               const void* d_frames, const uint64_t* d_frameOffsets, size_t nTensors, unsigned elemBytes, size_t maxTotalBlocks,
                                               void* d_planes, uint64_t planesCapacity, uint64_t* d_planeOffsets, size_t* d_planeResults,
                                               void* d_workspace, size_t workspaceBytes, void* stream);

FSEHIP_API int FSEHIP_planes_split_xor_dbatch(void* d_planes, uint64_t* d_planeOffsets, size_t* d_tensorResults, const void* d_src, const void* d_base,
                                              const uint64_t* d_srcOffsets, size_t nTensors, unsigned elemBytes, uint64_t capacity, void* stream);
FSEHIP_API int FSEHIP_planes_merge_xor_dbatch(void* d_dst, const uint64_t* d_dstOffsets, size_t* d_results, const void* d_planes, const uint64_t* d_planeOffsets,
                                              const size_t* d_planeSizes, const void* d_base, size_t nTensors, unsigned elemBytes, uint64_t dstCapacity, void* stream);
FSEHIP_API int FSEHIP_tensor_compress_delta_dbatch(void* d_dst, uint64_t dstCapacity, uint64_t* d_frameOffsets, size_t* d_frameResults, size_t* d_tensorResults,
                                                   const void* d_src, const void* d_base, const uint64_t* d_srcOffsets, size_t nTensors, unsigned elemBytes,
                                                   uint64_t capacity, size_t maxTotalBlocks, unsigned blockSizeId, int codec, unsigned slotAlignLog,
                                                   void* d_planes, uint64_t* d_planeOffsets, void* d_workspace, size_t workspaceBytes, void* stream);
FSEHIP_API int FSEHIP_tensor_compress_mixed_dbatch(void* d_dst, uint64_t dstCapacity, uint64_t* d_frameOffsets, size_t* d_frameResults, size_t* d_tensorResults,
                                                   const void* d_src, const void* d_base, const uint64_t* d_srcOffsets, size_t nTensors, unsigned elemBytes,
                                                   uint64_t capacity, size_t maxTotalBlocks, unsigned blockSizeId, uint8_t* d_codecs, int policy,
                                                   unsigned tolerancePermille, unsigned slotAlignLog, void* d_planes, uint64_t* d_planeOffsets,
                                                   void* d_workspace, size_t workspaceBytes, void* stream);
FSEHIP_API int FSEHIP_tensor_decompress_delta_dbatch(void* d_dst, const uint64_t* d_dstOffsets, uint64_t dstCapacity, const void* d_base, size_t* d_results,
                                                     const void* d_frames, const uint64_t* d_frameOffsets, size_t nTensors, unsigned elemBytes, size_t maxTotalBlocks,
                                                     void* d_planes, uint64_t planesCapacity, uint64_t* d_planeOffsets, size_t* d_planeResults,
                                                     void* d_workspace, size_t workspaceBytes, void* stream);

#define FSEHIP_FSEU16_MAX_SYMBOL_VALUE 286
#define FSEHIP_FSEU16_MAX_TABLELOG 13
#define FSEHIP_FSEU16_DEFAULT_TABLELOG 12
FSEHIP_API size_t FSEHIP_FSE_countU16(unsigned* count, unsigned* maxSymbolValuePtr, const unsigned short* src, size_t srcSize);
FSEHIP_API size_t FSEHIP_FSE_compressU16(void* dst, size_t dstCapacity, const unsigned short* src, size_t srcSize, unsigned maxSymbolValue, unsigned tableLog);
FSEHIP_API size_t FSEHIP_FSE_decompressU16(unsigned short* dst, size_t dstCapacity, const void* cSrc, size_t cSrcSize);
FSEHIP_API size_t FSEHIP_FSE_compressU16_batch_workspaceSize(size_t nBlocks);
FSEHIP_API size_t FSEHIP_FSE_decompressU16_batch_workspaceSize(size_t nBlocks);
FSEHIP_API int FSEHIP_FSE_countU16_batch(unsigned* d_counts, unsigned* d_maxSymbolValues, size_t* d_results, const unsigned short* d_src, size_t srcStrideBytes,
                                         const size_t* d_srcSizes, size_t uniformSrcSize, unsigned maxSymbolValue, size_t nBlocks, void* stream);
FSEHIP_API int FSEHIP_FSE_compressU16_batch(void* d_dst, size_t dstStride, size_t dstCapacity, size_t* d_results, const unsigned short* d_src, size_t srcStrideBytes,
                                            const size_t* d_srcSizes, size_t uniformSrcSize, unsigned maxSymbolValue, unsigned tableLog, size_t nBlocks,
                                            void* d_workspace, size_t workspaceBytes, void* stream);
FSEHIP_API int FSEHIP_FSE_decompressU16_batch(unsigned short* d_dst, size_t dstStrideBytes, size_t dstCapacity, size_t* d_results, const void* d_cSrc, size_t cStride,
                                              const size_t* d_cSizes, size_t uniformCSize, size_t nBlocks, void* d_workspace, size_t workspaceBytes, void* stream);

#ifdef FSEHIP_INTERNAL
FSEHIP_API int FSEHIP_probe_begin(void);
FSEHIP_API int FSEHIP_probe_collect(double* totalMs16, unsigned* launches16);
FSEHIP_API int FSEHIP_debug_decodeTiming(int enable, unsigned long long* out16);
#endif

FSEHIP_API void FSEHIP_shardRange(size_t nBlocks, int rank, int world, size_t* first, size_t* count);

#define FSEHIP_SCRATCH_BUSY (-2)
FSEHIP_API int FSEHIP_releaseScratch(void);
FSEHIP_API int FSEHIP_shutdown(void);

FSEHIP_API int FSEHIP_prepareDevice(void);

typedef struct { int deviceOrdinal; int computeUnits; int ldsBytesPerCU; int wavefrontSize; char archName[64]; } FSEHIP_DeviceInfo;
FSEHIP_API int FSEHIP_deviceInfo(FSEHIP_DeviceInfo* info);
FSEHIP_API const char* FSEHIP_versionString(void);

#ifdef FSEHIP_DROPIN_NAMES
#define HIST_count FSEHIP_HIST_count
#define FSE_compress FSEHIP_FSE_compress
#define FSE_compress2 FSEHIP_FSE_compress2
#define FSE_decompress FSEHIP_FSE_decompress
#define FSE_compress_usingCTable FSEHIP_FSE_compress_usingCTable
#define FSE_decompress_usingDTable FSEHIP_FSE_decompress_usingDTable
#define HUF_compress FSEHIP_HUF_compress
#define HUF_compress2 FSEHIP_HUF_compress2
#define HUF_decompress FSEHIP_HUF_decompress
#define HUF_compress1X_usingCTable FSEHIP_HUF_compress1X_usingCTable
#define HUF_compress4X_usingCTable FSEHIP_HUF_compress4X_usingCTable
#define HUF_decompress4X_usingDTable FSEHIP_HUF_decompress4X_usingDTable
#define HUF_decompress4X1_usingDTable FSEHIP_HUF_decompress4X1_usingDTable
#define HUF_decompress1X_usingDTable FSEHIP_HUF_decompress1X_usingDTable
#define HUF_decompress1X1_usingDTable FSEHIP_HUF_decompress1X1_usingDTable
#define HIST_count_wksp FSEHIP_HIST_count_wksp
#define HIST_countFast FSEHIP_HIST_countFast
#define HIST_countFast_wksp FSEHIP_HIST_countFast_wksp
#define HIST_count_simple FSEHIP_HIST_count_simple
#define FSE_compress_wksp FSEHIP_FSE_compress_wksp
#define FSE_decompress_wksp FSEHIP_FSE_decompress_wksp
#define HUF_compress4X_wksp FSEHIP_HUF_compress4X_wksp
#define HUF_compress1X_wksp FSEHIP_HUF_compress1X_wksp
#define HUF_compress1X FSEHIP_HUF_compress1X
#define HUF_decompress4X1_DCtx_wksp FSEHIP_HUF_decompress4X1_DCtx_wksp
#endif
#ifdef FSEHIP_DROPIN_GLUE_NAMES
#define FSE_optimalTableLog FSEHIP_FSE_optimalTableLog
#define FSE_normalizeCount FSEHIP_FSE_normalizeCount
#define FSE_NCountWriteBound FSEHIP_FSE_NCountWriteBound
#define FSE_writeNCount FSEHIP_FSE_writeNCount
#define FSE_readNCount FSEHIP_FSE_readNCount
#define FSE_buildCTable FSEHIP_FSE_buildCTable
#define FSE_buildCTable_wksp FSEHIP_FSE_buildCTable_wksp
#define FSE_buildDTable FSEHIP_FSE_buildDTable
#define HUF_buildCTable FSEHIP_HUF_buildCTable
#define HUF_buildCTable_wksp FSEHIP_HUF_buildCTable_wksp
#define HUF_writeCTable FSEHIP_HUF_writeCTable
#define HUF_readDTableX1 FSEHIP_HUF_readDTableX1
#define HUF_readDTableX1_wksp FSEHIP_HUF_readDTableX1_wksp
#define HUF_decompress4X1 FSEHIP_HUF_decompress4X1
#define HUF_decompress4X1_DCtx FSEHIP_HUF_decompress4X1_DCtx
#define HUF_decompress1X1 FSEHIP_HUF_decompress1X1
#define HUF_decompress1X1_DCtx FSEHIP_HUF_decompress1X1_DCtx
#define HUF_decompress1X1_DCtx_wksp FSEHIP_HUF_decompress1X1_DCtx_wksp
#define HUF_readDTableX2 FSEHIP_HUF_readDTableX2
#define HUF_readDTableX2_wksp FSEHIP_HUF_readDTableX2_wksp
#define HUF_decompress4X2 FSEHIP_HUF_decompress4X2
#define HUF_decompress4X2_DCtx FSEHIP_HUF_decompress4X2_DCtx
#define HUF_decompress4X2_DCtx_wksp FSEHIP_HUF_decompress4X2_DCtx_wksp
#define HUF_decompress1X2 FSEHIP_HUF_decompress1X2
#define HUF_decompress1X2_DCtx FSEHIP_HUF_decompress1X2_DCtx
#define HUF_decompress1X2_DCtx_wksp FSEHIP_HUF_decompress1X2_DCtx_wksp
#define HUF_decompress4X2_usingDTable FSEHIP_HUF_decompress4X2_usingDTable
#define HUF_decompress1X2_usingDTable FSEHIP_HUF_decompress1X2_usingDTable
#endif
#ifdef FSEHIP_DROPIN_U16_NAMES
#define FSE_countU16 FSEHIP_FSE_countU16
#define FSE_compressU16 FSEHIP_FSE_compressU16
#define FSE_decompressU16 FSEHIP_FSE_decompressU16
#endif

#ifdef __cplusplus
}
#endif
#endif
```

Baseline: 205,900 MiB/s of uncompressed data through encode+decode (whole job).

## Use persistent bounded grids for FSE decode, lane encode and table build kernels

Converts the decode kernel (non-REV11 classes), the per-lane encode kernel and the 64-wide decode table builder into grid-stride loops, launching them with a grid capped at a per-CU multiple of the CU count instead of one workgroup per block group. It also folds the clearing of the encode list counters into the histogram kernel, which removes a separate zeroing launch. The aim is to cut workgroup launch and scheduling overhead and the extra tiny kernel. The cost is less dynamic load balancing across workgroups, extra __syncthreads between iterations, and a debug override for the grid cap.

After: 206,800 MiB/s of uncompressed data through encode+decode (whole job), median of 6. No clear change (+0.4%).

```diff
diff --git a/finitestateentropy_amd/_lib.py b/finitestateentropy_amd/_lib.py
--- a/finitestateentropy_amd/_lib.py
+++ b/finitestateentropy_amd/_lib.py
@@ -29,4 +29,6 @@
             raise OSError("libfsehip.so is missing (%s): build it with finitestateentropy_amd.build_library(); "
                           "there is no CPU fallback" % path)
         _LIB = ctypes.CDLL(path)
+        _LIB.FSEHIP_debug_gridCap.argtypes = [ctypes.c_uint]
+        _LIB.FSEHIP_debug_gridCap.restype = ctypes.c_int
     return _LIB
diff --git a/finitestateentropy_amd/csrc/capi.hip b/finitestateentropy_amd/csrc/capi.hip
--- a/finitestateentropy_amd/csrc/capi.hip
+++ b/finitestateentropy_amd/csrc/capi.hip
@@ -59,6 +59,17 @@
     }
     return p;
 }
+#include <atomic>
+namespace { std::atomic<unsigned> g_gridCapOverride{0}; }
+unsigned grid_cap(unsigned perCU)
+{
+    const unsigned o = g_gridCapOverride.load(std::memory_order_relaxed);
+    if (o) return o;
+    const DevProps& p = dev_props();
+    return perCU * (unsigned)(p.ok && p.cus > 0 ? p.cus : 256);
+}
+extern "C" __attribute__((visibility("default"))) int FSEHIP_debug_gridCap(unsigned cap) { g_gridCapOverride.store(cap, std::memory_order_relaxed); return 0; }
+
 hipError_t ensure_dyn_lds(const void* kernel, int bytes)
 {
     int dev = 0;
diff --git a/finitestateentropy_amd/csrc/capi_batch.hip b/finitestateentropy_amd/csrc/capi_batch.hip
--- a/finitestateentropy_amd/csrc/capi_batch.hip
+++ b/finitestateentropy_amd/csrc/capi_batch.hip
@@ -137,7 +137,9 @@
     for (size_t b0 = 0; b0 < nBlocks; b0 += chunk) {
         const size_t nb = pass_blocks(nBlocks, b0, chunk);
         const BlockView src = subview(srcAll, b0);
-        CK(launch_hist(ws.cb.hist_args(msv, src, nb), s));
+        HistArgs h = ws.cb.hist_args(msv, src, nb);
+        h.encCounts = ws.encCounts;
+        CK(launch_hist(h, s));
         FseCPrepArgs c;
         c.counts = ws.cb.counts; c.maxSVs = ws.cb.maxSVs; c.histResults = ws.cb.hres; c.src = src;
         c.dst = (u8*)d_dst + b0 * dstStride; c.dstStride = dstStride; c.dstCapacity = dstCapacity;
@@ -148,7 +150,7 @@
         FseEncArgs e;
         e.dst = (u8*)d_dst + b0 * dstStride; e.dstStride = dstStride; e.dstCapacity = dstCapacity; e.results = d_results + b0;
         e.src = src; e.ctables = ws.ctables; e.ctStrideU32 = w.ctU32; e.meta = ws.cb.meta;
-        e.maxTableLog = w.maxTl; e.G = 0; e.slotU32 = 0; e.nBlocks = nb; e.list = ws.encLists; e.count = ws.encCounts;
+        e.maxTableLog = w.maxTl; e.G = 0; e.slotU32 = 0; e.nBlocks = nb; e.list = ws.encLists; e.count = ws.encCounts; e.countCleared = 1;
         CK(launch_fse_encode_auto(e, s));
     }
     return 0;
diff --git a/finitestateentropy_amd/csrc/fse_decode.hip b/finitestateentropy_amd/csrc/fse_decode.hip
--- a/finitestateentropy_amd/csrc/fse_decode.hip
+++ b/finitestateentropy_amd/csrc/fse_decode.hip
@@ -346,22 +346,33 @@
     }
 }
 
-template <bool FAST, bool TIMED, bool CALLER, bool VIEW = false>
+template <bool FAST, bool TIMED, bool CALLER, bool VIEW = false, bool LOOP = false>
 __global__ __launch_bounds__(FSE_DEC_THREADS) void k_fse_decode(FseDecArgs a)
 {
+    static_assert(!LOOP || (!CALLER && !TIMED), "the looping form is the one-shot path's: no symbol-scratch slot to hand back, no cycle accounting");
     extern __shared__ __attribute__((aligned(16))) u32 lds[];
     const int tid = threadIdx.x, lane = tid & 63, wave = tid >> 6;
     unsigned long long tBorn = 0, wBorn = 0;
     (void)tBorn; (void)wBorn;
     TIMING(tBorn = __builtin_readcyclecounter(); wBorn = wall_clock64(););
-    const size_t first = (size_t)blockIdx.x * a.G;
     static_assert(FSE_DBINS % 4 == 0, "the bin lengths are read as 16-byte vectors");
+    uint4 cvEntry[FSE_DBINS / 4];
+    if constexpr (LOOP) {
+#pragma unroll
+        for (u32 i = 0; i < FSE_DBINS / 4; ++i) cvEntry[i] = ((const uint4*)a.count)[i];
+    }
+    for (size_t wg = blockIdx.x;; wg += gridDim.x) {
+    if (LOOP && wg != blockIdx.x) {
+        __syncthreads();
+        __builtin_amdgcn_s_setprio(0);
+    }
+    const size_t first = wg * (size_t)a.G;
     size_t nTot = a.nBlocks, q0 = first;
     u32 bin0 = 0, cnt0 = 0xFFFFFFFFu;
     if (a.count) {
         uint4 cv[FSE_DBINS / 4];
 #pragma unroll
-        for (u32 i = 0; i < FSE_DBINS / 4; ++i) cv[i] = ((const uint4*)a.count)[i];
+        for (u32 i = 0; i < FSE_DBINS / 4; ++i) { if constexpr (LOOP) cv[i] = cvEntry[i]; else cv[i] = ((const uint4*)a.count)[i]; }
         u64 before = 0;
         bool found = false;
 #pragma unroll
@@ -394,6 +405,7 @@
 
     u32* const flagsSh = (u32*)(ldsb + (size_t)a.G * slotBytes);
     if (tid < 6 || tid == 7) flagsSh[tid] = 0;
+    if (LOOP && tid >= 32 && tid < 64) flagsSh[tid] = 0;
     const bool decWave = wave < FSE_DEC_WAVES;
     u8* const tlSh = (u8*)(flagsSh + 8);
     if (CALLER) {
@@ -620,7 +632,10 @@
         ctl->inLo = (u32)ib; ctl->inHi = (u32)(ib >> 32); ctl->outLo = (u32)ob; ctl->outHi = (u32)(ob >> 32); ctl->symLo = (u32)tb; ctl->symHi = (u32)(tb >> 32);
     }
     __syncthreads();
-    if (!decWave) { fse_decode_service<TIMED, CALLER>(a, ldsb, ctlAll, slotBytes, ringOff, inOff, lane, (wave - FSE_DEC_WAVES) * FSE_SRV_G, FAST, flagsSh); return; }
+    if (!decWave) {
+        fse_decode_service<TIMED, CALLER>(a, ldsb, ctlAll, slotBytes, ringOff, inOff, lane, (wave - FSE_DEC_WAVES) * FSE_SRV_G, FAST, flagsSh);
+        if constexpr (LOOP) continue; else return;
+    }
 
     __builtin_amdgcn_s_setprio(3);
     uint2* const myRing = (uint2*)(ldsb + (size_t)(gsl < a.G ? gsl : 0) * slotBytes + ringOff) + half;
@@ -743,6 +758,8 @@
                             atomicAdd(&g_decTiming[14], tE - tBulk1); });
     }
     if (CALLER) fse_scratch_slot_done(a, flagsSh, lane);
+    if constexpr (!LOOP) return;
+    }
 }
 
 static void fse_decode_geometry(unsigned ldsLog, size_t ldsBytes, unsigned* slotU32, int* G)
@@ -795,7 +812,7 @@
     return hipSuccess;
 }
 
-static hipError_t fse_decode_launch(FseDecArgs a, bool rev, hipStream_t s)
+static hipError_t fse_decode_launch(FseDecArgs a, bool rev, hipStream_t s, bool loop = false)
 {
     const size_t ldsBytes = FSE_DEC_LDS;
     const bool caller = a.atab == nullptr;
@@ -810,12 +827,28 @@
     fse_decode_geometry(a.ldsLog, ldsBytes, &a.slotU32, &a.G);
     if (a.G < 1) return hipErrorInvalidValue;
     if (caller && ((size_t)a.G << a.ldsLog) > FSE_SYM_SLOT_BYTES) return hipErrorInvalidValue;
-    const size_t groups = (a.nBlocks + a.G - 1) / a.G;
+    size_t groups = (a.nBlocks + a.G - 1) / a.G;
+    if (loop && (caller || !a.count || !a.list)) return hipErrorInvalidValue;
+    if (loop && rev && g_decTimingOn.load(std::memory_order_relaxed)) loop = false;
+    if (loop) {
+        const size_t cap = grid_cap(FSE_WGS_PER_CU);
+        groups = groups < cap ? groups : cap;
+        hipError_t e = ensure_dyn_lds((const void*)k_fse_decode<true, false, false, false, true>, FSE_DEC_LDS);
+        if (e == hipSuccess) e = ensure_dyn_lds((const void*)k_fse_decode<false, false, false, false, true>, FSE_DEC_LDS);
+        if (e != hipSuccess) return e;
+    }
     if (a.dstOffsets) {
         if (caller || !a.dstCaps) return hipErrorInvalidValue;
         hipError_t e = ensure_dyn_lds((const void*)k_fse_decode<true, false, false, true>, FSE_DEC_LDS);
         if (e == hipSuccess) e = ensure_dyn_lds((const void*)k_fse_decode<false, false, false, true>, FSE_DEC_LDS);
+        if (e == hipSuccess && loop) e = ensure_dyn_lds((const void*)k_fse_decode<true, false, false, true, true>, FSE_DEC_LDS);
+        if (e == hipSuccess && loop) e = ensure_dyn_lds((const void*)k_fse_decode<false, false, false, true, true>, FSE_DEC_LDS);
         if (e != hipSuccess) return e;
+        if (loop) {
+            if (rev) hipLaunchKernelGGL((k_fse_decode<true, false, false, true, true>), dim3((unsigned)groups), dim3(FSE_DEC_THREADS), ldsBytes, s, a);
+            else     hipLaunchKernelGGL((k_fse_decode<false, false, false, true, true>), dim3((unsigned)groups), dim3(FSE_DEC_THREADS), ldsBytes, s, a);
+            return hipGetLastError();
+        }
         if (rev) hipLaunchKernelGGL((k_fse_decode<true, false, false, true>), dim3((unsigned)groups), dim3(FSE_DEC_THREADS), ldsBytes, s, a);
         else     hipLaunchKernelGGL((k_fse_decode<false, false, false, true>), dim3((unsigned)groups), dim3(FSE_DEC_THREADS), ldsBytes, s, a);
         return hipGetLastError();
@@ -829,6 +862,8 @@
         else if (rev) hipLaunchKernelGGL((k_fse_decode<true, false, true>), dim3((unsigned)groups), dim3(FSE_DEC_THREADS), ldsBytes, s, a);
         else     hipLaunchKernelGGL((k_fse_decode<false, false, true>), dim3((unsigned)groups), dim3(FSE_DEC_THREADS), ldsBytes, s, a);
     }
+    else if (loop && rev) hipLaunchKernelGGL((k_fse_decode<true, false, false, false, true>), dim3((unsigned)groups), dim3(FSE_DEC_THREADS), ldsBytes, s, a);
+    else if (loop)        hipLaunchKernelGGL((k_fse_decode<false, false, false, false, true>), dim3((unsigned)groups), dim3(FSE_DEC_THREADS), ldsBytes, s, a);
     else if (rev && g_decTimingOn.load(std::memory_order_relaxed)) hipLaunchKernelGGL((k_fse_decode<true, true, false>), dim3((unsigned)groups), dim3(FSE_DEC_THREADS), ldsBytes, s, a);
     else if (rev) hipLaunchKernelGGL((k_fse_decode<true, false, false>), dim3((unsigned)groups), dim3(FSE_DEC_THREADS), ldsBytes, s, a);
     else          hipLaunchKernelGGL((k_fse_decode<false, false, false>), dim3((unsigned)groups), dim3(FSE_DEC_THREADS), ldsBytes, s, a);
@@ -890,7 +925,7 @@
         if (c != FSE_DCLS_REV11 && a.maxTableLog <= FSE_DEC_FAST_MAXLOG) break;
         a.list = lists + (size_t)c * FSE_DBINS * a.nBlocks; a.count = counts + c * FSE_DBINS;
         a.ldsLog = c == FSE_DCLS_REV11 ? (a.maxTableLog < FSE_DEC_FAST_MAXLOG ? a.maxTableLog : FSE_DEC_FAST_MAXLOG) : a.maxTableLog;
-        e = fse_decode_launch(a, c != FSE_DCLS_PLAIN, s);
+        e = fse_decode_launch(a, c != FSE_DCLS_PLAIN, s, c != FSE_DCLS_REV11);
     }
     probe_after(PK_FSE_DECODE, s);
     return e;
diff --git a/finitestateentropy_amd/csrc/fse_encode.hip b/finitestateentropy_amd/csrc/fse_encode.hip
--- a/finitestateentropy_amd/csrc/fse_encode.hip
+++ b/finitestateentropy_amd/csrc/fse_encode.hip
@@ -7,39 +7,9 @@
         (x) = *(const u16*)(ldsb + ((((x) >> nb) << 1) + f2));                                       \
     }
 
-__global__ __launch_bounds__(64) void k_fse_encode(FseEncArgs a)
+DEV void fse_encode_lane(const FseEncArgs& a, const u32* lds, size_t first, u32 lane)
 {
-    extern __shared__ __attribute__((aligned(16))) u32 lds[];
     const u8* const ldsb = (const u8*)lds;
-    const u32 lane = threadIdx.x;
-    const size_t first = (size_t)blockIdx.x * a.G;
-
-    if (a.meta) {
-        const size_t bb = first + lane;
-        const bool mine = lane < (u32)a.G && bb < a.nBlocks && !fse_enc_skip(a.meta[bb].state, a.onlyState);
-        if (!__any(mine)) return;
-    }
-
-    for (int g = 0; g < a.G; ++g) {
-        const size_t b = first + g;
-        if (b >= a.nBlocks) break;
-        if (a.meta && fse_enc_skip(a.meta[b].state, a.onlyState)) continue;
-        if (a.sizeSplit && view_size(a.src, b) >= FSE_ENC_WAVE_MIN) continue;
-        const u32* t = a.ctables + b * a.ctStrideU32;
-        const u32 h = t[0];
-        const u32 tl = h & 0xFFFFu, msv = (h >> 16) > 255u ? 255u : (h >> 16);
-        if (tl > a.maxTableLog) continue;
-        const u32 ttStart = 1 + (tl ? (1u << (tl - 1)) : 1u);
-        const u32 words = ttStart + 2 * (msv + 1);
-        u32* s = lds + (size_t)g * a.slotU32;
-        const u32 stOff = (u32)(g * a.slotU32 + 1) * 4u;
-        for (u32 i = lane; i < words; i += 64) {
-            u32 v = t[i];
-            if (i >= ttStart && (((i - ttStart) & 1u) == 0)) v = 2u * v + stOff;
-            s[i] = v;
-        }
-    }
-    __syncthreads();
     if (lane >= (u32)a.G) return;
     const size_t b = first + lane;
     if (b >= a.nBlocks) return;
@@ -135,6 +105,42 @@
     } else a.results[b] = csize;
 }
 
+__global__ __launch_bounds__(64) void k_fse_encode(FseEncArgs a)
+{
+    extern __shared__ __attribute__((aligned(16))) u32 lds[];
+    const u32 lane = threadIdx.x;
+    for (size_t first = (size_t)blockIdx.x * a.G; first < a.nBlocks; first += (size_t)gridDim.x * a.G) {
+        if (a.meta) {
+            const size_t bb = first + lane;
+            const bool mine = lane < (u32)a.G && bb < a.nBlocks && !fse_enc_skip(a.meta[bb].state, a.onlyState);
+            if (!__any(mine)) continue;
+        }
+
+        for (int g = 0; g < a.G; ++g) {
+            const size_t b = first + g;
+            if (b >= a.nBlocks) break;
+            if (a.meta && fse_enc_skip(a.meta[b].state, a.onlyState)) continue;
+            if (a.sizeSplit && view_size(a.src, b) >= FSE_ENC_WAVE_MIN) continue;
+            const u32* t = a.ctables + b * a.ctStrideU32;
+            const u32 h = t[0];
+            const u32 tl = h & 0xFFFFu, msv = (h >> 16) > 255u ? 255u : (h >> 16);
+            if (tl > a.maxTableLog) continue;
+            const u32 ttStart = 1 + (tl ? (1u << (tl - 1)) : 1u);
+            const u32 words = ttStart + 2 * (msv + 1);
+            u32* s = lds + (size_t)g * a.slotU32;
+            const u32 stOff = (u32)(g * a.slotU32 + 1) * 4u;
+            for (u32 i = lane; i < words; i += 64) {
+                u32 v = t[i];
+                if (i >= ttStart && (((i - ttStart) & 1u) == 0)) v = 2u * v + stOff;
+                s[i] = v;
+            }
+        }
+        __syncthreads();
+        fse_encode_lane(a, lds, first, lane);
+        __syncthreads();
+    }
+}
+
 #define FSE_ENC_LDS (80 * 1024)
 static void fse_encode_geometry(unsigned maxTableLog, unsigned* slotU32, int* G)
 {
@@ -151,7 +157,7 @@
     return (size_t)G * 2 * cus;
 }
 
-hipError_t launch_fse_encode(FseEncArgs a, hipStream_t s)
+hipError_t launch_fse_encode(FseEncArgs a, hipStream_t s, bool boundedGrid)
 {
     if (a.nBlocks == 0) return hipSuccess;
     const size_t ldsBytes = FSE_ENC_LDS;
@@ -159,7 +165,8 @@
     fse_encode_geometry(a.maxTableLog, &a.slotU32, &a.G);
     if (a.nBlocks > 1 && ((a.src.stride > 0x3FFFFFFu) || (a.dstStride > 0x3FFFFFFu))) a.G = 1;
     if (a.dstCapacity > 0x7FFFFFF0u) a.dstCapacity = 0x7FFFFFF0u;
-    const size_t groups = (a.nBlocks + a.G - 1) / a.G;
+    size_t groups = (a.nBlocks + a.G - 1) / a.G;
+    if (boundedGrid) { const size_t cap = grid_cap(2); groups = groups < cap ? groups : cap; }
     probe_before(PK_FSE_ENCODE, s);
     hipLaunchKernelGGL(k_fse_encode, dim3((unsigned)groups), dim3(64), ldsBytes, s, a);
     probe_after(PK_FSE_ENCODE, s);
diff --git a/finitestateentropy_amd/csrc/fse_encode_wave.hip b/finitestateentropy_amd/csrc/fse_encode_wave.hip
--- a/finitestateentropy_amd/csrc/fse_encode_wave.hip
+++ b/finitestateentropy_amd/csrc/fse_encode_wave.hip
@@ -460,8 +460,10 @@
 hipError_t launch_fse_enc_lists(const FseEncArgs& a, hipStream_t s)
 {
     if (a.nBlocks == 0) return hipSuccess;
-    const hipError_t e = launch_zero_u32(a.count, FSE_EBINS, s);
-    if (e != hipSuccess) return e;
+    if (!a.countCleared) {
+        const hipError_t e = launch_zero_u32(a.count, FSE_EBINS, s);
+        if (e != hipSuccess) return e;
+    }
     hipLaunchKernelGGL(k_fse_enc_lists, dim3((unsigned)((a.nBlocks + 63) / 64)), dim3(64), 0, s, a);
     return hipGetLastError();
 }
diff --git a/finitestateentropy_amd/csrc/fse_tables.hip b/finitestateentropy_amd/csrc/fse_tables.hip
--- a/finitestateentropy_amd/csrc/fse_tables.hip
+++ b/finitestateentropy_amd/csrc/fse_tables.hip
@@ -162,54 +162,58 @@
 __global__ __launch_bounds__(64) void k_fse_dbuild(FseDPrepArgs a, u32 capTs, int firstList, int nLists, u32 ldsCapTs)
 {
     extern __shared__ __attribute__((aligned(16))) u8 wbLds[];
-    {   u32 total = 0;
-        for (int k = firstList / (int)FSE_DBINS; k < (firstList + nLists) / (int)FSE_DBINS; ++k) total += a.counts[FSE_DCLS_COUNT + k];
-        if (blockIdx.x >= total) return;
-    }
+    constexpr bool STRIDE = MAXC == 64;
+    u32 total = 0;
+    for (int k = firstList / (int)FSE_DBINS; k < (firstList + nLists) / (int)FSE_DBINS; ++k) total += a.counts[FSE_DCLS_COUNT + k];
+    if (blockIdx.x >= total) return;
     constexpr int MAXL = 2 * FSE_DBINS;
     static_assert(FSE_DBINS % 4 == 0, "the list lengths are read as 16-byte vectors");
     uint4 cv[MAXL / 4];
 #pragma unroll
     for (int i = 0; i < MAXL / 4; ++i) cv[i] = 4 * i < nLists ? ((const uint4*)(a.counts + firstList))[i] : make_uint4(0, 0, 0, 0);
-    u32 idx = blockIdx.x;
-    int c = firstList + nLists;
-    {   u32 before = 0; bool found = false;
-#pragma unroll
-        for (int i = 0; i < MAXL; ++i) {
-            const uint4 v = cv[i >> 2];
-            const u32 n = (i & 3) == 0 ? v.x : (i & 3) == 1 ? v.y : (i & 3) == 2 ? v.z : v.w;
-            const bool here = !found & (i < nLists) & (idx < before + n);
-            c = here ? firstList + i : c; idx = here ? idx - before : idx;
-            found |= here;
-            before += n;
-        }
-    }
-    if (c == firstList + nLists) return;
-    const size_t b = a.lists[(size_t)c * a.nBlocks + idx];
-    const u32 lane = threadIdx.x;
-    const FseMeta m = a.meta[b];
-    if (m.state == 0) return;
-    const u32 tl = m.tableLog, ts = 1u << tl;
-    if (ts > ldsCapTs || ts > 64u * MAXC) {
-        if (lane == 0) { a.meta[b].state = 0; a.results[b] = FERR(tableLog_tooLarge); }
-        return;
-    }
-    const WaveBuildLds w = wave_build_carve(wbLds, ldsCapTs, false);
-    *(uint2*)(w.nrm + 4 * lane) = *(const uint2*)(a.norms + b * 256 + 4 * lane);
-    __syncthreads();
-    const bool rev = ((m.state >> 2) & 3u) != FSE_DCLS_PLAIN;
-    u16* const A = a.atab + b * capTs;
-    u8* const S = a.symtab + b * capTs;
-    const bool fast = wave_spread_rank<MAXC>(w, m.maxSV, tl, lane, [&](u32 s) { return (u32)(int)w.nrm[s]; }, [&](u32 u, u32 s, u32 r, u32 nrm) {
-        const int n = (int)nrm;
-        const u32 next = (n > 0 ? (u32)n : 1u) + r;
-        const u32 nb = tl - hibit32(next);
-        const u32 ns = (next << nb) - ts;
-        const u32 x = rev ? __brev(u) >> (32u - tl) : u;
-        A[x] = rev ? (u16)(nb | ((__brev(ns) >> (32u - tl)) << 5)) : (u16)((ns & 0xFFFu) | (nb << 12));
-        S[x] = (u8)s;
-    });
-    if (lane == 0) a.meta[b].state = m.state | (fast ? 2u : 0u);
+    u32 pos = blockIdx.x;
+    do {
+        if (STRIDE && pos != blockIdx.x) __syncthreads();
+        u32 idx = pos;
+        int c = firstList + nLists;
+        {   u32 before = 0; bool found = false;
+#pragma unroll
+            for (int i = 0; i < MAXL; ++i) {
+                const uint4 v = cv[i >> 2];
+                const u32 n = (i & 3) == 0 ? v.x : (i & 3) == 1 ? v.y : (i & 3) == 2 ? v.z : v.w;
+                const bool here = !found & (i < nLists) & (idx < before + n);
+                c = here ? firstList + i : c; idx = here ? idx - before : idx;
+                found |= here;
+                before += n;
+            }
+        }
+        if (c == firstList + nLists) return;
+        const size_t b = a.lists[(size_t)c * a.nBlocks + idx];
+        const u32 lane = threadIdx.x;
+        const FseMeta m = a.meta[b];
+        if (m.state == 0) continue;
+        const u32 tl = m.tableLog, ts = 1u << tl;
+        if (ts > ldsCapTs || ts > 64u * MAXC) {
+            if (lane == 0) { a.meta[b].state = 0; a.results[b] = FERR(tableLog_tooLarge); }
+            continue;
+        }
+        const WaveBuildLds w = wave_build_carve(wbLds, ldsCapTs, false);
+        *(uint2*)(w.nrm + 4 * lane) = *(const uint2*)(a.norms + b * 256 + 4 * lane);
+        __syncthreads();
+        const bool rev = ((m.state >> 2) & 3u) != FSE_DCLS_PLAIN;
+        u16* const A = a.atab + b * capTs;
+        u8* const S = a.symtab + b * capTs;
+        const bool fast = wave_spread_rank<MAXC>(w, m.maxSV, tl, lane, [&](u32 s) { return (u32)(int)w.nrm[s]; }, [&](u32 u, u32 s, u32 r, u32 nrm) {
+            const int n = (int)nrm;
+            const u32 next = (n > 0 ? (u32)n : 1u) + r;
+            const u32 nb = tl - hibit32(next);
+            const u32 ns = (next << nb) - ts;
+            const u32 x = rev ? __brev(u) >> (32u - tl) : u;
+            A[x] = rev ? (u16)(nb | ((__brev(ns) >> (32u - tl)) << 5)) : (u16)((ns & 0xFFFu) | (nb << 12));
+            S[x] = (u8)s;
+        });
+        if (lane == 0) a.meta[b].state = m.state | (fast ? 2u : 0u);
+    } while (STRIDE && total - pos > gridDim.x && ((pos += gridDim.x), true));
 }
 
 __global__ __launch_bounds__(256) void k_fse_export_dtable(FseDPrepArgs a, u32 capTs, u32* dtables, size_t dtStrideU32)
@@ -286,8 +290,11 @@
 {
     if (wb_small(ldsCapTs))
         hipLaunchKernelGGL(k_fse_dbuild<32>, dim3((unsigned)a.nBlocks), dim3(64), wave_build_lds_bytes(ldsCapTs, false), s, a, capTs, firstList, nLists, ldsCapTs);
-    else
-        hipLaunchKernelGGL(k_fse_dbuild<64>, dim3((unsigned)a.nBlocks), dim3(64), wave_build_lds_bytes(ldsCapTs, false), s, a, capTs, firstList, nLists, ldsCapTs);
+    else {
+        const size_t cap = grid_cap(16);
+        hipLaunchKernelGGL(k_fse_dbuild<64>, dim3((unsigned)(a.nBlocks < cap ? a.nBlocks : cap)), dim3(64), wave_build_lds_bytes(ldsCapTs, false), s, a, capTs, firstList,
+                           nLists, ldsCapTs);
+    }
 }
 static void launch_fse_dbuilds(const FseDPrepArgs& a, hipStream_t s)
 {
diff --git a/finitestateentropy_amd/csrc/hist.hip b/finitestateentropy_amd/csrc/hist.hip
--- a/finitestateentropy_amd/csrc/hist.hip
+++ b/finitestateentropy_amd/csrc/hist.hip
@@ -36,6 +36,7 @@
     const unsigned limitIn = (a.maxSVs && !a.useUniformIn) ? a.maxSVs[b] : a.uniformMaxSV;
     const bool checked = limitIn < 255u && !a.trustInput;
     const unsigned nOut = limitIn < 255u ? limitIn + 1u : 256u;
+    if (a.encCounts && b == 0 && lane < FSE_EBINS) a.encCounts[lane] = 0;
 
     u32 t0 = 0, t1 = 0, t2 = 0, t3 = 0;
 
diff --git a/finitestateentropy_amd/csrc/internal.h b/finitestateentropy_amd/csrc/internal.h
--- a/finitestateentropy_amd/csrc/internal.h
+++ b/finitestateentropy_amd/csrc/internal.h
@@ -25,6 +25,7 @@
     size_t* results;
     BlockView src;
     size_t nBlocks;
+    u32* encCounts = nullptr;
 };
 hipError_t launch_hist(const HistArgs& a, hipStream_t s);
 #define HIST_PIECE ((size_t)65536)
@@ -72,6 +73,7 @@
     unsigned maxTableLog;
     int G;
     unsigned slotU32;
+    int countCleared = 0;
     size_t nBlocks;
     unsigned onlyState;
     unsigned sizeSplit;
@@ -81,7 +83,7 @@
 enum { FSE_ENC_PAR = 1, FSE_ENC_LANE = 2 };
 #define FSE_ENC_WAVE_MIN 2048u
 __host__ __device__ inline bool fse_enc_skip(unsigned state, unsigned onlyState) { return state == 0 || (onlyState != 0 && state != onlyState); }
-hipError_t launch_fse_encode(FseEncArgs a, hipStream_t s);
+hipError_t launch_fse_encode(FseEncArgs a, hipStream_t s, bool boundedGrid = false);
 size_t fse_encode_blocks_per_round(unsigned maxTableLog);
 hipError_t launch_fse_encode_wave(FseEncArgs a, hipStream_t s);
 hipError_t launch_fse_enc_lists(const FseEncArgs& a, hipStream_t s);
@@ -102,7 +104,7 @@
     if (e == hipSuccess) e = launch_fse_encode_wave(a, s);
     if (e != hipSuccess) return e;
     a.onlyState = FSE_ENC_LANE;
-    return launch_fse_encode(a, s);
+    return launch_fse_encode(a, s, true);
 }
 
 #ifndef FSE_DBINS_N
@@ -290,6 +292,7 @@
 struct DevProps { int cus; int ldsPerCU; bool ok; };
 const DevProps& dev_props();
 hipError_t ensure_dyn_lds(const void* kernel, int bytes);
+unsigned grid_cap(unsigned perCU);
 int fse_compress_view(void* d_dst, size_t dstStride, size_t dstCapacity, size_t* d_results, const BlockView& src, unsigned maxSymbolValue, unsigned tableLog,
                       size_t nBlocks, void* d_workspace, size_t workspaceBytes, hipStream_t s);
 int huf_compress_view(int streams, void* d_dst, size_t dstStride, size_t dstCapacity, size_t* d_results, const BlockView& src, unsigned maxSymbolValue,
diff --git a/include/fsehip.h b/include/fsehip.h
--- a/include/fsehip.h
+++ b/include/fsehip.h
@@ -331,6 +331,7 @@
 FSEHIP_API int FSEHIP_probe_begin(void);
 FSEHIP_API int FSEHIP_probe_collect(double* totalMs16, unsigned* launches16);
 FSEHIP_API int FSEHIP_debug_decodeTiming(int enable, unsigned long long* out16);
+FSEHIP_API int FSEHIP_debug_gridCap(unsigned cap);
 #endif
 
 FSEHIP_API void FSEHIP_shardRange(size_t nBlocks, int rank, int world, size_t* first, size_t* count);
```
